# mit-acl/roman

Measured on AMD Instinct MI355X. Metric: submap-pair alignments/sec + p50 latency at n=m=200 objects, d=512, higher is better.
Workload: dtype f64 (fixed-point SpMV sums); 1 GPU; config 3: batch of 256 submap pairs per GPU, n=200 m=200 d=512, method=semanticgrav (xyz + 512-d descriptors + gravity prior); p50 latency measured on config 2 (single pair); pairs_per_call=256, n=200, m=200, d=512, method=semanticgrav, batches_in_flight=3

## Files before the change

include/roman_hip.h:

```cpp
#ifndef ROMAN_HIP_H
#define ROMAN_HIP_H

#include <stdint.h>

#ifdef __cplusplus
extern "C" {
#endif

#if defined(__GNUC__)
#define ROMAN_API __attribute__((visibility("default")))
#else
#define ROMAN_API
#endif

#define ROMAN_MAX_RATIO_FEATURES 8

#define ROMAN_OK                0
#define ROMAN_E_INVALID        -1
#define ROMAN_E_NO_DEVICE      -2
#define ROMAN_E_HIP            -3
#define ROMAN_E_NOMEM          -4
#define ROMAN_E_UNSUPPORTED    -5
#define ROMAN_E_TOO_LARGE      -6
#define ROMAN_E_INTERNAL       -7
// ... 283 lines not shown
                                int32_t S, const roman_submap_desc_t* descs,
                                double* pool, int32_t* count, int32_t* src, int64_t* ids_out, int32_t* status,
                                int32_t desc_dim, double* desc_out);

ROMAN_API int roman_submaps(roman_ctx_t* ctx, const roman_submap_params_t* sparams, int32_t N, int32_t F,
                            const double* seg_feats, const double* seg_times, const int64_t* seg_ids,
                            int32_t S, const roman_submap_desc_t* descs,
                            double* pool, int32_t* count, int32_t* src, int64_t* ids_out, int32_t* status,
                            int32_t desc_dim, double* desc_out);


typedef struct roman_frame_select_params {
    int32_t thin;
    int32_t want_mean;
    double  thin_dist;
    int32_t reserved[2];
} roman_frame_select_params_t;

ROMAN_API int roman_frame_select_dev(roman_ctx_t* ctx, const roman_frame_select_params_t* fparams, int32_t S, int32_t cap,
                                     const int32_t* count, const int32_t* src, int32_t N, const double* seg_times,
                                     int32_t Nf, const double* frame_times, const double* frame_pos, int32_t d, const double* frame_desc,
                                     uint64_t* mask, int32_t* n_sel, double* span, double* mean);

ROMAN_API int roman_frame_select(roman_ctx_t* ctx, const roman_frame_select_params_t* fparams, int32_t S, int32_t cap,
                                 const int32_t* count, const int32_t* src, int32_t N, const double* seg_times,
                                 int32_t Nf, const double* frame_times, const double* frame_pos, int32_t d, const double* frame_desc,
                                 uint64_t* mask, int32_t* n_sel, double* span, double* mean);

ROMAN_API int roman_stacked_sim_dev(roman_ctx_t* ctx, int32_t d, int32_t Nf0, const double* desc0, int32_t S0, const uint64_t* mask0,
                                    int32_t Nf1, const double* desc1, int32_t S1, const uint64_t* mask1, double* sim);

ROMAN_API int roman_stacked_sim(roman_ctx_t* ctx, int32_t d, int32_t Nf0, const double* desc0, int32_t S0, const uint64_t* mask0,
                                int32_t Nf1, const double* desc1, int32_t S1, const uint64_t* mask1, double* sim);

ROMAN_API int roman_ctx_set_stacked_band(roman_ctx_t* ctx, int32_t rows);


#define ROMAN_GRID_NEARBY  1
#define ROMAN_GRID_SKIP    2
#define ROMAN_GRID_GATED   4
#define ROMAN_GRID_TODO    8

typedef struct roman_grid_gate_params {
    double  radius;
    double  skip_distance;
    int32_t desc_dim;
    int32_t reserved0;
    double  desc_thresh;
    int32_t single_robot_lc;
    int32_t reserved1;
    double  lc_time_thresh;
    int32_t reserved[2];
} roman_grid_gate_params_t;

ROMAN_API int roman_grid_gate_dev(roman_ctx_t* ctx, const roman_grid_gate_params_t* gparams, int32_t S0, int32_t S1,
                                  const double* pos0, const double* pos_gt0, const double* T_w0, const double* time0, const double* desc0,
                                  const double* pos1, const double* pos_gt1, const double* T_w1, const double* time1, const double* desc1,
                                  double* dist, int32_t* flags, double* yaw_deg, double* sim, double* T_ij,
                                  int32_t* pairs, double* T_ref, int32_t* enable, int32_t* n_todo);

ROMAN_API int roman_grid_gate(roman_ctx_t* ctx, const roman_grid_gate_params_t* gparams, int32_t S0, int32_t S1,
                              const double* pos0, const double* pos_gt0, const double* T_w0, const double* time0, const double* desc0,
                              const double* pos1, const double* pos_gt1, const double* T_w1, const double* time1, const double* desc1,
                              double* dist, int32_t* flags, double* yaw_deg, double* sim, double* T_ij,
                              int32_t* pairs, double* T_ref, int32_t* enable, int32_t* n_todo);

ROMAN_API int roman_grid_gate_sim_dev(roman_ctx_t* ctx, const roman_grid_gate_params_t* gparams, int32_t S0, int32_t S1,
                                      const double* pos0, const double* pos_gt0, const double* T_w0, const double* time0,
                                      const double* pos1, const double* pos_gt1, const double* T_w1, const double* time1,
                                      double* dist, int32_t* flags, double* yaw_deg, const double* sim, double* T_ij,
                                      int32_t* pairs, double* T_ref, int32_t* enable, int32_t* n_todo);

ROMAN_API int roman_grid_gate_sim(roman_ctx_t* ctx, const roman_grid_gate_params_t* gparams, int32_t S0, int32_t S1,
                                  const double* pos0, const double* pos_gt0, const double* T_w0, const double* time0,
                                  const double* pos1, const double* pos_gt1, const double* T_w1, const double* time1,
                                  double* dist, int32_t* flags, double* yaw_deg, const double* sim, double* T_ij,
                                  int32_t* pairs, double* T_ref, int32_t* enable, int32_t* n_todo);



ROMAN_API int roman_submaps_fill_dev(roman_ctx_t* ctx, int32_t point_dim, int32_t cap, int32_t N, int32_t F,
                                     const double* seg_feats, const int64_t* seg_ids, int32_t S, const roman_submap_desc_t* descs,
                                     const int32_t* count, const int32_t* src, double* pool, int64_t* ids_out,
                                     int32_t desc_dim, double* desc_out);

ROMAN_API int roman_submaps_fill(roman_ctx_t* ctx, int32_t point_dim, int32_t cap, int32_t N, int32_t F,
                                 const double* seg_feats, const int64_t* seg_ids, int32_t S, const roman_submap_desc_t* descs,
                                 const int32_t* count, const int32_t* src, double* pool, int64_t* ids_out,
                                 int32_t desc_dim, double* desc_out);

ROMAN_API int roman_submap_boxes_dev(roman_ctx_t* ctx, int32_t S, int32_t F, int32_t cap, const double* pool, const int32_t* count,
                                     const double* T_odom_center, double* box);

ROMAN_API int roman_submap_boxes(roman_ctx_t* ctx, int32_t S, int32_t F, int32_t cap, const double* pool, const int32_t* count,
                                 const double* T_odom_center, double* box);

ROMAN_API int roman_grid_gate_aabb_dev(roman_ctx_t* ctx, const roman_grid_gate_params_t* gparams, int32_t S0, int32_t S1,
                                       const double* pos0, const double* pos_gt0, const double* T_w0, const double* time0, const double* desc0,
                                       const double* pos1, const double* pos_gt1, const double* T_w1, const double* time1, const double* desc1,
                                       double* dist, int32_t* flags, double* yaw_deg, double* sim, double* T_ij,
                                       int32_t* pairs, double* T_ref, int32_t* enable, int32_t* n_todo,
                                       const double* box0, const double* box1, const double* sim_in);

ROMAN_API int roman_grid_gate_aabb(roman_ctx_t* ctx, const roman_grid_gate_params_t* gparams, int32_t S0, int32_t S1,
                                   const double* pos0, const double* pos_gt0, const double* T_w0, const double* time0, const double* desc0,
                                   const double* pos1, const double* pos_gt1, const double* T_w1, const double* time1, const double* desc1,
                                   double* dist, int32_t* flags, double* yaw_deg, double* sim, double* T_ij,
                                   int32_t* pairs, double* T_ref, int32_t* enable, int32_t* n_todo,
                                   const double* box0, const double* box1, const double* sim_in);


ROMAN_API int roman_create_all_to_all(int32_t n1, int32_t n2, int32_t* out);

ROMAN_API int roman_score(roman_ctx_t* ctx, const roman_params_t* params,
                const double* D1, int32_t n1, const double* D2, int32_t n2, int32_t F,
                const int32_t* assoc, int32_t n_assoc);

ROMAN_API int roman_set_matrix_data(roman_ctx_t* ctx, const roman_params_t* params,
                          const double* M, const double* C, int32_t n);

ROMAN_API int roman_solve(roman_ctx_t* ctx, const double* u0);

ROMAN_API int roman_num_associations(const roman_ctx_t* ctx, int32_t* n_assoc);
ROMAN_API int roman_num_selected(const roman_ctx_t* ctx, int32_t* n_sel);
ROMAN_API int roman_get_selected_associations(const roman_ctx_t* ctx, int32_t* out);
ROMAN_API int roman_get_solution(const roman_ctx_t* ctx, int32_t* nodes, double* u, double* score,
                       roman_stats_t* stats);
ROMAN_API int roman_get_dense_matrices(const roman_ctx_t* ctx, double* M, double* C);
ROMAN_API int roman_get_upper_csr(const roman_ctx_t* ctx, int64_t* nnz, int64_t* rowptr ,
                        int32_t* cols, double* vals, double* diag );


ROMAN_API int roman_pose_batch(roman_ctx_t* ctx, int32_t dim, int32_t B,
                     const double* pts1, const double* pts2, const int64_t* corr_off,
                     double* T_out, int32_t* status_out);


#define ROMAN_STAGE_SINGLE   0
#define ROMAN_STAGE_COUNT_PASS 1
#define ROMAN_STAGE_FILL     2
#define ROMAN_STAGE_SOLVE    3
#define ROMAN_STAGE_COUNT    4
ROMAN_API int roman_profile_enable(roman_ctx_t* ctx, int on);
ROMAN_API int roman_profile_reset(roman_ctx_t* ctx);
ROMAN_API int roman_profile_get(roman_ctx_t* ctx, double ms[ROMAN_STAGE_COUNT],
                      int64_t launches[ROMAN_STAGE_COUNT]);

ROMAN_API int roman_debug_math(roman_ctx_t* ctx, int kind, const double* in1, const double* in2,
                     int64_t n, double* out);
ROMAN_API int roman_debug_cosine(roman_ctx_t* ctx, const roman_params_t* params,
                       const double* D1, int32_t n1, const double* D2, int32_t n2, int32_t F,
                       double* out);
ROMAN_API int roman_debug_live(const roman_ctx_t* ctx, int32_t* n_live, int32_t* idx, double* score);

ROMAN_API const char* roman_version(void);

#ifdef __cplusplus
}
#endif
#endif
```

roman_amd/_abi.py:

```python
import ctypes as C
import os

ROMAN_MAX_RATIO_FEATURES = 8

ROMAN_OK = 0
ROMAN_E_INVALID = -1
ROMAN_E_NOMEM = -4
ROMAN_E_UNSUPPORTED = -5
ROMAN_E_TOO_LARGE = -6
ROMAN_E_INTERNAL = -7
ROMAN_ST_OK = 0
ROMAN_ST_EMPTY_MAP = 1
ROMAN_ST_INSUFFICIENT = 2
ROMAN_ST_MAXITER = 4
ROMAN_ST_ASSOC_TRUNCATED = 8
ROMAN_ST_TIE_FALLBACK = 16
ROMAN_ST_WORKSPACE = 32
ROMAN_ST_INTERNAL = 64

ROMAN_INV_EUCLIDEAN = 0
ROMAN_INV_ROMAN = 1
ROMAN_INV_EUCLIDEAN_PRUNED = 2

ROMAN_FUSE_GEOMETRIC_MEAN = 0
# ... 175 lines not shown
    ]


class RomanSubmapDesc(C.Structure):
    _fields_ = [
        ("pos", C.c_double * 3),
        ("T_center_odom", C.c_double * 16),
        ("time", C.c_double),
        ("t_hi", C.c_double),
        ("t_lo", C.c_double),
    ]


class RomanGridGateParams(C.Structure):
    _fields_ = [
        ("radius", C.c_double),
        ("skip_distance", C.c_double),
        ("desc_dim", C.c_int32),
        ("reserved0", C.c_int32),
        ("desc_thresh", C.c_double),
        ("single_robot_lc", C.c_int32),
        ("reserved1", C.c_int32),
        ("lc_time_thresh", C.c_double),
        ("reserved", C.c_int32 * 2),
    ]


class RomanFrameSelectParams(C.Structure):
    _fields_ = [
        ("thin", C.c_int32),
        ("want_mean", C.c_int32),
        ("thin_dist", C.c_double),
        ("reserved", C.c_int32 * 2),
    ]


ROMAN_GRID_NEARBY = 1
ROMAN_GRID_SKIP = 2
ROMAN_GRID_GATED = 4
ROMAN_GRID_TODO = 8

SUBMAP_LDS_CAND = 4096

STATS_NBYTES = C.sizeof(RomanStats)
MNO_SOLUTION_NBYTES = C.sizeof(RomanMnoSolution)
RANSAC_RECORD_NBYTES = C.sizeof(RomanRansacRecord)
SUBMAP_PARAMS_NBYTES = C.sizeof(RomanSubmapParams)
SUBMAP_DESC_NBYTES = C.sizeof(RomanSubmapDesc)
GRID_GATE_PARAMS_NBYTES = C.sizeof(RomanGridGateParams)
FRAME_SELECT_PARAMS_NBYTES = C.sizeof(RomanFrameSelectParams)
STACKED_BAND_MIN = 32
LC_PARAMS_NBYTES = C.sizeof(RomanLcParams)
LC_RECORD_NBYTES = C.sizeof(RomanLcRecord)
PARAMS_NBYTES = C.sizeof(RomanParams)

_LIB = None
_LIB_PATH = os.environ.get("ROMAN_HIP_LIBRARY") or os.path.join(os.path.dirname(os.path.abspath(__file__)), "csrc", "libroman_hip.so")


class RomanHipError(RuntimeError):
    pass


def lib_path():
    return _LIB_PATH


def load_library():
    global _LIB
    if _LIB is not None:
        return _LIB
    if not os.path.exists(_LIB_PATH):
        raise RomanHipError(
            f"{_LIB_PATH} is missing: build it with `python -c 'import __graft_entry__ as g; g.build()'` "
            "(hipcc --offload-arch=gfx950).  There is no CPU fallback for roman_amd.")
    lib = C.CDLL(_LIB_PATH)
    vp, i32, i64, dbl = C.c_void_p, C.c_int32, C.c_int64, C.c_double
    P = C.POINTER
    ctxp = vp
    protos = {
        "roman_params_default": (C.c_int, [P(RomanParams)]),
        "roman_ctx_create": (C.c_int, [P(ctxp), C.c_int, vp]),
        "roman_ctx_destroy": (C.c_int, [ctxp]),
        "roman_ctx_set_pipeline": (C.c_int, [ctxp, C.c_int]),
        "roman_ctx_sync": (C.c_int, [ctxp]),
        "roman_ctx_set_host_batching": (C.c_int, [ctxp, C.c_int, C.c_int]),
        "roman_ctx_set_wide_teams": (C.c_int, [ctxp, C.c_int]),
        "roman_ctx_join": (C.c_int, [ctxp, C.c_int]),
        "roman_ctx_join_on": (C.c_int, [ctxp, C.c_int, C.c_void_p]),
        "roman_ctx_skipped": (C.c_int, [ctxp, C.c_int, P(i64)]),
        "roman_last_error": (C.c_char_p, [ctxp]),
        "roman_align_batch_dev": (C.c_int, [ctxp, P(RomanParams), i32, vp, vp, vp, vp, vp, i32,
                                            vp, vp, vp, i32, vp, vp, vp, vp, vp]),
        "roman_align_batch": (C.c_int, [ctxp, P(RomanParams), i32, vp, i64, vp, vp, vp, vp, i32,
                                        vp, vp, vp, i32, vp, vp, vp, vp, vp]),
        "roman_align_batch_resident": (C.c_int, [ctxp, P(RomanParams), i32, vp, vp, vp, vp, vp, i32,
                                                 vp, vp, vp, i32, vp, vp, vp, vp, vp]),
        "roman_lc_tail_dev": (C.c_int, [ctxp, P(RomanLcParams), i32, vp, vp, vp, vp, vp, vp, vp, vp, vp, vp, vp, vp]),
        "roman_align_lc_batch_dev": (C.c_int, [ctxp, P(RomanParams), i32, vp, vp, vp, vp, vp, i32,
                                               vp, vp, vp, i32, vp, vp, vp, vp, vp,
                                               P(RomanLcParams), vp, vp, vp, vp, vp, vp, vp, vp, vp]),
        "roman_align_lc_batch": (C.c_int, [ctxp, P(RomanParams), i32, vp, i64, vp, vp, vp, vp, i32,
                                           vp, vp, vp, i32, vp, vp, vp, vp, vp,
                                           P(RomanLcParams), vp, vp, vp, i32, vp, vp, i32, vp, vp, vp, vp]),
        "roman_shared_ids_dev": (C.c_int, [ctxp, i32, vp, vp, vp, vp, vp, vp, vp]),
        "roman_shared_reduce_dev": (C.c_int, [ctxp, i32, i32, vp, i64, vp, vp, vp, vp, vp, vp, vp]),
        "roman_align_lc_batch_ids": (C.c_int, [ctxp, P(RomanParams), i32, vp, i64, vp, vp, vp, vp, i32,
                                               vp, vp, vp, i32, vp, vp, vp, vp, vp,
                                               P(RomanLcParams), vp, vp, vp, i32, vp, vp, i32, vp, vp, vp, vp,
                                               vp, vp, vp, vp]),
        "roman_mno_batch_dev": (C.c_int, [ctxp, P(RomanParams), i32, vp, vp, vp, vp, vp, i32,
                                          vp, vp, i32, i32, vp, vp, vp]),
        "roman_mno_batch": (C.c_int, [ctxp, P(RomanParams), i32, vp, i64, vp, vp, vp, vp, i32,
                                      vp, vp, i32, i32, vp, vp, vp]),
        "roman_ransac_batch_dev": (C.c_int, [ctxp, P(RomanRansacParams), i32, vp, vp, vp, vp, vp, i32, vp, vp, vp]),
        "roman_ransac_batch": (C.c_int, [ctxp, P(RomanRansacParams), i32, vp, i64, vp, vp, vp, vp, i32, vp, vp, vp]),
        "roman_submaps_dev": (C.c_int, [ctxp, P(RomanSubmapParams), i32, i32, vp, vp, vp, i32, vp, vp, vp, vp, vp, vp, i32, vp]),
        "roman_submaps": (C.c_int, [ctxp, P(RomanSubmapParams), i32, i32, vp, vp, vp, i32, vp, vp, vp, vp, vp, vp, i32, vp]),
        "roman_grid_gate_dev": (C.c_int, [ctxp, P(RomanGridGateParams), i32, i32] + [vp] * 19),
        "roman_grid_gate": (C.c_int, [ctxp, P(RomanGridGateParams), i32, i32] + [vp] * 19),
        "roman_grid_gate_sim_dev": (C.c_int, [ctxp, P(RomanGridGateParams), i32, i32] + [vp] * 17),
        "roman_grid_gate_sim": (C.c_int, [ctxp, P(RomanGridGateParams), i32, i32] + [vp] * 17),
        "roman_submaps_fill_dev": (C.c_int, [ctxp, i32, i32, i32, i32, vp, vp, i32, vp, vp, vp, vp, vp, i32, vp]),
        "roman_submaps_fill": (C.c_int, [ctxp, i32, i32, i32, i32, vp, vp, i32, vp, vp, vp, vp, vp, i32, vp]),
        "roman_submap_boxes_dev": (C.c_int, [ctxp, i32, i32, i32, vp, vp, vp, vp]),
        "roman_submap_boxes": (C.c_int, [ctxp, i32, i32, i32, vp, vp, vp, vp]),
        "roman_grid_gate_aabb_dev": (C.c_int, [ctxp, P(RomanGridGateParams), i32, i32] + [vp] * 22),
        "roman_grid_gate_aabb": (C.c_int, [ctxp, P(RomanGridGateParams), i32, i32] + [vp] * 22),
        "roman_frame_select_dev": (C.c_int, [ctxp, P(RomanFrameSelectParams), i32, i32, vp, vp, i32, vp, i32, vp, vp, i32, vp, vp, vp, vp, vp]),
        "roman_frame_select": (C.c_int, [ctxp, P(RomanFrameSelectParams), i32, i32, vp, vp, i32, vp, i32, vp, vp, i32, vp, vp, vp, vp, vp]),
        "roman_stacked_sim_dev": (C.c_int, [ctxp, i32, i32, vp, i32, vp, i32, vp, i32, vp, vp]),
        "roman_stacked_sim": (C.c_int, [ctxp, i32, i32, vp, i32, vp, i32, vp, i32, vp, vp]),
        "roman_ctx_set_stacked_band": (C.c_int, [ctxp, i32]),
        "roman_ctx_has_history": (C.c_int, [ctxp, P(RomanParams), i32, P(i32)]),
        "roman_ctx_cosine_screen_stats": (C.c_int, [ctxp, P(C.c_int64), P(C.c_int64), P(C.c_double)]),
        "roman_create_all_to_all": (C.c_int, [i32, i32, vp]),
        "roman_deal_problems": (C.c_int, [i32, vp, vp, vp, i32, i32, vp, P(i32)]),
        "roman_score": (C.c_int, [ctxp, P(RomanParams), vp, i32, vp, i32, i32, vp, i32]),
        "roman_set_matrix_data": (C.c_int, [ctxp, P(RomanParams), vp, vp, i32]),
        "roman_solve": (C.c_int, [ctxp, vp]),
        "roman_num_associations": (C.c_int, [ctxp, P(i32)]),
        "roman_num_selected": (C.c_int, [ctxp, P(i32)]),
        "roman_get_selected_associations": (C.c_int, [ctxp, vp]),
        "roman_get_solution": (C.c_int, [ctxp, vp, vp, P(dbl), P(RomanStats)]),
        "roman_get_dense_matrices": (C.c_int, [ctxp, vp, vp]),
        "roman_get_upper_csr": (C.c_int, [ctxp, P(i64), vp, vp, vp, vp]),
        "roman_pose_batch": (C.c_int, [ctxp, i32, i32, vp, vp, vp, vp, vp]),
        "roman_profile_enable": (C.c_int, [ctxp, C.c_int]),
        "roman_profile_reset": (C.c_int, [ctxp]),
        "roman_profile_get": (C.c_int, [ctxp, P(dbl), P(i64)]),
        "roman_debug_math": (C.c_int, [ctxp, C.c_int, vp, vp, i64, vp]),
        "roman_debug_cosine": (C.c_int, [ctxp, P(RomanParams), vp, i32, vp, i32, i32, vp]),
        "roman_debug_live": (C.c_int, [ctxp, P(i32), vp, vp]),
        "roman_version": (C.c_char_p, []),
    }
    for name, (res, args) in protos.items():
        fn = getattr(lib, name)
        fn.restype = res
        fn.argtypes = args
    lib._roman_symbols = tuple(protos)
    _LIB = lib
    return lib


EXPORTED_SYMBOLS = (
    "roman_params_default", "roman_ctx_create", "roman_ctx_destroy", "roman_ctx_set_pipeline", "roman_ctx_sync", "roman_ctx_set_host_batching", "roman_ctx_set_wide_teams", "roman_ctx_join", "roman_ctx_join_on",
    "roman_ctx_skipped", "roman_last_error",
    "roman_align_batch_dev", "roman_align_batch", "roman_align_batch_resident", "roman_lc_tail_dev", "roman_align_lc_batch_dev", "roman_align_lc_batch", "roman_shared_ids_dev", "roman_shared_reduce_dev", "roman_align_lc_batch_ids", "roman_mno_batch_dev", "roman_mno_batch", "roman_ransac_batch_dev", "roman_ransac_batch", "roman_submaps_dev", "roman_submaps", "roman_grid_gate_dev", "roman_grid_gate", "roman_grid_gate_sim_dev", "roman_grid_gate_sim", "roman_submaps_fill_dev", "roman_submaps_fill", "roman_submap_boxes_dev", "roman_submap_boxes", "roman_grid_gate_aabb_dev", "roman_grid_gate_aabb", "roman_frame_select_dev", "roman_frame_select", "roman_stacked_sim_dev", "roman_stacked_sim", "roman_ctx_set_stacked_band", "roman_ctx_has_history", "roman_ctx_cosine_screen_stats", "roman_deal_problems", "roman_create_all_to_all", "roman_score",
    "roman_set_matrix_data", "roman_solve", "roman_num_associations", "roman_num_selected",
    "roman_get_selected_associations", "roman_get_solution", "roman_get_dense_matrices",
    "roman_get_upper_csr", "roman_pose_batch", "roman_profile_enable", "roman_profile_reset",
    "roman_profile_get", "roman_debug_math", "roman_debug_cosine", "roman_debug_live",
    "roman_version",
)
```

roman_amd/csrc/kernels.hip.h:

```cpp
#pragma once
#include <hip/hip_cooperative_groups.h>
#include <hip/hip_runtime.h>
#include <stdint.h>
#include <type_traits>
#include "../../include/roman_hip.h"

namespace roman {

constexpr int WAVE = 64;
constexpr int STREAM_MAXL = 3072;

struct DevParams {
    roman_params_t p;
    double sig2;
    double sin_unc;
    double x_eps;
    double x_mindist;
    int32_t single;
    int32_t gravity;
    int32_t F;
    int32_t max_compact;
    int32_t gmode;
    int32_t diag_one;
    int32_t keep_all;
// ... 2287 lines not shown
#define LMARK(i_) do { } while (0)
#endif
        for (int q = tid; q < L; q += LISTS_NT) degS[q] = degGiven ? rowCnt[lo + q] : 0u;
        __syncthreads();
        if (!degGiven) {
        sweep([&](int k, unsigned long long m, int c) {
            if (m) {
                atomicAdd(&degS[k], (uint32_t)__popcll(m));
                while (m) { atomicAdd(&degS[(c << 6) + __builtin_ctzll(m)], 1u); m &= m - 1ull; }
            }
        });
        __syncthreads();
        }
        LMARK(1);
        int N = 64; while (N < L) N <<= 1;
        if (eqMax <= 0 || !place_keys(L, N, eqMax, [&](int k) { return degS[k]; }, keyS, reinterpret_cast<uint32_t*>(tabS), reinterpret_cast<uint32_t*>(tabS) + (STREAM_MAXL + 64), tmpS, wsum)) {
        for (int t = tid; t < N; t += LISTS_NT) keyS[t] = (t < L) ? (((degS[t] + 1u) << 12) | (uint32_t)(4095 - t)) : 0u;
        __syncthreads();
        for (int k2 = 2; k2 <= N; k2 <<= 1)
            for (int j2 = k2 >> 1; j2 > 0; j2 >>= 1) {
                for (int t = tid; t < (N >> 1); t += LISTS_NT) {
                    const int i1 = ((t & ~(j2 - 1)) << 1) | (t & (j2 - 1)), i2 = i1 | j2;
                    const uint32_t a = keyS[i1], c2 = keyS[i2];
                    const bool desc = (i1 & k2) == 0;
                    if ((a < c2) == desc) { keyS[i1] = c2; keyS[i2] = a; }
                }
                __syncthreads();
            }
        }
        LMARK(2);
        uint32_t total = 0;
        {
            const int PER = (L + LISTS_NT - 1) / LISTS_NT;
            uint32_t sum = 0;
            for (int t = 0; t < PER; ++t) {
                const int q = tid * PER + t;
                if (q < L) sum += (min((keyS[q] >> 12) - 1u, (uint32_t)(L - 1 - q)) + 3u) & ~3u;
            }
            const uint32_t inc = wave_incl_scan(sum);
            if (lane == WAVE - 1) wsum[w] = inc;
            __syncthreads();
            uint32_t wbase = 0;
            for (int t = 0; t < NW; ++t) { if (t < w) wbase += wsum[t]; total += wsum[t]; }
            if (tid == 0) {
                const unsigned long long base = atomicAdd(&tot->listTop, (unsigned long long)total);
                st[b].listOff = (int64_t)base;
                const bool fits = (long long)(base + total) <= capList;
                if (!fits) { st[b].kind = 2; atomicAdd(&tot->overflow, 1); }
                okS = fits ? 1 : 0;
            }
            uint32_t run = wbase + inc - sum;
            for (int t = 0; t < PER; ++t) {
                const int q = tid * PER + t;
                if (q < L) {
                    const uint32_t k = 4095u - (keyS[q] & 4095u);
                    perm[lo + q] = k; rowPos[lo + k] = (uint32_t)q; tmpS[q] = (uint16_t)k;
                    tabS[k] = ((unsigned long long)run << 16) | (unsigned long long)q; listOff[lo + q] = run; degS[k] = 0u;
                    run += (min((keyS[q] >> 12) - 1u, (uint32_t)(L - 1 - q)) + 3u) & ~3u;
                }
            }
        }
        __syncthreads();
        if (!okS) continue;
        uint16_t* const lists = listPool + st[b].listOff;
        LMARK(3);
        {
        uint32_t* const qw = qS + w * LISTS_QCAP;
        uint32_t qn = 0;
        auto lds_order = [&]() {
            __builtin_amdgcn_fence(__ATOMIC_RELEASE, "wavefront"); __builtin_amdgcn_wave_barrier(); __builtin_amdgcn_fence(__ATOMIC_ACQUIRE, "wavefront");
        };
        auto place = [&](uint32_t base, uint32_t n, auto full) {
            constexpr int CH = LISTS_QRUN / WAVE;
            uint32_t kk[CH], qq[CH], slot[CH]; unsigned long long tk[CH], tq[CH]; bool act[CH];
#pragma unroll
            for (int x = 0; x < CH; ++x) {
                const uint32_t idx = (uint32_t)(x * WAVE + lane);
                act[x] = decltype(full)::value || idx < n;
                const uint32_t e = qw[base + (act[x] ? idx : 0u)];
                kk[x] = e >> 16; qq[x] = e & 0xffffu;
                tk[x] = tabS[kk[x]]; tq[x] = tabS[qq[x]];
            }
#pragma unroll
            for (int x = 0; x < CH; ++x) {
                const bool mine = ((uint32_t)tk[x] & 0xffffu) < ((uint32_t)tq[x] & 0xffffu);
                if (act[x]) slot[x] = atomicAdd(&degS[mine ? kk[x] : qq[x]], 1u);
            }
#pragma unroll
            for (int x = 0; x < CH; ++x) {
                const bool mine = ((uint32_t)tk[x] & 0xffffu) < ((uint32_t)tq[x] & 0xffffu);
                const uint32_t at = (uint32_t)((mine ? tk[x] : tq[x]) >> 16) + slot[x];
                const uint16_t v = (uint16_t)(mine ? qq[x] : kk[x]);
                if (act[x]) { if (at < (uint32_t)winCap) winS[at] = v; else lists[at] = v; }
            }
        };
        auto drain = [&]() {
            if (qn >= (uint32_t)LISTS_QRUN) {
                lds_order();
                while (qn >= (uint32_t)LISTS_QRUN) { qn -= LISTS_QRUN; place(qn, LISTS_QRUN, std::true_type{}); }
                lds_order();
            }
        };
        sweep([&](int k, unsigned long long m, int c) {
            const uint32_t cnt = (uint32_t)__popcll(m);
            const uint32_t incl = wave_incl_scan(cnt);
            const uint32_t npairs = (uint32_t)__builtin_amdgcn_readlane((int)incl, WAVE - 1);
            const uint32_t kq = ((uint32_t)k << 16) | (uint32_t)(c << 6);
            if (qn + npairs <= (uint32_t)LISTS_QCAP) {
                uint32_t at = qn + incl - cnt;
                while (m) { qw[at++] = kq + (uint32_t)__builtin_ctzll(m); m &= m - 1ull; }
                qn += npairs;
            } else {
                while (true) {
                    const unsigned long long bm = __ballot(m != 0ull);
                    if (bm == 0ull) break;
                    if (m) {
                        qw[qn + __builtin_amdgcn_mbcnt_hi((uint32_t)(bm >> 32), __builtin_amdgcn_mbcnt_lo((uint32_t)bm, 0u))] = kq + (uint32_t)__builtin_ctzll(m);
                        m &= m - 1ull;
                    }
                    qn += (uint32_t)__popcll(bm);
                    drain();
                }
            }
            drain();
        });
        lds_order();
        if (qn) place(0u, qn, std::false_type{});
        }
        __syncthreads();
        LMARK(4);
        for (int p = tid; p < L; p += LISTS_NT) {
            const uint32_t k = tmpS[p];
            const uint32_t cnt = degS[k];
            rowCnt[lo + p] = cnt;
            const uint32_t o = (uint32_t)(tabS[k] >> 16);
            for (uint32_t e = o + cnt; e < o + ((cnt + 3u) & ~3u); ++e) { if (e < (uint32_t)winCap) winS[e] = (uint16_t)0xffffu; else lists[e] = (uint16_t)0xffffu; }
            dst.lp[lo + p] = src.lp[lo + k]; dst.ld[lo + p] = src.ld[lo + k];
        }
        {
            const uint32_t nq = min(total, (uint32_t)winCap) >> 2;
            __syncthreads();
            for (uint32_t i = (uint32_t)tid; i < nq; i += LISTS_NT)
                reinterpret_cast<uint2*>(lists)[i] = reinterpret_cast<const uint2*>(winS)[i];
        }
#ifdef ROMAN_LISTS_TIMING
        LMARK(5);
        if (tid == 0 && (b & 63) == 0) printf("[k_lists] b=%d L=%d cycles: degrees %llu sort %llu offsets %llu scatter %llu tail %llu\n", b, L,
                                              tl_[1] - tl_[0], tl_[2] - tl_[1], tl_[3] - tl_[2], tl_[4] - tl_[3], tl_[5] - tl_[4]);
#endif
#undef LMARK
    }
}

__global__ void __launch_bounds__(64) k_slicegeom(const ProbDesc* __restrict__ probs, ProbState* __restrict__ st,
                                                  const uint32_t* __restrict__ rowCnt,
                                                  uint32_t* __restrict__ sliceWidth, uint32_t* __restrict__ sliceBase)
{
    const int b = blockIdx.x, lane = threadIdx.x;
    if (st[b].kind != 0) return;
    const int L = st[b].L;
    const int64_t lo = probs[b].liveOff;
    const int nsl = (L + 63) >> 6;
    uint32_t width = 0;
    if (lane < nsl) {
        const int hi = min(L, (lane << 6) + 64);
        for (int p = lane << 6; p < hi; ++p) width = max(width, rowCnt[lo + p]);
        width = (width + 3u) & ~3u;
        sliceWidth[lo + lane] = width;
    }
    const uint32_t v = width * 64u;
    const uint32_t ex = wave_excl_scan(v, lane);
    if (lane < nsl) sliceBase[lo + lane] = ex;
    if (lane == WAVE - 1) st[b].nnzCap = ex + v;
}

__global__ void __launch_bounds__(1024) k_probscan(int B, int NG , long long capNnz, ProbState* __restrict__ st, BatchTotals* __restrict__ tot)
{
    __shared__ long long shl[17];
    __shared__ int shi[17];
    __shared__ int red[1];
    const int tid = threadIdx.x, nt = blockDim.x;
    const int PER = (B + nt - 1) / nt;
    const int b0 = tid * PER, b1 = min(B, b0 + PER);
    constexpr int PC = 8;
    int cK[PC], cL[PC]; uint32_t cC[PC];
#pragma unroll
    for (int j = 0; j < PC; ++j) { const int b = b0 + j; const bool in = j < PER && b < b1; cK[j] = in ? st[b].kind : 2; cL[j] = in ? st[b].L : 0; cC[j] = in ? st[b].nnzCap : 0u; }
    auto get = [&](int b, int& kind, int& L, long long& cap) {
        const int j = b - b0;
        if (j < PC) {
#pragma unroll
            for (int t = 0; t < PC; ++t) if (t == j) { kind = cK[t]; L = cL[t]; cap = (long long)cC[t]; }
        } else { kind = st[b].kind; L = st[b].L; cap = (long long)st[b].nnzCap; }
        if (kind >= 2) cap = 0;
    };
    long long sC = 0;
    for (int b = b0; b < b1; ++b) { int kind, L; long long cap; get(b, kind, L, cap); sC += cap; }
    long long totC; int totG;
    const long long baseC = block_excl_scan(sC, shl, totC);
    int sG = 0;
    {
        long long acc = baseC;
        for (int b = b0; b < b1; ++b) {
            int kind, L; long long cap; get(b, kind, L, cap);
            acc += cap;
            if (kind == 0 && acc <= capNnz) sG += min(NG, (L + 63) >> 6);
        }
    }
    const int baseG = block_excl_scan(sG, shi, totG);
    if (tid == 0) red[0] = 0;
    __syncthreads();
    int nover = 0;
    {
        long long acc = baseC; int gacc = baseG;
        for (int b = b0; b < b1; ++b) {
            int kind, L; long long cap; get(b, kind, L, cap);
            const bool fits = acc + cap <= capNnz;
            const int ng = (kind == 0 && fits) ? min(NG, (L + 63) >> 6) : 0;
            st[b].nnzOff = fits ? acc : 0; st[b].sgBase = gacc;
            if (!fits && kind < 2) { st[b].kind = 2; ++nover; }
            acc += cap; gacc += ng;
        }
    }
    for (int off = 32; off > 0; off >>= 1) nover += __shfl_xor(nover, off);
    if ((tid & 63) == 0 && nover) atomicAdd(&red[0], nover);
    __syncthreads();
    if (tid == 0) { tot->nnzTotal = totC < capNnz ? totC : capNnz; tot->sliceGroups = totG; tot->needNnz = totC; tot->overflow += red[0]; }
}

constexpr int FILL_E = 1;
constexpr int FILL_Q = 256;

constexpr int FILL_RPB = 128;
struct FillRows { int32_t* k; int32_t* i; int32_t* j; uint32_t* base; double* s; double* za; double* zb; };
constexpr int FILL_ROWBYTES = 4 * 4 + 3 * 8;

template <bool GRAV, typename IdxT, int CM, bool QUAD>
__device__ __forceinline__ uint32_t fill_item(const DevParams& D, const ProbDesc& pd, int L, int row0, int nrows, int wq0, int Ww,
                                              int w, int wpb, int lane,
                                              const int32_t* cI, const int32_t* cJ, const double* cS,
                                              const double* cZa, const double* cZb, const uint32_t* cBase, const uint32_t* cPos,
                                              const double* __restrict__ TA, const double* __restrict__ TB,
                                              const unsigned long long* __restrict__ mbase, const uint32_t* __restrict__ pbase,
                                              const FillRows& R ,
                                              uint32_t* qK, uint32_t* qQ, uint32_t* qE,
                                              IdxT* __restrict__ cols, double* __restrict__ vals)
{
    constexpr bool LDSCOL = CM == 1;
    const int W = (L + 63) >> 6;
    const int64_t nwords = (int64_t)nrows * Ww;
    const int w0 = wq0 >> 6;
    const unsigned long long lt = (1ull << lane) - 1ull;
    uint32_t head = 0, queued = 0, upper = 0;

    auto evaluate = [&](uint32_t take) {
        __builtin_amdgcn_fence(__ATOMIC_RELEASE, "wavefront");
        __builtin_amdgcn_wave_barrier();
        __builtin_amdgcn_fence(__ATOMIC_ACQUIRE, "wavefront");
        bool on[FILL_E]; int rl[FILL_E], k[FILL_E], q[FILL_E]; uint32_t e[FILL_E];
        int i[FILL_E], j[FILL_E], iq[FILL_E], jq[FILL_E]; double sk[FILL_E], sq[FILL_E], dz[FILL_E];
        uint32_t base[FILL_E], pk[FILL_E], pq[FILL_E];
#pragma unroll
        for (int h = 0; h < FILL_E; ++h) {
            const uint32_t idx = (uint32_t)lane + 64u * (uint32_t)h;
            on[h] = idx < take;
            const uint32_t s = (head + (on[h] ? idx : 0u)) & (FILL_Q - 1);
            rl[h] = (int)qK[s]; k[h] = R.k[rl[h]]; q[h] = (int)qQ[s]; e[h] = qE[s];
        }
#pragma unroll
        for (int h = 0; h < FILL_E; ++h) {
            if (LDSCOL) {
                i[h] = cI[k[h]]; j[h] = cJ[k[h]]; iq[h] = cI[q[h]]; jq[h] = cJ[q[h]]; sk[h] = cS[k[h]]; sq[h] = cS[q[h]];
                dz[h] = GRAV ? (cZa[k[h]] - cZa[q[h]]) - (cZb[k[h]] - cZb[q[h]]) : 0.0;
                base[h] = cBase[k[h]]; pk[h] = cPos[k[h]]; pq[h] = cPos[q[h]];
            } else {
                const int r_ = rl[h], ql = q[h] - wq0;
                i[h] = R.i[r_]; j[h] = R.j[r_]; iq[h] = cI[ql]; jq[h] = cJ[ql]; sk[h] = R.s[r_]; sq[h] = cS[ql];
                dz[h] = GRAV ? (R.za[r_] - cZa[ql]) - (R.zb[r_] - cZb[ql]) : 0.0;
                base[h] = R.base[r_]; pk[h] = (uint32_t)(row0 + r_); pq[h] = cPos[ql];
            }
        }
        double a[FILL_E], bb[FILL_E];
#pragma unroll
        for (int h = 0; h < FILL_E; ++h) { a[h] = TA[(int64_t)i[h] * pd.n1 + iq[h]]; bb[h] = TB[(int64_t)j[h] * pd.n2 + jq[h]]; }
#pragma unroll
        for (int h = 0; h < FILL_E; ++h) {
            double c;
            if (GRAV && D.gmode != 3) {
                const double ch = fabs(a[h] - bb[h]);
                const double hm = a[h] > bb[h] ? a[h] : bb[h];
                double cv = fabs(dz[h]) - D.sin_unc * hm;
                if (cv < 0.0) cv = 0.0;
                c = sqrt(ch * ch + cv * cv);
            } else {
                c = fabs(a[h] - bb[h]);
            }
            const double sa = fx_exp(((-0.5 * c) * c) / D.sig2);
            const double v = fuse_pair(D, sa, sk[h], sq[h]);
            const bool keep = v > D.p.affinityeps;
            if (on[h]) {
                cols[col_pos<QUAD>(base[h] & ~63u, base[h] & 63u, e[h])] = keep ? (IdxT)pq[h] : fb_inert<IdxT>(pk[h]);
                vals[val_pos<QUAD>(base[h] & ~63u, base[h] & 63u, e[h])] = keep ? v : 0.0;
                upper += (keep && q[h] > k[h]) ? 1u : 0u;
            }
        }
        head = (head + take) & (FILL_Q - 1); queued -= take;
    };

    const int64_t nblk = (nwords + 63) >> 6;
    unsigned long long m_next = 0ull; uint32_t p_next = 0u, k_next = 0u;
    auto fetch = [&](int64_t x_) {
        const int r_ = (int)x_ / Ww;
        const int64_t a_ = (int64_t)R.k[r_] * W + (w0 + ((int)x_ - r_ * Ww));
        k_next = (uint32_t)r_; m_next = mbase[a_]; p_next = pbase[a_];
    };
    {
        const int64_t x = (int64_t)w * 64 + lane;
        if (w < nblk && x < nwords) fetch(x);
    }
    for (int64_t blk = w; blk < nblk; blk += wpb) {
        unsigned long long m = m_next; uint32_t e = p_next; const uint32_t kl = k_next;
        const int64_t x = blk * 64 + lane;
        {
            const int64_t xn = x + (int64_t)wpb * 64;
            m_next = 0ull; p_next = 0u;
            if (blk + wpb < nblk && xn < nwords) fetch(xn);
// ... 1014 lines not shown
constexpr int ST_MAXSL = STREAM_MAXL / 64;
constexpr int SMALL_MAXL = 128;
constexpr int COO_E = 6;
constexpr int COO_CAP = 64 * COO_E;
constexpr uint32_t ST_CZ = 0x8000u, ST_MASK = 0x7fffu;
constexpr unsigned long long FX_MAGIC_BITS = 0x4338000000000000ull;
#define FX_MAGIC 6755399441055744.0

#define ROMAN_GLOBAL __attribute__((address_space(1)))
#define ROMAN_LDS __attribute__((address_space(3)))
typedef const ROMAN_GLOBAL unsigned long long* g_quad_cp;
typedef const ROMAN_GLOBAL dbl2_t* g_pair_cp;
typedef const ROMAN_LDS double* l_vec_cp;
typedef ROMAN_LDS unsigned long long* l_acc_p;

__device__ __forceinline__ uint32_t uni(uint32_t v) { return (uint32_t)__builtin_amdgcn_readfirstlane((int)v); }
__device__ __forceinline__ int uni(int v) { return __builtin_amdgcn_readfirstlane(v); }
__device__ __forceinline__ double uni(double v)
{
    const long long b = __double_as_longlong(v);
    const int lo = __builtin_amdgcn_readfirstlane((int)b), hi = __builtin_amdgcn_readfirstlane((int)(b >> 32));
    return __longlong_as_double(((long long)hi << 32) | (unsigned int)lo);
}

template <int CTRL, int ROWMASK>
__device__ __forceinline__ double dpp_mov(double v)
{
    const long long b = __double_as_longlong(v);
    const int lo = __builtin_amdgcn_update_dpp(0, (int)b, CTRL, ROWMASK, 0xf, false);
    const int hi = __builtin_amdgcn_update_dpp(0, (int)(b >> 32), CTRL, ROWMASK, 0xf, false);
    return __longlong_as_double(((long long)hi << 32) | (unsigned int)lo);
}
__device__ __forceinline__ double wave_sum63(double v)
{
    v += dpp_mov<0xB1, 0xf>(v);
    v += dpp_mov<0x4E, 0xf>(v);
    v += dpp_mov<0x124, 0xf>(v);
    v += dpp_mov<0x128, 0xf>(v);
    v += dpp_mov<0x142, 0xa>(v);
    v += dpp_mov<0x143, 0xc>(v);
    return v;
}
__device__ __forceinline__ double wave_max63(double v)
{
    v = fmax(v, dpp_mov<0xB1, 0xf>(v));
    v = fmax(v, dpp_mov<0x4E, 0xf>(v));
    v = fmax(v, dpp_mov<0x124, 0xf>(v));
    v = fmax(v, dpp_mov<0x128, 0xf>(v));
    v = fmax(v, dpp_mov<0x142, 0xa>(v));
    v = fmax(v, dpp_mov<0x143, 0xc>(v));
    return v;
}
__device__ __forceinline__ double readlane63(double v)
{
    const long long b = __double_as_longlong(v);
    const int lo = __builtin_amdgcn_readlane((int)b, 63), hi = __builtin_amdgcn_readlane((int)(b >> 32), 63);
    return __longlong_as_double(((long long)hi << 32) | (unsigned int)lo);
}

constexpr int RED_STRIDE = 8;
constexpr int red_doubles(int NW) { return 2 * NW * RED_STRIDE + 8 > 72 ? 2 * NW * RED_STRIDE + 8 : 72; }
template <int NW, int NS, int NM>
__device__ __forceinline__ void block_red(double (&sv)[NS > 0 ? NS : 1], double (&mv)[NM > 0 ? NM : 1], double* red, int& par, int tid)
{
    static_assert(NS + NM <= RED_STRIDE, "reduction scratch");
    static_assert(NW == 1 || NW == 4 || NW == 8 || NW == 16, "cross-wave butterfly");
    if (NW == 1) {
#pragma unroll
        for (int i = 0; i < NS; ++i) sv[i] = uni(readlane63(wave_sum63(sv[i])));
#pragma unroll
        for (int i = 0; i < NM; ++i) mv[i] = uni(readlane63(wave_max63(mv[i])));
        __syncthreads();
        return;
    }
    double* rr = red + NW * RED_STRIDE * par;
    par ^= 1;
    const int w = uni(tid >> 6);
#pragma unroll
    for (int i = 0; i < NS; ++i) {
        const double s = readlane63(wave_sum63(sv[i]));
        if ((tid & 63) == 0) rr[RED_STRIDE * w + i] = s;
    }
#pragma unroll
    for (int i = 0; i < NM; ++i) {
        const double m = readlane63(wave_max63(mv[i]));
        if ((tid & 63) == 0) rr[RED_STRIDE * w + NS + i] = m;
    }
    __syncthreads();
    const int src = (tid & 63) & (NW - 1);
#pragma unroll
    for (int i = 0; i < NS; ++i) {
        double v = rr[RED_STRIDE * src + i];
        v += dpp_mov<0xB1, 0xf>(v);
        v += dpp_mov<0x4E, 0xf>(v);
        if (NW > 4) v += dpp_mov<0x124, 0xf>(v);
        if (NW > 8) v += dpp_mov<0x128, 0xf>(v);
        sv[i] = uni(v);
    }
#pragma unroll
    for (int i = 0; i < NM; ++i) {
        double v = rr[RED_STRIDE * src + NS + i];
        v = fmax(v, dpp_mov<0xB1, 0xf>(v));
        v = fmax(v, dpp_mov<0x4E, 0xf>(v));
        if (NW > 4) v = fmax(v, dpp_mov<0x124, 0xf>(v));
        if (NW > 8) v = fmax(v, dpp_mov<0x128, 0xf>(v));
        mv[i] = uni(v);
    }
}

template <int NW, int NS>
__device__ __forceinline__ const double* block_post(const double (&sv)[NS], double* red, int& par, int tid)
{
    static_assert(NW == 4 || NW == 8 || NW == 16, "cross-wave butterfly");
    double* rr = red + NW * RED_STRIDE * par;
    par ^= 1;
    const int w = uni(tid >> 6);
#pragma unroll
    for (int i = 0; i < NS; ++i) {
        const double s = readlane63(wave_sum63(sv[i]));
        if ((tid & 63) == 0) rr[RED_STRIDE * w + i] = s;
    }
    return rr;
}
template <int NW, int NS>
__device__ __forceinline__ void block_collect(double (&sv)[NS], const double* rr, int tid)
{
    const int src = (tid & 63) & (NW - 1);
#pragma unroll
    for (int i = 0; i < NS; ++i) {
        double v = rr[RED_STRIDE * src + i];
        v += dpp_mov<0xB1, 0xf>(v);
        v += dpp_mov<0x4E, 0xf>(v);
        if (NW > 4) v += dpp_mov<0x124, 0xf>(v);
        if (NW > 8) v += dpp_mov<0x128, 0xf>(v);
        sv[i] = uni(v);
    }
}

__device__ __forceinline__ double fx_decode(unsigned long long a, double inv)
{
    return fma((double)(uint32_t)(a >> 32), 4294967296.0, (double)(uint32_t)a) * inv;
}

template <int NW, bool HASCZ, int MAXL, bool COOONLY = false >
__device__ void solve_up(const DevParams& D, int b, const ProbDesc& pd, ProbState* st,
                         const double* __restrict__ feats, const int32_t* __restrict__ assoc,
                         const int32_t* __restrict__ plp , const int32_t* __restrict__ lpAsc,
                         const uint32_t* __restrict__ rowPosPool, const double* __restrict__ pld ,
                         const uint32_t* __restrict__ sliceBasePool,
                         const uint16_t* __restrict__ colsPool, const double* __restrict__ valsPool,
                         const double* __restrict__ u0, const SolveOut& O,
                         double* xg , unsigned long long* accM , unsigned long long* accC , int Lc,
                         uint32_t* cumQ , double* red, int* sint, unsigned char* cooLds ,
                         int cooPre = -1 ,
                         int rbPre = -1 )
{
    constexpr int NT = NW * 64;
#ifdef ROMAN_SOLVE_TIMING
    const unsigned long long tentry_ = __builtin_readcyclecounter();
#endif
#ifdef ROMAN_SMALL_TIMING
    const unsigned long long tw0_ = wall_clock64();
#endif
    constexpr int KMAX = (MAXL + NT - 1) / NT;
    constexpr int LCAP = MAXL + 64;
    const roman_params_t& P = D.p;
    const double p_eps = uni(P.eps), p_beta = uni(P.beta), p_tol_u = uni(P.tol_u), p_tol_F = uni(P.tol_F);
    const int p_maxin = uni(P.maxiniters), p_maxout = uni(P.maxoliters), p_maxls = uni(P.maxlsiters), p_rescale = uni(P.rescale_u0);
    const int tid = threadIdx.x, lane = tid & 63, w = uni(tid >> 6);
#define FOR_K_ALL(k_, p_) _Pragma("unroll") for (int k_ = 0; k_ < KMAX; ++k_) if ([[maybe_unused]] const int p_ = tid + k_ * NT; true)
#define FOR_K(k_, p_) _Pragma("unroll") for (int k_ = 0; k_ < KMAX; ++k_) if ([[maybe_unused]] const int p_ = tid + k_ * NT; NW != 1 || k_ < kUsed)
    const int L = uni(st[b].L), rb = rbPre >= 0 ? rbPre : uni(st[b].rowBase);
    const int kUsed = uni((L + NT - 1) / NT);
    const int64_t lo = pd.liveOff;
    const int nsl = (L + 63) >> 6;
    int par = 0;

    int status = ROMAN_ST_OK;
    roman_stats_t S;
    S.n_assoc_in = pd.nA; S.n_live = L; S.nnz_upper = (int64_t)st[b].nnzUpper;
    S.n_pass = 0; S.outer_iters = 0; S.inner_iters = 0; S.ls_trials = 0; S.score = 0.0; S.d_final = 0.0;
    int n_pass = 0, ls_trials = 0, inner_iters = 0;
    double F = 0.0, d = 0.0;
    if (pd.n1 == 0 || pd.n2 == 0) status |= ROMAN_ST_EMPTY_MAP;
    if (L <= 0) {
        finish_one(D, b, pd, feats, assoc, plp, lpAsc, rowPosPool, nullptr, O, nullptr, nullptr, nullptr, nullptr, L, rb, lo, F, status, S, red, sint);
        return;
    }
#ifdef ROMAN_SOLVE_TIMING
    unsigned long long tacc[8] = {0, 0, 0, 0, 0, 0, 0, 0}, tcnt[8] = {0, 0, 0, 0, 0, 0, 0, 0};
    unsigned long long tlast = __builtin_readcyclecounter();
#endif
    g_quad_cp cbase = (g_quad_cp)(colsPool + st[b].nnzOff) + lane;
    g_pair_cp vbase = (g_pair_cp)(valsPool + st[b].nnzOff) + lane;
    l_vec_cp xl = (l_vec_cp)xg;
    l_acc_p aM = (l_acc_p)accM; l_acc_p aC = (l_acc_p)accC;

    __syncthreads();
    const uint32_t cqv = cooPre >= 0 ? 0u : ((lane < nsl) ? (sliceBasePool[lo + lane] >> 8) : (st[b].nnzCap >> 8));
#define CUMQ(s_) ((uint32_t)__builtin_amdgcn_readlane((int)cqv, (s_)))
    for (int p = tid; p < Lc; p += NT) { xg[p] = 0.0; accM[p] = 0ull; accC[p] = 0ull; }
    double u[KMAX], Wu[KMAX], sd[KMAX], tk[KMAX], Mn[KMAX], Cn[KMAX];
    FOR_K_ALL(k, p) {
        const bool in = p < L;
        sd[k] = in ? pld[lo + p] : 0.0;
        u[k] = in ? (u0 ? u0[lo + plp[lo + p]] : 1.0) : 0.0;
        Wu[k] = tk[k] = Mn[k] = Cn[k] = 0.0;
    }
    __syncthreads();

    [[maybe_unused]] uint32_t cpq[COO_E]; [[maybe_unused]] double cv[COO_E];
    [[maybe_unused]] int cooRounds = -1;
    if constexpr (NW == 1) {
        uint32_t* lpq = reinterpret_cast<uint32_t*>(cooLds); double* lv = reinterpret_cast<double*>(cooLds + 4 * COO_CAP);
        const uint32_t Tq = CUMQ(nsl);
        const uint32_t q1 = nsl > 1 ? CUMQ(1) : Tq;
        uint32_t cnt = 0;
        if (cooPre >= 0) {
            cnt = (uint32_t)cooPre;
            cooRounds = (int)((cnt + 63u) >> 6);
#pragma unroll
            for (int e = 0; e < COO_E; ++e) {
                const uint32_t at = (uint32_t)lane * (uint32_t)cooRounds + (uint32_t)e;
                const bool have = e < cooRounds && at < cnt;
                const uint32_t dummy = (uint32_t)L + (uint32_t)lane;
                cpq[e] = have ? lpq[at] : (dummy | (dummy << 8) | 0x10000u);
                cv[e] = have ? lv[at] : 0.0;
            }
            __syncthreads();
        } else
        if (!COOONLY && (unsigned long long)st[b].nnzUpper <= (unsigned long long)COO_CAP && nsl <= 2) {
            for (uint32_t qq = 0; qq < Tq; ++qq) {
                const unsigned long long cw = cbase[(size_t)qq * 64];
                const dbl2_t v0 = vbase[(size_t)(2 * qq) * 64], v1 = vbase[(size_t)(2 * qq + 1) * 64];
                const uint32_t row = (qq >= q1 ? 64u : 0u) + (uint32_t)lane;
                const double v4[4] = {v0.x, v0.y, v1.x, v1.y};
#pragma unroll
                for (int e = 0; e < 4; ++e) {
                    const uint32_t lab = (uint32_t)(cw >> (16 * e)) & 0xffffu, col = lab & ST_MASK;
                    const bool real = col < (uint32_t)L;
                    const unsigned long long m_ = __ballot(real);
                    if (real) {
                        const uint32_t at = cnt + (uint32_t)__builtin_amdgcn_mbcnt_hi((uint32_t)(m_ >> 32), __builtin_amdgcn_mbcnt_lo((uint32_t)m_, 0u));
                        if (at < (uint32_t)COO_CAP) { lpq[at] = row | (col << 8) | ((lab & ST_CZ) ? 0x10000u : 0u); lv[at] = v4[e]; }
                    }
                    cnt += (uint32_t)__popcll(m_);
                }
            }
            __syncthreads();
            if (cnt <= (uint32_t)COO_CAP) {
                cooRounds = (int)((cnt + 63u) >> 6);
#pragma unroll
                for (int e = 0; e < COO_E; ++e) {
                    const uint32_t at = (uint32_t)lane * (uint32_t)cooRounds + (uint32_t)e;
                    const bool have = e < cooRounds && at < cnt;
                    const uint32_t dummy = (uint32_t)L + (uint32_t)lane;
                    cpq[e] = have ? lpq[at] : (dummy | (dummy << 8) | 0x10000u);
                    cv[e] = have ? lv[at] : 0.0;
                }
            }
            __syncthreads();
        }
    }

    [[maybe_unused]] const double* pendRR = nullptr; [[maybe_unused]] bool pend = false;
    double usum = 0.0, alpha = 1.0, unsum = 0.0, du2 = 0.0, xmaxT = 0.0;
    auto collect_pending = [&]() {
        if constexpr (NW != 1) {
            if (pend) { double q2[2]; block_collect<NW, 2>(q2, pendRR, tid); unsum = q2[0]; du2 = q2[1]; pend = false; }
        }
    };
    auto spmv = [&](double xmax, int mp1, const bool split, const double de_) {
        TMARK(3);
        if (!(xmax > 0.0) || mp1 <= 0) {
            if constexpr (NW != 1) { if (pend) { __syncthreads(); collect_pending(); } }
            FOR_K(k, p) { Mn[k] = 0.0; Cn[k] = 0.0; }
            ++n_pass;
            return;
        }
        const double de = (!split && de_ > 0.0) ? de_ : 0.0;
        int e_ = (int)((__double_as_longlong(xmax) >> 52) & 0x7ff) - 1023;
        int s_ = 48 - e_;
        if (de > 0.0) s_ -= (int)((__double_as_longlong(1.0 + de) >> 52) & 0x7ff) - 1023 + 1;
        s_ = s_ > 960 ? 960 : (s_ < -960 ? -960 : s_);
        const double sc = bits_f64((unsigned long long)(1023 + s_) << 52), inv = bits_f64((unsigned long long)(1023 - s_) << 52);
        bool streamed = false;
        if constexpr (NW == 1) streamed = cooRounds >= 0;
        const int Sx = (COOONLY || streamed) ? 0 : min(nsl, (mp1 + 63) >> 6);
        const uint32_t T = COOONLY ? 0u : CUMQ(Sx);
        const uint32_t qs = (uint32_t)(((unsigned long long)T * (unsigned)w) / NW), qe = (uint32_t)(((unsigned long long)T * (unsigned)(w + 1)) / NW);
        [[maybe_unused]] unsigned long long rc[ST_D]; [[maybe_unused]] dbl2_t rv0[ST_D], rv1[ST_D];
        if constexpr (!COOONLY) {
            const uint32_t qlast = (qe > qs ? qe : qs + 1u) - 1u;
            g_quad_cp cb0 = T ? cbase : (g_quad_cp)colsPool + lane;
            g_pair_cp vb0 = T ? vbase : (g_pair_cp)valsPool + lane;
#pragma unroll
            for (int t = 0; t < ST_D; ++t) {
                const uint32_t qq = min(qs + (uint32_t)t, qlast);
                rc[t] = cb0[(size_t)qq * 64];
                rv0[t] = vb0[(size_t)(2 * qq) * 64]; rv1[t] = vb0[(size_t)(2 * qq + 1) * 64];
            }
        }
        FOR_K(k, p) if (p < L) xg[p] = tk[k] * sc;
        __syncthreads();
        collect_pending();
        TMARK(6);
        if constexpr (NW == 1) {
            if (cooRounds >= 0) {
#pragma unroll
                for (int e = 0; e < COO_E; ++e) {
                    if (e < cooRounds) {
                        const uint32_t p_ = cpq[e] & 0xffu, q_ = (cpq[e] >> 8) & 0xffu;
                        const bool cz = HASCZ && (cpq[e] & 0x10000u);
                        const double xp_ = xl[p_], xq_ = xl[q_];
                        const double w_ = cz ? cv[e] : cv[e] + de;
                        if (xq_ != 0.0) {
                            __hip_atomic_fetch_add(aM + p_, (unsigned long long)__double_as_longlong(fma(w_, xq_, FX_MAGIC)) - FX_MAGIC_BITS, __ATOMIC_RELAXED, __HIP_MEMORY_SCOPE_WORKGROUP);
                            if (split && !cz) __hip_atomic_fetch_add(aC + p_, (unsigned long long)__double_as_longlong(xq_ + FX_MAGIC) - FX_MAGIC_BITS, __ATOMIC_RELAXED, __HIP_MEMORY_SCOPE_WORKGROUP);
                        }
                        if (xp_ != 0.0) {
                            __hip_atomic_fetch_add(aM + q_, (unsigned long long)__double_as_longlong(fma(w_, xp_, FX_MAGIC)) - FX_MAGIC_BITS, __ATOMIC_RELAXED, __HIP_MEMORY_SCOPE_WORKGROUP);
                            if (split && !cz) __hip_atomic_fetch_add(aC + q_, (unsigned long long)__double_as_longlong(xp_ + FX_MAGIC) - FX_MAGIC_BITS, __ATOMIC_RELAXED, __HIP_MEMORY_SCOPE_WORKGROUP);
                        }
                        __builtin_amdgcn_sched_barrier(0);
                    }
                }
            }
        }
        auto stream = [&](auto split_tag) {
            constexpr bool SPLIT = decltype(split_tag)::value;
            int s = 0;
            {
                int lo_ = 0, hi_ = Sx;
                while (hi_ - lo_ > 1) { const int mid_ = (lo_ + hi_) >> 1; if (CUMQ(mid_) <= qs) lo_ = mid_; else hi_ = mid_; }
                s = lo_;
            }
            uint32_t nextB = CUMQ(s + 1);
            unsigned long long smI = 0ull; [[maybe_unused]] unsigned long long scI = 0ull;
            uint32_t pieceQ = qs;
            double xp = xl[s * 64 + lane];
            double xpn = xl[(s + 1) * 64 + lane];
            [[maybe_unused]] unsigned long long iCp = (unsigned long long)__double_as_longlong(xp + FX_MAGIC) - FX_MAGIC_BITS;
            l_vec_cp ga[4], gn[4]; double xa[4], xn[4];
#define UP_GATHER(C_, G_, X_)                                                                               \
            {                                                                                               \
                const uint32_t lo__ = (uint32_t)(C_), hi__ = (uint32_t)((C_) >> 32);                        \
                (G_)[0] = xl + (lo__ & ST_MASK); (G_)[1] = xl + ((lo__ >> 16) & ST_MASK);                   \
                (G_)[2] = xl + (hi__ & ST_MASK); (G_)[3] = xl + ((hi__ >> 16) & ST_MASK);                   \
                (X_)[0] = *(G_)[0]; (X_)[1] = *(G_)[1]; (X_)[2] = *(G_)[2]; (X_)[3] = *(G_)[3];             \
            }
#define UP_PUSH(G_, OFF_, V_) __hip_atomic_fetch_add((l_acc_p)(G_) + (OFF_), (V_), __ATOMIC_RELAXED, __HIP_MEMORY_SCOPE_WORKGROUP)
#define UP_CONSUME(Q_, C_, V0_, V1_)                                                                        \
            {                                                                                               \
                [[maybe_unused]] const uint32_t clo = (uint32_t)(C_), chi = (uint32_t)((C_) >> 32);         \
                                                         \
                const double w0 = SPLIT ? (V0_).x : ((HASCZ && (clo & ST_CZ)) ? (V0_).x : (V0_).x + de);    \
                const double w1 = SPLIT ? (V0_).y : ((HASCZ && (clo & (ST_CZ << 16))) ? (V0_).y : (V0_).y + de); \
                const double w2 = SPLIT ? (V1_).x : ((HASCZ && (chi & ST_CZ)) ? (V1_).x : (V1_).x + de);    \
                const double w3 = SPLIT ? (V1_).y : ((HASCZ && (chi & (ST_CZ << 16))) ? (V1_).y : (V1_).y + de); \
                smI += (unsigned long long)__double_as_longlong(fma(w0, xa[0], FX_MAGIC));                  \
                smI += (unsigned long long)__double_as_longlong(fma(w1, xa[1], FX_MAGIC));                  \
                smI += (unsigned long long)__double_as_longlong(fma(w2, xa[2], FX_MAGIC));                  \
                smI += (unsigned long long)__double_as_longlong(fma(w3, xa[3], FX_MAGIC));                  \
                if constexpr (SPLIT) {                                                                      \
                    if (HASCZ) {                                                                            \
                        scI += (unsigned long long)__double_as_longlong(((clo & ST_CZ) ? 0.0 : xa[0]) + FX_MAGIC); \
                        scI += (unsigned long long)__double_as_longlong(((clo & (ST_CZ << 16)) ? 0.0 : xa[1]) + FX_MAGIC); \
                        scI += (unsigned long long)__double_as_longlong(((chi & ST_CZ) ? 0.0 : xa[2]) + FX_MAGIC); \
                        scI += (unsigned long long)__double_as_longlong(((chi & (ST_CZ << 16)) ? 0.0 : xa[3]) + FX_MAGIC); \
                    } else {                  \
                        scI += (unsigned long long)__double_as_longlong(xa[0] + FX_MAGIC);                  \
                        scI += (unsigned long long)__double_as_longlong(xa[1] + FX_MAGIC);                  \
                        scI += (unsigned long long)__double_as_longlong(xa[2] + FX_MAGIC);                  \
                        scI += (unsigned long long)__double_as_longlong(xa[3] + FX_MAGIC);                  \
                    }                                                                                       \
                }                                                                                           \
                if (xp != 0.0) {                                \
                    UP_PUSH(ga[0], LCAP, (unsigned long long)__double_as_longlong(fma(w0, xp, FX_MAGIC)) - FX_MAGIC_BITS); \
                    UP_PUSH(ga[1], LCAP, (unsigned long long)__double_as_longlong(fma(w1, xp, FX_MAGIC)) - FX_MAGIC_BITS); \
                    UP_PUSH(ga[2], LCAP, (unsigned long long)__double_as_longlong(fma(w2, xp, FX_MAGIC)) - FX_MAGIC_BITS); \
                    UP_PUSH(ga[3], LCAP, (unsigned long long)__double_as_longlong(fma(w3, xp, FX_MAGIC)) - FX_MAGIC_BITS); \
                    if constexpr (SPLIT) {                                                                  \
                        if (!HASCZ || !(clo & ST_CZ)) UP_PUSH(ga[0], 2 * LCAP, iCp);                        \
                        if (!HASCZ || !(clo & (ST_CZ << 16))) UP_PUSH(ga[1], 2 * LCAP, iCp);                \
                        if (!HASCZ || !(chi & ST_CZ)) UP_PUSH(ga[2], 2 * LCAP, iCp);                        \
                        if (!HASCZ || !(chi & (ST_CZ << 16))) UP_PUSH(ga[3], 2 * LCAP, iCp);                \
                    }                                                                                       \
                }                                                                                           \
                if ((Q_) + 1 == nextB || (Q_) + 1 == qe) {             \
                    const unsigned long long nterm = (unsigned long long)(((Q_) + 1 - pieceQ) * 4u) * FX_MAGIC_BITS; \
                    UP_PUSH(xl + (s * 64 + lane), LCAP, smI - nterm);                                       \
                    if constexpr (SPLIT) UP_PUSH(xl + (s * 64 + lane), 2 * LCAP, scI - nterm);              \
                    smI = 0ull; scI = 0ull; pieceQ = (Q_) + 1;                                              \
                    if ((Q_) + 1 < qe) {                                                                    \
                        const int s_old_ = s;                                                               \
                        do { ++s; nextB = CUMQ(s + 1); } while (nextB <= (Q_) + 1);                         \
                        xp = (s == s_old_ + 1) ? xpn : xl[s * 64 + lane];                                   \
                        xpn = xl[(s + 1) * 64 + lane];                                                      \
                        iCp = (unsigned long long)__double_as_longlong(xp + FX_MAGIC) - FX_MAGIC_BITS;      \
                    }                                                                                       \
                }                                                                                           \
            }
            UP_GATHER(rc[0], ga, xa)
            uint32_t q0 = qs;
            for (; q0 + ST_D <= qe; q0 += ST_D) {
#pragma unroll
                for (int t = 0; t < ST_D; ++t) {
                    const uint32_t q = q0 + t;
                    const unsigned long long c = rc[t];
                    const dbl2_t v0 = rv0[t], v1 = rv1[t];
                    const uint32_t qn = min(q + (uint32_t)ST_D, qe - 1u);
                    rc[t] = cbase[(size_t)qn * 64];
                    rv0[t] = vbase[(size_t)(2 * qn) * 64]; rv1[t] = vbase[(size_t)(2 * qn + 1) * 64];
                    UP_GATHER(rc[(t + 1) % ST_D], gn, xn)
                    UP_CONSUME(q, c, v0, v1)
#pragma unroll
                    for (int e = 0; e < 4; ++e) { ga[e] = gn[e]; xa[e] = xn[e]; }
                }
            }
#pragma unroll
            for (int t = 0; t < ST_D; ++t) {
                const uint32_t q = q0 + t;
                if (q < qe) {
                    UP_GATHER(rc[(t + 1) % ST_D], gn, xn)
                    UP_CONSUME(q, rc[t], rv0[t], rv1[t])
#pragma unroll
                    for (int e = 0; e < 4; ++e) { ga[e] = gn[e]; xa[e] = xn[e]; }
                }
            }
#undef UP_CONSUME
#undef UP_PUSH
#undef UP_GATHER
        };
        if (!COOONLY && qs < qe) {
            if (split) stream(std::true_type{}); else stream(std::false_type{});
        }
        TMARK(Sx <= 2 ? 4 : 0);
        __syncthreads();
        TMARK(1);
        FOR_K(k, p) {
            if (p < L) {
                Mn[k] = fx_decode(accM[p], inv); accM[p] = 0ull;
                if (split) { Cn[k] = fx_decode(accC[p], inv); accC[p] = 0ull; } else Cn[k] = 0.0;
            } else { Mn[k] = 0.0; Cn[k] = 0.0; }
        }
        ++n_pass;
        TMARK(2);
    };

    enum { PH_RESCALE, PH_INIT, PH_TRIAL, PH_SPLIT };
    int phase = p_rescale ? PH_RESCALE : PH_INIT;
    int mp1T = 0;
    int i = 0, j = 0, kk = 0;

    auto normalize_u = [&]() {
        double r[1] = {0.0}, m0[1] = {0.0};
        FOR_K(k, p) r[0] += u[k] * u[k];
        block_red<NW, 1, 0>(r, m0, red, par, tid);
        const double nr = sqrt(r[0]);
        if (nr > 0.0) FOR_K(k, p) u[k] /= nr;
    };
    auto load_u_as_x = [&]() {
        double r0[1] = {0.0}, m2[2] = {0.0, 0.0};
        FOR_K(k, p) { tk[k] = u[k]; m2[0] = fmax(m2[0], u[k]); if (u[k] > 0.0) m2[1] = (double)(p + 1); }
        block_red<NW, 0, 2>(r0, m2, red, par, tid);
        xmaxT = m2[0]; mp1T = (int)m2[1];
    };
    auto finish_trial = [&](double r2, const double (&m2)[2]) {
        const double nr = sqrt(r2);
        double q[2] = {0.0, 0.0}, m0[1] = {0.0};
        FOR_K(k, p) {
            double t = tk[k];
            if (nr > 0.0 && t != 0.0) { t /= nr; tk[k] = t; }
            q[0] += t;
            const double df = t - u[k]; q[1] += df * df;
        }
        TMARK(3);
        if constexpr (NW == 1) { block_red<NW, 2, 0>(q, m0, red, par, tid); unsum = q[0]; du2 = q[1]; }
        else { pendRR = block_post<NW, 2>(q, red, par, tid); pend = true; }
        TMARK(7);
        xmaxT = (nr > 0.0) ? m2[0] / nr : m2[0]; mp1T = (int)m2[1];
    };
    auto build_trial = [&]() {
        double r[1] = {0.0}, m2[2] = {0.0, 0.0};
        FOR_K(k, p) {
            const double up = u[k];
            const double g = ((sd[k] + d) * up - d * usum) + Wu[k];
            double t = up + alpha * g;
            t = (p < L && t > 0.0) ? t : 0.0;
            tk[k] = t; r[0] += t * t;
            m2[0] = fmax(m2[0], t);
            if (t > 0.0) m2[1] = (double)(p + 1);
        }
        TMARK(3);
        block_red<NW, 1, 2>(r, m2, red, par, tid);
        TMARK(6);
        finish_trial(r[0], m2);
    };
    auto objective = [&](const double (&uu)[KMAX], const double (&ww)[KMAX], double us) -> double {
        double r[1] = {0.0}, m0[1] = {0.0};
        FOR_K(k, p) {
            const double up = uu[k];
            const double g = ((sd[k] + d) * up - d * us) + ww[k];
            r[0] += up * g;
        }
        block_red<NW, 1, 0>(r, m0, red, par, tid);
        return r[0];
    };
    auto d_ratio = [&](bool absval, double& acc, double& cnt) {
        double r2[2] = {0.0, 0.0}, m0[1] = {0.0};
        FOR_K(k, p) {
            const double up = u[k], Cbu = (usum - Cn[k]) - up;
            if (p < L && Cbu > p_eps && up > p_eps) { const double r_ = (Mn[k] + sd[k] * up) / Cbu; r2[0] += absval ? fabs(r_) : r_; r2[1] += 1.0; }
        }
        block_red<NW, 2, 0>(r2, m0, red, par, tid);
        acc = r2[0]; cnt = r2[1];
    };

    if (phase == PH_INIT) normalize_u();
    load_u_as_x();
    for (;;) {
        spmv(xmaxT, mp1T, phase == PH_INIT || phase == PH_SPLIT, phase == PH_TRIAL ? d : 0.0);
        if (phase == PH_RESCALE) {
            FOR_K(k, p) u[k] = (p < L) ? Mn[k] + sd[k] * u[k] : 0.0;
            normalize_u();
            load_u_as_x();
            phase = PH_INIT;
            continue;
        }
        if (phase == PH_INIT) {
            double r1[1] = {0.0}, m0[1] = {0.0};
            FOR_K(k, p) r1[0] += u[k];
            block_red<NW, 1, 0>(r1, m0, red, par, tid);
            usum = r1[0];
            double acc, cnt;
            d_ratio(false, acc, cnt);
            d = (cnt > 0.0) ? acc / cnt : 0.0;
            i = 0;
            if (i >= p_maxout) break;
        } else if (phase == PH_SPLIT) {
            double acc, cnt;
            d_ratio(true, acc, cnt);
            if (cnt > 0.0) d += acc / cnt; else break;
            ++i;
            if (i >= p_maxout) break;
        } else {
            ++ls_trials;
            const double Fnew = objective(tk, Mn, unsum);
            const double deltaF = Fnew - F;
            if (deltaF < -p_eps && kk + 1 < p_maxls) {
                alpha *= p_beta; ++kk;
                build_trial();
                continue;
            }
            const double du = sqrt(du2);
            F = Fnew; usum = unsum;
            FOR_K(k, p) { u[k] = tk[k]; Wu[k] = Mn[k]; }
            ++inner_iters; ++j;
            const bool stop = du < p_tol_u || fabs(deltaF) < p_tol_F;
            if (stop || j >= p_maxin) {
                phase = PH_SPLIT;
                continue;
            }
        }
        if (phase != PH_TRIAL) {
            FOR_K(k, p) Wu[k] = Mn[k] + Cn[k] * d;
            F = objective(u, Wu, usum); j = 0;
        }
        alpha = 1.0; kk = 0;
        build_trial();
        phase = PH_TRIAL;
    }
    if (i >= p_maxout) status |= ROMAN_ST_MAXITER;
    S.n_pass = n_pass; S.ls_trials = ls_trials; S.inner_iters = inner_iters;
    S.outer_iters = i; S.score = F; S.d_final = d;
#ifdef ROMAN_SOLVE_TIMING
    TMARK(3);
#endif
    __syncthreads();
    FOR_K(k, p) if (p < L) xg[p] = u[k];
#ifdef ROMAN_SMALL_TIMING
    const unsigned long long tt0_ = __builtin_readcyclecounter();
    const unsigned long long tw1_ = wall_clock64();
#endif
    finish_one(D, b, pd, feats, assoc, plp, lpAsc, rowPosPool, nullptr, O, xg, reinterpret_cast<double*>(accM),
               reinterpret_cast<int32_t*>(accC), reinterpret_cast<int32_t*>(accC) + Lc, L, rb, lo, F, status, S, red, sint);
#ifdef ROMAN_SOLVE_TIMING
    if (tid == 0 && O.dbg) {
        unsigned long long sum_ = 0; for (int t = 0; t < 8; ++t) sum_ += tacc[t];
        tacc[5] = __builtin_readcyclecounter() - tentry_ - sum_; tcnt[5] = 1;
        unsigned long long* dg = O.dbg + (size_t)b * 16;
        for (int t = 0; t < 8; ++t) { dg[t] = tacc[t]; dg[8 + t] = tcnt[t]; }
    }
#endif
#ifdef ROMAN_SMALL_TIMING
    if (tid == 0 && ((b & 255) == 0 || b < 2 || (NW == 1 && n_pass >= 100)))
        printf("[solve_up<%d>] b=%d L=%d nnz=%llu passes %d tail (selection, pose, outputs) %llu cycles; wall clock (10 ns): entered %llu iteration done %llu left %llu\n", NW, b, L,
               (unsigned long long)st[b].nnzUpper, n_pass, __builtin_readcyclecounter() - tt0_, tw0_, tw1_, wall_clock64());
#endif
#undef FOR_K
#undef FOR_K_ALL
#undef CUMQ
}

template <int NW, bool HASCZ, int MAXL>
__global__ void __launch_bounds__(NW * 64, NW == 1 ? 3 : 1) k_solve_up(DevParams D, int B, const ProbDesc* __restrict__ probs,
                                                      ProbState* __restrict__ st,
                                                      const double* __restrict__ feats, const int32_t* __restrict__ assoc,
                                                      const int32_t* __restrict__ plp, const int32_t* __restrict__ lpAsc,
                                                      const uint32_t* __restrict__ rowPos, const double* __restrict__ pld,
                                                      const uint32_t* __restrict__ sliceBase,
                                                      const uint16_t* __restrict__ cols, const double* __restrict__ vals,
                                                      const double* __restrict__ u0, SolveOut O,
                                                      int* __restrict__ queue, int Lc, int Llo, int Lhi, int R )
{
    extern __shared__ __attribute__((aligned(16))) unsigned char smem[];
    double* xg = reinterpret_cast<double*>(smem);
    unsigned long long* accM = reinterpret_cast<unsigned long long*>(xg + Lc);
    unsigned long long* accC = accM + Lc;
    double* red = reinterpret_cast<double*>(accC + Lc);
    uint32_t* cumQ = reinterpret_cast<uint32_t*>(red + red_doubles(NW));
    int* sint = reinterpret_cast<int*>(cumQ + ST_MAXSL + 2);
    unsigned char* cooLds = reinterpret_cast<unsigned char*>(sint + 8);
    for (;;) {
        if (threadIdx.x < WAVE) {
            const int ln = threadIdx.x;
            int base_ = B; unsigned long long m_ = 0ull;
            for (;;) {
                int t_ = 0;
                if (ln == 0) t_ = atomicAdd(queue, R);
                base_ = __builtin_amdgcn_readfirstlane(t_);
                if (base_ >= B) break;
                const int b_ = base_ + ln;
                bool take = false;
                if (ln < R && b_ < B) { const int Lq = st[b_].L; take = st[b_].kind == 0 && Lq >= Llo && Lq <= Lhi; }
                m_ = __ballot(take);
                if (m_) break;
            }
            if (ln == 0) { sint[2] = base_; sint[3] = (int)(uint32_t)m_; sint[4] = (int)(uint32_t)(m_ >> 32); }
        }
        __syncthreads();
        const int base = uni(sint[2]);
        unsigned long long mask = ((unsigned long long)(uint32_t)uni(sint[4]) << 32) | (unsigned long long)(uint32_t)uni(sint[3]);
        __syncthreads();
        if (base >= B) break;
        while (mask) {
        const int b = base + __builtin_ctzll(mask);
        mask &= mask - 1ull;
        const ProbDesc pd = probs[b];
        solve_up<NW, HASCZ, MAXL>(D, b, pd, st, feats, assoc, plp, lpAsc, rowPos, pld, sliceBase, cols, vals, u0, O,
                                  xg, accM, accC, Lc, cumQ, red, sint, cooLds);
        __syncthreads();
        }
    }
}

constexpr int SMALL_PAIR_CAP = 2304;
constexpr size_t small_lds_bytes()
{
    size_t o = (size_t)3 * 8 * (SMALL_MAXL + 64) + sizeof(double) * red_doubles(1) + sizeof(uint32_t) * (ST_MAXSL + 2) + sizeof(int) * 8;
    o = (o + 15) & ~(size_t)15;
    return o + (size_t)12 * COO_CAP + (size_t)SMALL_MAXL * (16 + 8 + 4 + 2 + 2);
}

__device__ __forceinline__ bool pair_gate_rt(const DevParams& D, int gm, double a, double bb, double dz)
{
    switch (gm) {
    case 1: return pair_gate<1>(D, a, bb, dz);
    case 2: return pair_gate<2>(D, a, bb, dz);
    case 3: return pair_gate<3>(D, a, bb, dz);
    default: return pair_gate<0>(D, a, bb, dz);
    }
}

template <bool FAST>
__global__ void __launch_bounds__(64, 3) k_small(DevParams D, int B, const ProbDesc* __restrict__ probs, ProbState* __restrict__ st,
                                              const double* __restrict__ feats, const int32_t* __restrict__ assoc,
                                              const double* __restrict__ tabPool,
                                              const int32_t* __restrict__ lp, const int32_t* __restrict__ li, const int32_t* __restrict__ lj,
                                              const double* __restrict__ ls, const double* __restrict__ ld,
                                              const double* __restrict__ lza, const double* __restrict__ lzb,
                                              int32_t* __restrict__ plp, double* __restrict__ pld, uint32_t* __restrict__ rowPos,
                                              const double* __restrict__ u0, SolveOut O, int* __restrict__ queue)
{
    constexpr int Lc1 = SMALL_MAXL + 64;
    extern __shared__ __attribute__((aligned(16))) unsigned char smem[];
    double* xg = reinterpret_cast<double*>(smem);
    unsigned long long* accM = reinterpret_cast<unsigned long long*>(xg + Lc1);
    unsigned long long* accC = accM + Lc1;
    double* red = reinterpret_cast<double*>(accC + Lc1);
    uint32_t* cumQ = reinterpret_cast<uint32_t*>(red + red_doubles(1));
    int* sint = reinterpret_cast<int*>(cumQ + ST_MAXSL + 2);
    unsigned char* cooLds = smem + (((size_t)(reinterpret_cast<unsigned char*>(sint + 8) - smem) + 15) & ~(size_t)15);
    uint32_t* lpq = reinterpret_cast<uint32_t*>(cooLds); double* lv = reinterpret_cast<double*>(cooLds + 4 * COO_CAP);
    double2* cZ = reinterpret_cast<double2*>(cooLds + 12 * COO_CAP);
    static_assert((12 * COO_CAP) % 16 == 0, "cZ alignment");
    double* cS = reinterpret_cast<double*>(cZ + SMALL_MAXL);
    uint32_t* cIJ = reinterpret_cast<uint32_t*>(cS + SMALL_MAXL);
    uint16_t* posS = reinterpret_cast<uint16_t*>(cIJ + SMALL_MAXL);
    uint16_t* degS = posS + SMALL_MAXL;
    uint16_t* pairs = reinterpret_cast<uint16_t*>(smem);
    static_assert(SMALL_PAIR_CAP * 2 <= 3 * 8 * Lc1, "pair list fits the solver's vectors");
    const int lane = threadIdx.x;
    const int gm = D.gmode;
    for (;;) {
        {
            int t_ = 0;
            if (lane == 0) t_ = atomicAdd(queue, 1);
            const int b = __builtin_amdgcn_readfirstlane(t_);
            if (b >= B) break;
            {
                const int Lq = uni_i(st[b].L);
                if (!(uni_i(st[b].kind) == 0 && Lq >= 1 && Lq <= SMALL_MAXL)) continue;
            }
            const ProbDesc pd = probs[b];
            const int L = uni_i(st[b].L);
            const int64_t lo = pd.liveOff;
            const double* TA = tabPool + pd.tabOff;
            const double* TB = TA + (int64_t)pd.n1 * pd.n1;
            __syncthreads();
#ifdef ROMAN_SMALL_TIMING
            unsigned long long ts_[8]; ts_[0] = __builtin_readcyclecounter();
#define SMARK(i_) ts_[i_] = __builtin_readcyclecounter()
#else
#define SMARK(i_) do { } while (0)
#endif
            int ri[2], rj[2], rlp[2]; double rd[2], rza[2], rzb[2]; bool rv[2];
#pragma unroll
            for (int r = 0; r < 2; ++r) {
                const int k = r * 64 + lane;
                rv[r] = k < L;
                const int kk = rv[r] ? k : 0;
                ri[r] = li[lo + kk]; rj[r] = lj[lo + kk]; rlp[r] = lp[lo + kk]; rd[r] = ld[lo + kk];
                rza[r] = lza[lo + kk]; rzb[r] = lzb[lo + kk];
                if (rv[r]) { cIJ[k] = (uint32_t)ri[r] | ((uint32_t)rj[r] << 16); cZ[k] = make_double2(rza[r], rzb[r]); cS[k] = ls[lo + kk]; }
            }
            __syncthreads();
            SMARK(1);
            unsigned long long m[2][2] = {{0ull, 0ull}, {0ull, 0ull}};
            const double* rowA[2] = {TA + (int64_t)ri[0] * pd.n1, TA + (int64_t)ri[1] * pd.n1};
            const double* rowB[2] = {TB + (int64_t)rj[0] * pd.n2, TB + (int64_t)rj[1] * pd.n2};
            const int nr = L > 64 ? 2 : 1;
#pragma unroll
            for (int wd = 0; wd < 2; ++wd) {
                const int q1 = min(L, (wd + 1) * 64);
                for (int q0 = wd * 64; q0 < q1; q0 += 4) {
                    uint32_t pk[4]; double2 zz[4]; double a[2][4], bb[2][4];
#pragma unroll
                    for (int x = 0; x < 4; ++x) { const int q = min(q0 + x, q1 - 1); pk[x] = cIJ[q]; zz[x] = cZ[q]; }
#pragma unroll
                    for (int x = 0; x < 4; ++x)
#pragma unroll
                        for (int r = 0; r < 2; ++r)
                            if (r < nr) { a[r][x] = rowA[r][pk[x] & 0xffffu]; bb[r][x] = rowB[r][pk[x] >> 16]; }
#pragma unroll
                    for (int x = 0; x < 4; ++x) {
                        if (q0 + x < q1) {
#pragma unroll
                            for (int r = 0; r < 2; ++r) {
                                if (r < nr) {
                                    const double dz = gm ? fabs((rza[r] - zz[x].x) - (rzb[r] - zz[x].y)) : 0.0;
                                    const bool is = pair_gate_rt(D, gm, a[r][x], bb[r][x], dz);
                                    m[r][wd] |= (unsigned long long)(is ? 1u : 0u) << ((q0 + x) & 63);
                                }
                            }
                        }
                    }
                }
            }
#pragma unroll
            for (int r = 0; r < 2; ++r) if (!rv[r]) { m[r][0] = 0ull; m[r][1] = 0ull; }
            SMARK(2);
            int dg[2], pos[2];
#pragma unroll
            for (int r = 0; r < 2; ++r) { dg[r] = __popcll(m[r][0]) + __popcll(m[r][1]); if (rv[r]) degS[r * 64 + lane] = (uint16_t)dg[r]; }
            __syncthreads();
#pragma unroll
            for (int r = 0; r < 2; ++r) {
                int rank = 0;
                const int k = r * 64 + lane;
                if (r < nr) for (int k2 = 0; k2 < L; ++k2) { const int d2 = (int)degS[k2]; rank += (d2 > dg[r] || (d2 == dg[r] && k2 < k)) ? 1 : 0; }
                pos[r] = rank;
                if (rv[r]) { posS[k] = (uint16_t)rank; rowPos[lo + k] = (uint32_t)rank; plp[lo + rank] = rlp[r]; pld[lo + rank] = rd[r]; }
            }
            __syncthreads();
            SMARK(3);
            uint32_t cnt[2] = {0u, 0u};
#pragma unroll
            for (int r = 0; r < 2; ++r)
#pragma unroll
                for (int wd = 0; wd < 2; ++wd) {
                    unsigned long long x = m[r][wd], keep = 0ull;
                    while (x) {
                        const int bit = __builtin_ctzll(x);
                        x &= x - 1ull;
                        if ((int)posS[wd * 64 + bit] > pos[r]) { keep |= 1ull << bit; ++cnt[r]; }
                    }
                    m[r][wd] = keep;
                }
            const uint32_t inc0 = wave_incl_scan(cnt[0]), tot0 = (uint32_t)__builtin_amdgcn_readlane((int)inc0, 63);
            const uint32_t inc1 = wave_incl_scan(cnt[1]), tot1 = (uint32_t)__builtin_amdgcn_readlane((int)inc1, 63);
            const uint32_t cand = tot0 + tot1;
            if (cand > (uint32_t)SMALL_PAIR_CAP) continue;
            uint32_t off[2] = {inc0 - cnt[0], tot0 + inc1 - cnt[1]};
#pragma unroll
            for (int r = 0; r < 2; ++r)
#pragma unroll
                for (int wd = 0; wd < 2; ++wd) {
                    unsigned long long x = m[r][wd];
                    while (x) {
                        const int bit = __builtin_ctzll(x);
                        x &= x - 1ull;
                        pairs[off[r]++] = (uint16_t)((r * 64 + lane) | ((wd * 64 + bit) << 8));
                    }
                }
            __syncthreads();
            SMARK(4);
            uint32_t nk = 0;
            for (uint32_t c0 = 0; c0 < cand; c0 += 64u) {
                const uint32_t idx = c0 + (uint32_t)lane;
                const bool have = idx < cand;
                const uint32_t pr = pairs[have ? idx : 0u];
                const int k = (int)(pr & 0xffu), q = (int)(pr >> 8);
                const uint32_t pkk = cIJ[k], pkq = cIJ[q];
                const double a = TA[(int64_t)(pkk & 0xffffu) * pd.n1 + (pkq & 0xffffu)], bb = TB[(int64_t)(pkk >> 16) * pd.n2 + (pkq >> 16)];
                const double2 zk = cZ[k], zq = cZ[q];
                const double sk = cS[k], sq = cS[q];
                double v;
                if (D.gravity) v = fill_value<true, FAST>(D, a, bb, zk.x - zq.x, zk.y - zq.y, sk * sq, sk, sq);
                else v = fill_value<false, FAST>(D, a, bb, 0.0, 0.0, sk * sq, sk, sq);
                const bool keep = have && v > D.p.affinityeps;
                const unsigned long long km = __ballot(keep);
                if (keep) {
                    const uint32_t at = nk + (uint32_t)__builtin_amdgcn_mbcnt_hi((uint32_t)(km >> 32), __builtin_amdgcn_mbcnt_lo((uint32_t)km, 0u));
                    if (at < (uint32_t)COO_CAP) { lpq[at] = (uint32_t)posS[k] | ((uint32_t)posS[q] << 8); lv[at] = v; }
                }
                nk += (uint32_t)__popcll(km);
            }
            if (nk > (uint32_t)COO_CAP) continue;
            if (lane == 0) st[b].nnzUpper = (unsigned long long)nk;
            __syncthreads();
            SMARK(5);
            solve_up<1, false, SMALL_MAXL, true>(D, b, pd, st, feats, assoc, plp, lp, rowPos, pld, nullptr, nullptr, nullptr, u0, O,
                                           xg, accM, accC, Lc1, cumQ, red, sint, cooLds, (int)nk, (int)lo);
            if (lane == 0) st[b].kind = 3;
#ifdef ROMAN_SMALL_TIMING
            SMARK(6);
            if (lane == 0 && ((b & 255) == 0 || B <= 4)) printf("[k_small] b=%d L=%d cand=%u nnz=%u cycles: rows %llu tests %llu ranks %llu keep %llu values %llu solve+tail %llu\n", b, L, cand, nk,
                                                                ts_[1] - ts_[0], ts_[2] - ts_[1], ts_[3] - ts_[2], ts_[4] - ts_[3], ts_[5] - ts_[4], ts_[6] - ts_[5]);
#endif
#undef SMARK
        }
    }
}

constexpr int WIDE_NT = 512;
constexpr int WIDE_NW = WIDE_NT / 64;
constexpr int WIDE_KW = 2;
constexpr int WIDE_NRED = 10;
constexpr int WIDE_MAXBLK = 8;
constexpr int WIDE_U = 3;
constexpr int WIDE_MAXCH = 8;

__host__ __device__ constexpr size_t wide_fixed_lds(int bmWords) { return ((size_t)3 * 8 * (size_t)bmWords + 4 * ((size_t)bmWords + 2) + 15) & ~(size_t)15; }

struct WideShared {
    double wred[2][WIDE_NW][WIDE_NRED];
    double bc[2][WIDE_NRED];
    double red[72];
    int sint[4];
    int abort_;
    int sS[WIDE_NT / 64][8];
    uint32_t upT[WIDE_MAXBLK], upCS[WIDE_MAXBLK], upPB[WIDE_MAXBLK], upSB[WIDE_MAXBLK];
    int upG[WIDE_MAXBLK], upCU[WIDE_MAXBLK];
    int upI[4];
    double upFx;
};

__device__ __forceinline__ void st_pub(double* p, double v)
{
    __hip_atomic_store(reinterpret_cast<unsigned long long*>(p), (unsigned long long)__double_as_longlong(v), __ATOMIC_RELAXED, __HIP_MEMORY_SCOPE_AGENT);
}

constexpr int WIDE_MAX_TEAMS = 32;
constexpr int WIDE_BAR_WORDS = (56 + WIDE_MAX_TEAMS) * 32;
struct WideBar { unsigned* bar; unsigned epoch; int G; int xcc; unsigned nX; unsigned nActive; unsigned long long budget ;
                 int teamMode; int tG ; int tRank ; int team; };

__device__ __forceinline__ bool wide_spin(const unsigned* word, unsigned target, unsigned* bar, unsigned long long budget)
{
    const unsigned long long t0 = wall_clock64();
    unsigned n = 0;
    while (__hip_atomic_load(word, __ATOMIC_RELAXED, __HIP_MEMORY_SCOPE_AGENT) < target) {
        __builtin_amdgcn_s_sleep(1);
        if (((++n & 255u) == 0u || budget == 0ull) && (wall_clock64() - t0 > budget || __hip_atomic_load(bar, __ATOMIC_RELAXED, __HIP_MEMORY_SCOPE_AGENT) != 0u)) {
            __hip_atomic_store(bar, 1u, __ATOMIC_RELAXED, __HIP_MEMORY_SCOPE_AGENT);
            return false;
        }
    }
    return true;
}

template <bool RELEASE>
__device__ __forceinline__ bool wide_sync(WideShared& sh, WideBar& wb, int ltid)
{
    asm volatile("s_waitcnt vmcnt(0)" ::: "memory");
    __syncthreads();
    ++wb.epoch;
    if (ltid == 0) {
        if (RELEASE) { __builtin_amdgcn_fence(__ATOMIC_RELEASE, "agent"); asm volatile("s_waitcnt vmcnt(0)" ::: "memory"); }
        unsigned* bar = wb.bar;
        bool ok = true;
        if (wb.teamMode) {
            const unsigned old = __hip_atomic_fetch_add(bar + 32 * (24 + wb.team), 1u, __ATOMIC_RELAXED, __HIP_MEMORY_SCOPE_AGENT);
            if (old + 1u == wb.epoch * (unsigned)wb.tG) __hip_atomic_store(bar + 32 * (56 + wb.team), wb.epoch, __ATOMIC_RELAXED, __HIP_MEMORY_SCOPE_AGENT);
            else ok = wide_spin(bar + 32 * (56 + wb.team), wb.epoch, bar, wb.budget);
            if (!ok) sh.abort_ = 1;
            __builtin_amdgcn_fence(__ATOMIC_ACQUIRE, "agent");
        } else {
        const unsigned old = __hip_atomic_fetch_add(bar + 32 * (1 + wb.xcc), 1u, __ATOMIC_RELAXED, __HIP_MEMORY_SCOPE_AGENT);
        if (old + 1u == wb.epoch * wb.nX) {
            __hip_atomic_fetch_add(bar + 32 * 9, 1u, __ATOMIC_RELAXED, __HIP_MEMORY_SCOPE_AGENT);
            ok = wide_spin(bar + 32 * 9, wb.epoch * wb.nActive, bar, wb.budget);
            if (ok) __hip_atomic_store(bar + 32 * (10 + wb.xcc), wb.epoch, __ATOMIC_RELAXED, __HIP_MEMORY_SCOPE_AGENT);
        } else {
            ok = wide_spin(bar + 32 * (10 + wb.xcc), wb.epoch, bar, wb.budget);
        }
        if (!ok) sh.abort_ = 1;
        __builtin_amdgcn_fence(__ATOMIC_ACQUIRE, "agent");
        }
    }
    __syncthreads();
    return sh.abort_ == 0;
}

__device__ __forceinline__ bool wide_census(WideShared& sh, WideBar& wb, int ltid)
{
    unsigned x;
    asm volatile("s_getreg_b32 %0, hwreg(HW_REG_XCC_ID)" : "=s"(x));
    wb.xcc = (int)(x & 7u);
    if (ltid == 0) {
        unsigned* bar = wb.bar;
        sh.sint[2] = (int)__hip_atomic_fetch_add(bar + 32 * 18 + wb.xcc, 1u, __ATOMIC_RELAXED, __HIP_MEMORY_SCOPE_AGENT);
        asm volatile("s_waitcnt vmcnt(0)" ::: "memory");
        __hip_atomic_fetch_add(bar + 32 * 19, 1u, __ATOMIC_RELAXED, __HIP_MEMORY_SCOPE_AGENT);
        const bool ok = wide_spin(bar + 32 * 19, (unsigned)wb.G, bar, wb.budget);
        unsigned act = 0;
        for (int t = 0; t < 8; ++t) {
            const unsigned c_ = __hip_atomic_load(bar + 32 * 18 + t, __ATOMIC_RELAXED, __HIP_MEMORY_SCOPE_AGENT);
            act += c_ ? 1u : 0u;
            if (t == wb.xcc) sh.sint[0] = (int)c_;
        }
        sh.sint[1] = (int)act;
        if (!ok) sh.abort_ = 1;
    }
    __syncthreads();
    wb.nX = (unsigned)sh.sint[0]; wb.nActive = (unsigned)sh.sint[1];
    const int rankX = sh.sint[2];
    __syncthreads();
    if (wb.teamMode) {
        const int sub = wb.teamMode, nX = (int)wb.nX;
        const int sidx = min(sub - 1, (rankX * sub) / max(nX, 1));
        const int f0 = (sidx * nX + sub - 1) / sub, f1 = ((sidx + 1) * nX + sub - 1) / sub;
        wb.tG = f1 - f0; wb.tRank = rankX - f0; wb.team = wb.xcc * sub + sidx;
    } else { wb.tG = wb.G; wb.tRank = (int)blockIdx.x; wb.team = 0; }
    return sh.abort_ == 0;
}

template <int N, int NM = 0>
__device__ __forceinline__ bool wide_reduce(double (&v)[N > 0 ? N : 1], WideShared& sh, double* slots, WideBar& wb, int ltid)
{
    static_assert(N <= WIDE_NRED && NM <= N, "slot width");
    const int lane = ltid & 63, w = ltid >> 6, par = (int)(wb.epoch & 1u);
    const int G = wb.tG;
    slots += (size_t)wb.team * 2 * (size_t)wb.G * WIDE_NRED;
    if (N > 0) {
#pragma unroll
        for (int i = 0; i < N; ++i) {
            double x = v[i];
            if (i < N - NM) { for (int off = 32; off > 0; off >>= 1) x += __shfl_xor(x, off); }
            else { for (int off = 32; off > 0; off >>= 1) x = fmax(x, __shfl_xor(x, off)); }
            if (lane == 0) sh.wred[par][w][i] = x;
        }
        __syncthreads();
        if (ltid < N) {
            double t = 0.0;
            if (ltid < N - NM) { for (int ww = 0; ww < WIDE_NW; ++ww) t += sh.wred[par][ww][ltid]; }
            else { for (int ww = 0; ww < WIDE_NW; ++ww) t = fmax(t, sh.wred[par][ww][ltid]); }
            st_pub(slots + ((size_t)par * G + wb.tRank) * WIDE_NRED + ltid, t);
        }
    }
    if (!wide_sync<false>(sh, wb, ltid)) return false;
    if (N > 0) {
        if (w == 0) {
#pragma unroll
            for (int i = 0; i < N; ++i) {
                double a = 0.0;
// ... 2066 lines not shown
```

roman_amd/csrc/roman_hip.hip:

```cpp
#include <hip/hip_runtime.h>
#include <algorithm>
#include <cmath>
#include <cstdarg>
#include <cstdint>
#include <cstdio>
#include <cstdlib>
#include <cstring>
#include <new>
#include <string>
#include <vector>

#include "kernels.hip.h"

using namespace roman;

namespace {

thread_local std::string g_last_error;

struct DevBuf {
    void* p = nullptr; size_t cap = 0;
    hipError_t ensure(size_t bytes) {
        if (bytes <= cap) return hipSuccess;
        if (p) { hipError_t e = hipFree(p); p = nullptr; cap = 0; if (e != hipSuccess) return e; }
// ... 563 lines not shown
        if (D.pre_invw > 0.0 && std::isfinite(D.pre_invw)) {
            HIPCHK(c, WS.qtabPool.ensure(sizeof(uint16_t) * 4 * (size_t)std::max<int64_t>(sumQ4, 1) + 64));
            qtab = WS.qtabPool.as<uint16_t>();
        }
        hipLaunchKernelGGL(k_tables, dim3((unsigned)((maxN + RBt - 1) / RBt), 2, B), dim3(thr), tabLds, WS.stream, D, dP, in.feats, WS.tabPool.as<double>(), RBt, qtab);
    DBG(c, "k_tables");
    }
    {
        const int maxChunks = std::max(1, (maxA + LIVE_CHUNK - 1) / LIVE_CHUNK);
        const int32_t* only = cosLive ? WS.cosDense.as<int32_t>() : nullptr;
        HIPCHK(c, WS.chunkCnt.ensure(sizeof(int32_t) * (size_t)B * (size_t)maxChunks * 4));
        hipLaunchKernelGGL(k_live<0>, dim3((unsigned)maxChunks, (unsigned)B), dim3(256), 0, WS.stream, D, dP, dS, in.feats, in.assoc, WS.cosPool.as<double>(), WS.sTmp.as<double>(), PP.lp ,
                           WS.chunkCnt.as<int32_t>(), maxChunks, LP.lp, LP.li, LP.lj, LP.ls, LP.ld, LP.lza, LP.lzb, only);
        hipLaunchKernelGGL(k_live<1>, dim3((unsigned)maxChunks, (unsigned)B), dim3(256), 0, WS.stream, D, dP, dS, in.feats, in.assoc, WS.cosPool.as<double>(), WS.sTmp.as<double>(), PP.lp ,
                           WS.chunkCnt.as<int32_t>(), maxChunks, LP.lp, LP.li, LP.lj, LP.ls, LP.ld, LP.lza, LP.lzb, only);
    DBG(c, "k_live");
    }
    t0.stop();

    const int expL = std::max(SZ.expectMaxL, 1);
    const int ldsPerRow = ((2 * std::max(maxN, 1) + 1 + 1) & ~1) + 2;
    const int colBytesC = D.gravity ? 20 : 4;
    const int Lneed = (expL + 255) & ~255;
    const int NRc = ((size_t)16 * 2 * ldsPerRow * sizeof(double) + (size_t)std::min(Lneed, 2048) * colBytesC <= c->lds_max) ? 2 : 1;
    int wpb = 16;
    while (wpb > 1 && (size_t)wpb * NRc * ldsPerRow * sizeof(double) + 256 * colBytesC > c->lds_max) wpb >>= 1;
    if ((size_t)wpb * NRc * ldsPerRow * sizeof(double) + 256 * colBytesC > c->lds_max)
        return fail(c, ROMAN_E_TOO_LARGE, "maps of %d objects exceed the LDS table staging of this build", maxN);
    const int ldsPerWave = NRc * ldsPerRow;
    const size_t tabLds = (size_t)wpb * ldsPerWave * sizeof(double);
    int TCc = (int)std::min<size_t>((c->lds_max - tabLds) / colBytesC, 32768) & ~255;
    TCc = std::min(TCc, Lneed);
    const size_t pairLds = tabLds + (size_t)TCc * colBytesC;
    const int pairGrid = c->num_cu * std::max(1, std::min(2048 / (wpb * 64), (int)(c->lds_max / pairLds)));
    int preNR = 0, preWpb = 0, preTC = 0; size_t preLds = 0;
    const int preRow = (2 * std::max(maxN, 1) + 1 + 3) & ~3;
    {
        const char* preEnv = getenv("ROMAN_COUNT_PRE");
        const bool want = (preEnv ? preEnv[0] != '0' : true) && D.pre_invw > 0.0 && std::isfinite(D.pre_invw) && Lneed <= (preEnv ? 16000 : 4096) && maxN <= 32767;
        if (want) {
            const int tc = Lneed;
            for (int wp = PRE_WAVES; wp >= 8; wp -= 4) {
                const size_t need = (size_t)(tc + PRE_COLPAD + 4) * 4 + (size_t)wp * (size_t)count_pre_wave_bytes(preRow, tc);
                if (need <= c->lds_max) { preNR = PRE_NR; preWpb = wp; preTC = tc; preLds = need; break; }
            }
        }
    }

    StageTimer t1(c, ROMAN_STAGE_COUNT_PASS);
    {
        static const char* fusedEnv = getenv("ROMAN_SMALL_FUSED");
        const bool want = smallOut != nullptr && !(fusedEnv && fusedEnv[0] == '0') && D.p.maxiniters >= 1 && D.p.maxlsiters >= 1 && maxTab > 0 &&
                          (c->hist.valid ? c->hist.smallSeen : maxA <= 16 * SMALL_MAXL);
        if (want) {
            SolveOut O;
            int rc = make_solve_out(c, B, sumA, *smallOut, &O);
            if (rc) return rc;
            HIPCHK(c, hipMemsetAsync(WS.queue.as<int>() + 8, 0, sizeof(int), WS.stream));
            const bool fast = D.single && (D.p.single_mode == ROMAN_SINGLE_BOTH || D.p.single_mode == ROMAN_SINGLE_OFFDIAG) && D.p.distance_weight == 1.0 &&
                              D.p.fusion_method != ROMAN_FUSE_ARITHMETIC_MEAN && D.p.fusion_method != ROMAN_FUSE_PRODUCT;
            constexpr size_t ldsSmall = small_lds_bytes();
            const int grid = std::max(1, std::min(B, c->num_cu * 12));
            auto ks = fast ? k_small<true> : k_small<false>;
            hipLaunchKernelGGL(ks, dim3(grid), dim3(64), ldsSmall, WS.stream, D, B, dP, dS, in.feats, in.assoc, WS.tabPool.as<double>(),
                               LP.lp, LP.li, LP.lj, LP.ls, LP.ld, LP.lza, LP.lzb, WS.plp.as<int32_t>(), WS.pld.as<double>(), WS.rowPos.as<uint32_t>(),
                               smallU0, O, WS.queue.as<int>() + 8);
    DBG(c, "k_small");
            static const char* onlyEnv = getenv("ROMAN_SMALL_ONLY");
            D.small_only = (c->hist.valid && !c->hist.generalSeen && !(onlyEnv && onlyEnv[0] == '0')) ? 1 : 0;
            Dout->small_only = D.small_only;
        }
    }
    hipLaunchKernelGGL(k_rowbase, dim3(1), dim3(B > 256 ? 1024 : 256), 0, WS.stream, B, RPB, SZ.capMaskWords, dS, dT, D.small_only, cosScreen ? (const int32_t*)WS.cosDense.as<int32_t>() : (const int32_t*)nullptr);
    DBG(c, "k_rowbase");
    if (!D.small_only) {
    hipLaunchKernelGGL(k_items, dim3(B), dim3(256), 0, WS.stream, RPB, dS, WS.items.as<ItemDesc>());
    DBG(c, "k_items");
    }
    if (sumA > 0 && !D.small_only) {
        const bool needTiled = D.allow_fallback || TCc < Lneed;
        int degGiven = 0;
        for (int tiled = 0; tiled < (needTiled ? 2 : 1); ++tiled) {
            const void* kc = nullptr;
#define ROMAN_KC(GM_) kc = tiled ? (NRc == 2 ? reinterpret_cast<const void*>(k_count<GM_, 2, true>) : reinterpret_cast<const void*>(k_count<GM_, 1, true>)) \
                                 : (NRc == 2 ? reinterpret_cast<const void*>(k_count<GM_, 2, false>) : reinterpret_cast<const void*>(k_count<GM_, 1, false>))
            switch (D.gmode) { case 1: ROMAN_KC(1); break; case 2: ROMAN_KC(2); break; case 3: ROMAN_KC(3); break; default: ROMAN_KC(0); break; }
#undef ROMAN_KC
            const bool usePre = !tiled && preNR > 0;
            if (usePre) {
#define ROMAN_KP(GM_) kc = reinterpret_cast<const void*>(k_count<GM_, 1, false, true>)
                switch (D.gmode) { case 1: ROMAN_KP(1); break; case 2: ROMAN_KP(2); break; case 3: ROMAN_KP(3); break; default: ROMAN_KP(0); break; }
#undef ROMAN_KP
            }
            const size_t ldsK = usePre ? preLds : pairLds;
            const int wpbK = usePre ? preWpb : wpb;
            const int gridK = usePre ? c->num_cu * std::max(1, std::min(2048 / (wpbK * 64), (int)(c->lds_max / ldsK))) : pairGrid;
            const char* wholeEnv = getenv("ROMAN_COUNT_WHOLE");
            const bool wholeP = usePre && (wholeEnv ? wholeEnv[0] != '0' : B >= c->num_cu) && preLds + (size_t)preTC * 4 <= c->lds_max;
            if (wholeP) degGiven = 1;
            HIPCHK(c, dyn_lds(c, kc, ldsK + (wholeP ? (size_t)preTC * 4 : 0)));
            DevParams a_D = D; const ProbDesc* a_dP = dP; const ProbState* a_dS = dS; const BatchTotals* a_dT = dT; const ItemDesc* a_items = WS.items.as<ItemDesc>();
            const double* a_tab = WS.tabPool.as<double>(); const int32_t* a_li = LP.li; const int32_t* a_lj = LP.lj; const double* a_za = LP.lza; const double* a_zb = LP.lzb;
            uint32_t* a_rc = WS.rowCnt.as<uint32_t>(); unsigned long long* a_mask = WS.maskPool.as<unsigned long long>(); uint32_t* a_pref = WS.prefPool.as<uint32_t>();
            int a_TC = usePre ? preTC : TCc, a_lpw = usePre ? preRow : ldsPerWave;
            int a_RPB = wholeP ? -B : RPB;
            const uint16_t* a_qtab = WS.qtabPool.as<uint16_t>();
            void* args[] = {&a_D, &a_dP, &a_dS, &a_dT, &a_items, &a_tab, &a_li, &a_lj, &a_za, &a_zb, &a_rc, &a_mask, &a_pref, &a_TC, &a_lpw, &a_RPB, &a_qtab};
            HIPCHK(c, hipLaunchKernel(kc, dim3(gridK), dim3(wpbK * 64), args, ldsK + (wholeP ? (size_t)preTC * 4 : 0), WS.stream));
        }
    DBG(c, "k_count");
        const char* listsEnv = getenv("ROMAN_LISTS");
        const int fusedLists = listsEnv ? (listsEnv[0] == '0' ? 0 : 1) : (B >= std::max(8, c->num_cu / 8) ? 1 : 0);
        if (fusedLists) {
            static size_t listsStatic = 0;
            if (listsStatic == 0) {
                hipFuncAttributes fa;
                HIPCHK(c, hipFuncGetAttributes(&fa, reinterpret_cast<const void*>(k_lists)));
                listsStatic = std::max<size_t>(fa.sharedSizeBytes, 1);
            }
            const char* llEnv = getenv("ROMAN_LISTS_LDS");
            const size_t room = c->lds_max > listsStatic ? c->lds_max - listsStatic : 0;
            const size_t winBytes = std::min(room, llEnv ? (size_t)std::max(0, atoi(llEnv)) : room) & ~(size_t)15;
            if (winBytes) HIPCHK(c, dyn_lds(c, reinterpret_cast<const void*>(k_lists), winBytes));
            hipLaunchKernelGGL(k_lists, dim3((unsigned)std::max(1, std::min(B, 2 * c->num_cu))), dim3(LISTS_NT), winBytes, WS.stream, B, dP, dS, dT,
                               WS.maskPool.as<unsigned long long>(), WS.listPool.as<uint16_t>(), WS.listOff.as<uint32_t>(),
                               WS.rowCnt.as<uint32_t>(), WS.perm.as<uint32_t>(), WS.rowPos.as<uint32_t>(), LP, PP, (long long)SZ.capList, sort_eq_max(), degGiven,
                               (int)(winBytes / sizeof(uint16_t)));
    DBG(c, "k_lists");
        }
        if (!fusedLists || D.allow_fallback) {
        {
            const int Wexp = (expL + 63) / 64;
            const int tasks = ((Wexp + 7) / 8) * ((std::max(Wexp - 1, 1) + 7) / 8);
            const int T = std::max(tasks, 1);
            hipLaunchKernelGGL(k_mirror, dim3((unsigned)(T * ((B + 7) / 8) * 8)), dim3(512), 0, WS.stream, B, T, dS, WS.maskPool.as<unsigned long long>(), fusedLists);
    DBG(c, "k_mirror");
        }
        hipLaunchKernelGGL(k_rowprefix, dim3(c->num_cu * 2), dim3(1024), 0, WS.stream, dP, dS, dT, WS.items.as<ItemDesc>(),
                           WS.maskPool.as<unsigned long long>(), WS.prefPool.as<uint32_t>(), WS.rowCnt.as<uint32_t>(), RPB, fusedLists);
    DBG(c, "k_rowprefix");
        int sortThr = 1024;
        if (!D.allow_fallback) { int N2 = 64; while (N2 < expL) N2 <<= 1; sortThr = std::max(64, std::min(1024, N2 / 2)); }
        hipLaunchKernelGGL(k_rowsort, dim3(B), dim3(sortThr), 0, WS.stream, dP, dS, dT, WS.rowCnt.as<uint32_t>(), WS.rowPos.as<uint32_t>(), WS.perm.as<uint32_t>(),
                           WS.sliceWidth.as<uint32_t>(), WS.sliceBase.as<uint32_t>(), WS.listOff.as<uint32_t>(), SZ.capList, fusedLists, sort_eq_max());
    DBG(c, "k_rowsort");
        if (!fusedLists) {
        const int upThr = expL <= 256 ? 256 : 1024;
        hipLaunchKernelGGL(k_upper, dim3(c->num_cu * 2 * (1024 / upThr)), dim3(upThr), 0, WS.stream, dP, dS, dT, WS.items.as<ItemDesc>(),
                           WS.maskPool.as<unsigned long long>(), WS.listPool.as<uint16_t>(), WS.listOff.as<uint32_t>(),
                           WS.rowCnt.as<uint32_t>(), WS.perm.as<uint32_t>(), WS.rowPos.as<uint32_t>(), LP, PP, RPB);
    DBG(c, "k_upper");
        }
        }
        hipLaunchKernelGGL(k_slicegeom, dim3(B), dim3(64), 0, WS.stream, dP, dS, WS.rowCnt.as<uint32_t>(), WS.sliceWidth.as<uint32_t>(), WS.sliceBase.as<uint32_t>());
    DBG(c, "k_slicegeom");
    }
    int NG = (int)std::max<int64_t>(1, std::min<int64_t>(FILLS_MAXSPI, (3 * (int64_t)c->num_cu + B / 2) / std::max(B, 1)));
    {
        const int stride = std::max(1, (c->num_cu & ~7) / 8);
        auto gcd = [](int a, int b) { while (b) { const int t = a % b; a = b; b = t; } return a; };
        while (NG > 1 && gcd(stride % NG, NG) != 1) --NG;
    }
    const int Wmax = std::max(1, D.stream_maxL / 64);
    const int SPI = (Wmax + std::min(NG, Wmax) - 1) / std::min(NG, Wmax);
    if (!D.small_only) {
    hipLaunchKernelGGL(k_probscan, dim3(1), dim3(B > 256 ? 1024 : 256), 0, WS.stream, B, NG, SZ.capNnz, dS, dT);
    DBG(c, "k_probscan");
    }
    t1.stop();

    StageTimer t2(c, ROMAN_STAGE_FILL);
    if (sumA > 0 && !D.small_only) {
        const int colBytesF = D.gravity ? 32 : 16;
        const int TCs = D.stream_maxL;
        const int NO = (std::max(maxN, 1) + 1) & ~1;
        const size_t groupLds = sizeof(uint32_t) * (size_t)(3 * SPI * 64 + 2 * (SPI + 1) + 2);
        const bool obj = (size_t)TCs * (16 + 2) + (size_t)64 * NO + groupLds <= c->lds_max;
        const size_t sliceLds = obj ? (size_t)TCs * (16 + 2) + (size_t)64 * NO + groupLds : (size_t)TCs * (colBytesF + 2) + groupLds;
        if (sliceLds > c->lds_max) return fail(c, ROMAN_E_TOO_LARGE, "internal: stream column tile does not fit the LDS");
        const bool fast = D.single && (D.p.single_mode == ROMAN_SINGLE_BOTH || D.p.single_mode == ROMAN_SINGLE_OFFDIAG) && D.p.distance_weight == 1.0 &&
                          D.p.fusion_method != ROMAN_FUSE_ARITHMETIC_MEAN && D.p.fusion_method != ROMAN_FUSE_PRODUCT;
        auto kf = D.gravity ? (fast ? k_fill_list<true, true, false> : k_fill_list<true, false, false>) : (fast ? k_fill_list<false, true, false> : k_fill_list<false, false, false>);
        if (obj) kf = D.gravity ? (fast ? k_fill_list<true, true, true> : k_fill_list<true, false, true>) : (fast ? k_fill_list<false, true, true> : k_fill_list<false, false, true>);
        HIPCHK(c, dyn_lds(c, reinterpret_cast<const void*>(kf), sliceLds));
        const int fillThr = expL <= 256 ? 256 : 1024;
        const int fillWgs = std::max(1, std::min(1024 / fillThr, (int)(c->lds_max / sliceLds)));
        hipLaunchKernelGGL(kf, dim3((unsigned)((c->num_cu & ~7) * fillWgs)), dim3(fillThr), sliceLds, WS.stream,
                           D, B, dP, dS, dT, WS.tabPool.as<double>(), in.feats, NO, LP.li, LP.lj, LP.ls, LP.lza, LP.lzb,
                           WS.listPool.as<uint16_t>(), WS.listOff.as<uint32_t>(), WS.rowCnt.as<uint32_t>(), WS.perm.as<uint32_t>(), WS.rowPos.as<uint32_t>(),
                           WS.sliceWidth.as<uint32_t>(), WS.sliceBase.as<uint32_t>(), WS.cols16.as<uint16_t>(), WS.vals.as<double>(), TCs, NG, SPI);
    DBG(c, "k_fill_list");
        if (D.allow_fallback && (SZ.maxA > D.stream_maxL || D.p.maxiniters < 1 || D.p.maxlsiters < 1)) {
            const int colBytesG = D.gravity ? 40 : 24;
            const size_t ringLds = (size_t)16 * 3 * FILL_Q * sizeof(uint32_t) + (size_t)FILL_RPB * FILL_ROWBYTES;
            static_assert(FILL_RPB >= 128, "the work items of a batch are blocks of at most 128 rows");
            int TCf = (int)std::min<size_t>((c->lds_max - ringLds) / colBytesG, 32768) & ~63;
            TCf = std::min(TCf, std::max(64, (Lneed + 63) & ~63));
            const size_t fillLds = ringLds + (size_t)TCf * colBytesG;
            const int fillGrid = c->num_cu * std::max(1, std::min(2, (int)(c->lds_max / fillLds)));
            if (D.idx16) {
                auto kg = D.gravity ? k_fill<true, uint16_t, true> : k_fill<false, uint16_t, true>;
                HIPCHK(c, dyn_lds(c, reinterpret_cast<const void*>(kg), fillLds));
                hipLaunchKernelGGL(kg, dim3(fillGrid), dim3(1024), fillLds, WS.stream, D, dP, dS, dT, WS.items.as<ItemDesc>(), WS.tabPool.as<double>(),
                                   LP.li, LP.lj, LP.ls, LP.lza, LP.lzb,
                                   WS.rowCnt.as<uint32_t>(), WS.maskPool.as<unsigned long long>(), WS.prefPool.as<uint32_t>(), WS.rowPos.as<uint32_t>(),
                                   WS.sliceWidth.as<uint32_t>(), WS.sliceBase.as<uint32_t>(), WS.cols16.as<uint16_t>(), WS.vals.as<double>(), TCf, RPB, (const uint32_t*)WS.perm.as<uint32_t>());
            } else {
                auto kg = D.gravity ? k_fill<true, uint32_t, true> : k_fill<false, uint32_t, true>;
                HIPCHK(c, dyn_lds(c, reinterpret_cast<const void*>(kg), fillLds));
                hipLaunchKernelGGL(kg, dim3(fillGrid), dim3(1024), fillLds, WS.stream, D, dP, dS, dT, WS.items.as<ItemDesc>(), WS.tabPool.as<double>(),
                                   LP.li, LP.lj, LP.ls, LP.lza, LP.lzb,
                                   WS.rowCnt.as<uint32_t>(), WS.maskPool.as<unsigned long long>(), WS.prefPool.as<uint32_t>(), WS.rowPos.as<uint32_t>(),
                                   WS.sliceWidth.as<uint32_t>(), WS.sliceBase.as<uint32_t>(), WS.cols32.as<uint32_t>(), WS.vals.as<double>(), TCf, RPB, (const uint32_t*)WS.perm.as<uint32_t>());
            }
    DBG(c, "k_fill");
        }
    }
    t2.stop();
    HIPCHK(c, hipMemcpyAsync(WS.pinnedTotals, dT, sizeof(BatchTotals), hipMemcpyDeviceToHost, WS.stream));
    HIPCHK(c, hipEventRecord(WS.totEvent, WS.stream));
    WS.totPending = true; WS.totMaskBound = SZ.maskBound; WS.totSumA = SZ.sumA; WS.totMaxA = SZ.maxA; WS.totEpoch = c->histEpoch;
    HIPCHK(c, hipGetLastError());
    return ROMAN_OK;
}

int enqueue_solve(roman_ctx* c, const DevParams& D, int B, int64_t sumA, int64_t maxA , const double* feats, const int32_t* assoc,
                  const double* u0, bool hascz, int mayFallback , const BatchOut& out)
{
    const size_t R1 = (size_t)std::max<int64_t>(sumA, 1);
    SolveOut O;
    { int rc_ = make_solve_out(c, B, sumA, out, &O); if (rc_) return rc_; }
#ifdef ROMAN_SOLVE_TIMING
    HIPCHK(c, WS.hAux3.ensure(sizeof(unsigned long long) * 16 * (size_t)B));
    HIPCHK(c, hipMemsetAsync(WS.hAux3.p, 0, sizeof(unsigned long long) * 16 * (size_t)B, WS.stream));
    O.dbg = WS.hAux3.as<unsigned long long>();
#endif
    constexpr int NW = SOLVE_WAVES;
    const int Lc = STREAM_MAXL + 64;
    const size_t ldsUp = (size_t)3 * 8 * Lc + sizeof(double) * red_doubles(NW) + sizeof(uint32_t) * (ST_MAXSL + 2) + sizeof(int) * 8 + 16;
    const int wgPerCu = std::max(1, std::min((int)(c->lds_max / ldsUp), 2048 / (NW * 64)));
    const int gridUp = std::max(1, std::min(B, c->num_cu * wgPerCu));

    StageTimer t3(c, ROMAN_STAGE_SOLVE);
    const bool coopPlanned = mayFallback && D.wide != 0 && c->coop_ok;
    if (coopPlanned) {
        HIPCHK(c, WS.wideBar.ensure(sizeof(unsigned) * WIDE_BAR_WORDS));
        HIPCHK(c, WS.fbList.ensure(sizeof(int32_t) * (size_t)B));
        HIPCHK(c, hipMemsetAsync(WS.wideBar.p, 0, sizeof(unsigned) * WIDE_BAR_WORDS, WS.stream));
    }
    hipLaunchKernelGGL(k_skipped, dim3((unsigned)((B + 255) / 256)), dim3(256), 0, WS.stream, B, WS.probs.as<ProbDesc>(), WS.state.as<ProbState>(), O, WS.queue.as<int>(),
                       coopPlanned ? WS.fbList.as<int32_t>() : (int32_t*)nullptr, coopPlanned ? WS.wideBar.as<unsigned>() : (unsigned*)nullptr);
    DBG(c, "k_skipped");
    if (D.small_only) { t3.stop(); HIPCHK(c, hipGetLastError()); return ROMAN_OK; }
    static const char* smallEnv = getenv("ROMAN_SMALL");
    const bool small = !(smallEnv && smallEnv[0] == '0') && D.p.maxiniters >= 1 && D.p.maxlsiters >= 1 &&
                       (c->hist.valid ? c->hist.smallSeen : maxA <= 16 * SMALL_MAXL);
    const int Lc1 = SMALL_MAXL + 64;
    const size_t ldsUp1 = (size_t)3 * 8 * Lc1 + sizeof(double) * red_doubles(1) + sizeof(uint32_t) * (ST_MAXSL + 2) + sizeof(int) * 8 + 16 + (size_t)COO_CAP * 12;
    const int gridUp1 = std::max(1, std::min(B, c->num_cu * 24));
#define ROMAN_LAUNCH_UP(CZ_)                                                                                                  \
    do {                                                                                                                      \
        auto kup = k_solve_up<NW, CZ_, STREAM_MAXL>;                                                                          \
        HIPCHK(c, dyn_lds(c, reinterpret_cast<const void*>(kup), ldsUp)); \
        hipLaunchKernelGGL(kup, dim3(gridUp), dim3(NW * 64), ldsUp, WS.stream, D, B, WS.probs.as<ProbDesc>(), WS.state.as<ProbState>(), feats, assoc, \
                           WS.plp.as<int32_t>(), WS.lp.as<int32_t>(), WS.rowPos.as<uint32_t>(), WS.pld.as<double>(), WS.sliceBase.as<uint32_t>(), \
                           WS.cols16.as<uint16_t>(), WS.vals.as<double>(), u0, O, WS.queue.as<int>(), Lc, small ? SMALL_MAXL + 1 : 0, STREAM_MAXL, (small && c->hist.valid && !c->hist.largeSeen) ? 64 : 1); \
        if (small) {                                                                                                          \
            HIPCHK(c, dyn_lds(c, reinterpret_cast<const void*>(k_solve_up<1, CZ_, SMALL_MAXL>), ldsUp1));                       \
            hipLaunchKernelGGL((k_solve_up<1, CZ_, SMALL_MAXL>), dim3(gridUp1), dim3(64), ldsUp1, WS.stream, D, B, WS.probs.as<ProbDesc>(), WS.state.as<ProbState>(), feats, assoc, \
                               WS.plp.as<int32_t>(), WS.lp.as<int32_t>(), WS.rowPos.as<uint32_t>(), WS.pld.as<double>(), WS.sliceBase.as<uint32_t>(), \
                               WS.cols16.as<uint16_t>(), WS.vals.as<double>(), u0, O, WS.queue.as<int>() + 1, Lc1, 0, SMALL_MAXL, 1); \
        }                                                                                                                     \
    } while (0)
    if (hascz) ROMAN_LAUNCH_UP(true); else ROMAN_LAUNCH_UP(false);
#undef ROMAN_LAUNCH_UP
    DBG(c, "k_solve_up");
    if (mayFallback) {
        HIPCHK(c, WS.vMu.ensure(sizeof(double) * R1)); HIPCHK(c, WS.vCu.ensure(sizeof(double) * R1));
        HIPCHK(c, WS.vMun.ensure(sizeof(double) * R1)); HIPCHK(c, WS.vCun.ensure(sizeof(double) * R1));
        HIPCHK(c, WS.gU.ensure(sizeof(double) * R1)); HIPCHK(c, WS.gUn.ensure(sizeof(double) * R1));
        bool coop = D.wide != 0 && c->coop_ok;
        if (coop) {
            const int G = c->num_cu;
            int a_teams = 0;
            const int perXcd = std::max(1, (G + c->num_xcc - 1) / c->num_xcc);
            {
                constexpr int margin = 2;
                auto cap = [&](int sub) { return (int64_t)WIDE_KW * std::max(1, perXcd / sub - margin) * WIDE_NW * 64; };
                if (mayFallback >= 2 && maxA <= cap(1)) {
                    a_teams = 1;
                    for (int s_ = 2; s_ <= 4; ++s_) if (mayFallback > 6 * s_ && maxA <= cap(s_)) a_teams = s_;
                    if (a_teams == 2 && mayFallback > 18 && G == c->num_cu && maxA <= (int64_t)WIDE_KW * (perXcd / 3) * WIDE_NW * 64) a_teams = 3;
                }
                const char* teamEnv = getenv("ROMAN_WIDE_TEAMS");
                const int forced = teamEnv ? atoi(teamEnv) : c->wide_teams;
                if (teamEnv || c->wide_teams >= 0) a_teams = (forced >= 1 && forced <= 4 && mayFallback >= 1 && maxA <= cap(forced)) ? forced : 0;
            }
            if (a_teams) c->teams_launched = true;
            const int nTeams = a_teams ? 8 * a_teams : 1;
            const int NWGt = a_teams ? std::min(G, 2 * ((perXcd + a_teams - 1) / a_teams) + 8) * WIDE_NW : G * WIDE_NW;
            int a_ucfg = (D.idx16 && a_teams > 0 && maxA >= 8000) ? 1 : 0;
            { const char* e_ = getenv("ROMAN_WIDE_UPPER"); if (e_ && e_[0]) a_ucfg = (D.idx16 && e_[0] != '0') ? 1 : 0; }
            long long a_partStride = (long long)(((size_t)NWGt * WIDE_MAXCH + (size_t)(a_ucfg ? WIDE_MAXBLK : 1) * ((size_t)(maxA + 63) / 64) + 4) * 64 * 2);
            HIPCHK(c, WS.widePart.ensure(sizeof(double) * (size_t)a_partStride * (size_t)nTeams));
            HIPCHK(c, WS.wideSlots.ensure(sizeof(double) * 2 * (size_t)G * WIDE_NRED * (size_t)nTeams));
            DevParams Dv = D; int Bv = B;
            const ProbDesc* a_probs = WS.probs.as<ProbDesc>(); ProbState* a_state = WS.state.as<ProbState>();
            const double* a_feats = feats; const int32_t* a_assoc = assoc;
            const int32_t* a_lp = WS.lp.as<int32_t>(); const double* a_ld = WS.ld.as<double>();
            const uint32_t* a_perm = WS.perm.as<uint32_t>(); const uint32_t* a_rpos = WS.rowPos.as<uint32_t>(); const uint32_t* a_sb = WS.sliceBase.as<uint32_t>();
            const void* a_cols = D.idx16 ? (const void*)WS.cols16.as<uint16_t>() : (const void*)WS.cols32.as<uint32_t>(); const double* a_vals = WS.vals.as<double>();
            double* a_vU = WS.gU.as<double>(); double* a_vX = WS.gUn.as<double>(); double* a_vX2 = WS.vCun.as<double>();
            double* a_s0 = WS.vMu.as<double>(); double* a_s1 = WS.vCu.as<double>(); double* a_s2 = WS.vMun.as<double>();
            int32_t* a_plp = WS.plp.as<int32_t>();
            const double* a_u0 = u0; SolveOut a_O = O;
            double* a_part = WS.widePart.as<double>(); double* a_slots = WS.wideSlots.as<double>(); unsigned* a_bar = WS.wideBar.as<unsigned>();
            int a_bmw = (int)((maxA + 63) / 64) + 1;
            HIPCHK(c, WS.wideBm.ensure(sizeof(unsigned long long) * 3 * (size_t)a_bmw * (size_t)nTeams));
            unsigned long long* a_bm = WS.wideBm.as<unsigned long long>();
            const int64_t wideFixed = (int64_t)wide_fixed_lds(a_bmw);
            int a_xcap = (int)(((int64_t)c->lds_max - 4096 - wideFixed) / (int64_t)sizeof(double)) & ~63;
            if (a_xcap < 0) a_xcap = 0;
            const size_t wideLds = sizeof(double) * (size_t)a_xcap + (size_t)wideFixed;
            int a_ccfg = 6 | (128 << 8) | (4 << 16);
            { const char* e_ = getenv("ROMAN_WIDE_COMPACT"); if (e_ && e_[0]) a_ccfg = (int)strtol(e_, nullptr, 0); }
            int a_ySlots = NWGt / WIDE_NW;
            int a_ycap = a_ucfg ? ((a_xcap / 3) & ~63) : 0;
            if (a_ucfg && a_ycap < 64) a_ucfg = 0;
            if (a_ucfg) {
                HIPCHK(c, WS.wideY.ensure(sizeof(unsigned long long) * 2 * (size_t)a_ycap * (size_t)a_ySlots * (size_t)nTeams));
                HIPCHK(c, WS.wideUp.ensure(sizeof(uint32_t) * 1800 * (size_t)a_bmw * (size_t)nTeams));
            }
            unsigned long long* a_yPart = WS.wideY.as<unsigned long long>(); uint32_t* a_upMeta = WS.wideUp.as<uint32_t>();
            if ((a_ccfg & 0xff) || a_ucfg) {
                HIPCHK(c, WS.valsC.ensure(sizeof(double) * (size_t)WS.capNnz));
                HIPCHK(c, WS.colsC.ensure((D.idx16 ? sizeof(uint16_t) : sizeof(uint32_t)) * (size_t)WS.capNnz));
            }
            void* a_colsC = WS.colsC.p; double* a_valsC = WS.valsC.as<double>();
            const void* wideFn = D.idx16 ? (a_ucfg ? reinterpret_cast<const void*>(k_solve_wide<uint16_t, true>) : reinterpret_cast<const void*>(k_solve_wide<uint16_t, false>))
                                         : reinterpret_cast<const void*>(k_solve_wide<uint32_t, false>);
            HIPCHK(c, dyn_lds(c, wideFn, wideLds));
            unsigned long long a_ticks = c->spin_ticks;
            const int32_t* a_fb = WS.fbList.as<int32_t>();
            void* args[] = {&Dv, &Bv, &a_probs, &a_state, &a_feats, &a_assoc, &a_lp, &a_ld, &a_perm, &a_rpos, &a_sb, &a_cols, &a_vals,
                            &a_vU, &a_vX, &a_vX2, &a_s0, &a_s1, &a_s2, &a_plp, &a_u0, &a_O, &a_part, &a_slots, &a_bar, &a_bm, &a_bmw, &a_xcap, &a_ticks,
                            &a_teams, &a_fb, &a_partStride, &a_colsC, &a_valsC, &a_ccfg, &a_ucfg, &a_yPart, &a_ySlots, &a_ycap, &a_upMeta};
            if (!c->coopDone) HIPCHK(c, hipEventCreateWithFlags(&c->coopDone, hipEventDisableTiming));
            if (c->coopIssued) HIPCHK(c, hipStreamWaitEvent(WS.stream, c->coopDone, 0));
            const hipError_t e = hipLaunchCooperativeKernel(wideFn, dim3((unsigned)G), dim3(WIDE_NT), args, wideLds, WS.stream);
            if (e == hipSuccess) { HIPCHK(c, hipEventRecord(c->coopDone, WS.stream)); c->coopIssued = true; }
            if (e != hipSuccess) {
                (void)hipGetLastError();
                fprintf(stderr, "[roman_hip] cooperative launch failed (%s); large problems use the single-workgroup solver\n", hipGetErrorString(e));
                c->coop_ok = false; coop = false;
                if (D.idx16) return fail(c, ROMAN_E_HIP, "cooperative launch of the large-problem solver failed (%s); run the call again (it now takes the single-workgroup solver)", hipGetErrorString(e));
            }
    DBG(c, "k_solve_wide");
        }
        if (!coop) {
        const size_t fixed = 72 * sizeof(double) + 4 * sizeof(int);
        const int Lcap = (int)(((c->lds_max - fixed) / (2 * sizeof(double))) & ~(size_t)1);
        const size_t lds = (size_t)2 * sizeof(double) * (size_t)Lcap + fixed;
        const int grid = std::max(1, std::min(B, c->num_cu));
        HIPCHK(c, dyn_lds(c, reinterpret_cast<const void*>(k_solve<uint32_t, 1>), lds));
        hipLaunchKernelGGL((k_solve<uint32_t, 1>), dim3(grid), dim3(1024), lds, WS.stream, D, B, WS.probs.as<ProbDesc>(), WS.state.as<ProbState>(), feats, assoc,
                           WS.lp.as<int32_t>(), WS.ld.as<double>(), WS.perm.as<uint32_t>(), WS.rowPos.as<uint32_t>(), WS.sliceWidth.as<uint32_t>(), WS.sliceBase.as<uint32_t>(), WS.cols32.as<uint32_t>(), WS.vals.as<double>(),
                           WS.vMu.as<double>(), WS.vCu.as<double>(), WS.vMun.as<double>(), WS.vCun.as<double>(), WS.gU.as<double>(), WS.gUn.as<double>(),
                           WS.plp.as<int32_t>(), WS.pld.as<double>(), u0, O, WS.queue.as<int>() + 4, Lcap);
        }
    DBG(c, "k_solve");
    }
    t3.stop();
    HIPCHK(c, hipGetLastError());
#ifdef ROMAN_SOLVE_TIMING
    {
        std::vector<unsigned long long> h((size_t)B * 16);
        HIPCHK(c, hipMemcpyAsync(h.data(), WS.hAux3.p, sizeof(unsigned long long) * 16 * (size_t)B, hipMemcpyDeviceToHost, WS.stream));
        HIPCHK(c, hipStreamSynchronize(WS.stream));
        double acc[16] = {0};
        for (int b = 0; b < B; ++b) for (int t = 0; t < 16; ++t) acc[t] += (double)h[(size_t)b * 16 + t];
        const char* nm[8] = {"stream", "spmv-barrier", "decode", "elementwise", "stream-narrow", "setup+tail", "publish", "red-sums"};
        fprintf(stderr, "[solve timing] B=%d cycles/problem:", B);
        double tot_ = 0; for (int t = 0; t < 8; ++t) tot_ += acc[t] / B;
        for (int t = 0; t < 8; ++t) fprintf(stderr, " %s %.0f (n=%.1f)", nm[t], acc[t] / B, acc[8 + t] / B);
        fprintf(stderr, " total %.0f\n", tot_);
        if (B > 1) {
            std::vector<std::pair<double, int>> tt;
            for (int b = 0; b < B; ++b) { double t_ = 0; for (int t = 0; t < 8; ++t) t_ += (double)h[(size_t)b * 16 + t]; tt.push_back({t_, b}); }
            std::sort(tt.begin(), tt.end());
            for (int r = 0; r < 3; ++r) {
                const int b = tt[(size_t)(B - 1 - r)].second;
                fprintf(stderr, "   slow #%d (b=%d, %.0f cyc):", r, b, tt[(size_t)(B - 1 - r)].first);
                for (int t = 0; t < 8; ++t) fprintf(stderr, " %s %.0f (n=%.0f)", nm[t], (double)h[(size_t)b * 16 + t], (double)h[(size_t)b * 16 + 8 + t]);
                fprintf(stderr, "\n");
            }
            fprintf(stderr, "   median problem: %.0f cyc\n", tt[(size_t)B / 2].first);
        }
    }
#endif
    return ROMAN_OK;
}

int may_fallback(const DevParams& D, const std::vector<ProbDesc>& hd)
{
    if (!D.allow_fallback) return 0;
    if (D.p.maxiniters < 1 || D.p.maxlsiters < 1) return (int)hd.size();
    int n = 0;
    for (const ProbDesc& d : hd) if (d.nA > D.stream_maxL) ++n;
    return n;
}

int ensure_events(roman_ctx* c)
{
    for (int k = 0; k < ROMAN_MAX_PIPELINE; ++k)
        for (int s = 0; s < ROMAN_STAGE_COUNT; ++s) {
            if (!c->ws[k].evA[s]) HIPCHK(c, hipEventCreate(&c->ws[k].evA[s]));
            if (!c->ws[k].evB[s]) HIPCHK(c, hipEventCreate(&c->ws[k].evB[s]));
        }
    return ROMAN_OK;
}

int run_batch(roman_ctx* c, const DevParams& D0, const roman_params_t* params, const BatchIn& in, const double* u0, const BatchOut& out)
{
// ... 1788 lines not shown
        return fail(nullptr, ROMAN_E_INVALID, "bad arguments");
    std::vector<int64_t> work((size_t)B);
    for (int b = 0; b < B; ++b) {
        int64_t a = assoc_off ? assoc_off[b + 1] - assoc_off[b] : 0;
        if (a <= 0) a = (int64_t)n1[b] * n2[b];
        work[(size_t)b] = a * a;
    }
    std::vector<int32_t> order((size_t)B);
    for (int b = 0; b < B; ++b) order[(size_t)b] = b;
    std::stable_sort(order.begin(), order.end(), [&](int32_t x, int32_t y) { return work[(size_t)x] > work[(size_t)y]; });
    std::vector<int64_t> load((size_t)world, 0), count((size_t)world, 0);
    std::vector<int32_t> mine;
    for (int32_t b : order) {
        int r = 0;
        for (int t = 1; t < world; ++t)
            if (load[(size_t)t] < load[(size_t)r] || (load[(size_t)t] == load[(size_t)r] && count[(size_t)t] < count[(size_t)r])) r = t;
        load[(size_t)r] += std::max<int64_t>(work[(size_t)b], 1); count[(size_t)r] += 1;
        if (r == rank) mine.push_back(b);
    }
    std::sort(mine.begin(), mine.end());
    for (size_t t = 0; t < mine.size(); ++t) idx_out[t] = mine[t];
    *n_out = (int32_t)mine.size();
    return ROMAN_OK;
}

int roman_create_all_to_all(int32_t n1, int32_t n2, int32_t* out)
{
    if (n1 < 0 || n2 < 0 || (!out && (int64_t)n1 * n2 > 0)) return fail(nullptr, ROMAN_E_INVALID, "bad arguments");
    for (int32_t i = 0; i < n1; ++i) for (int32_t j = 0; j < n2; ++j) { out[2 * ((int64_t)i * n2 + j)] = i; out[2 * ((int64_t)i * n2 + j) + 1] = j; }
    return ROMAN_OK;
}

int roman_score(roman_ctx_t* c, const roman_params_t* params, const double* D1, int32_t n1,
                const double* D2, int32_t n2, int32_t F, const int32_t* assoc, int32_t n_assoc)
{
    if (!c) return fail(nullptr, ROMAN_E_INVALID, "ctx is NULL");
    if (n1 < 0 || n2 < 0 || F < 0 || (assoc && n_assoc < 0)) return fail(c, ROMAN_E_INVALID, "negative size");
    if ((n1 > 0 && !D1) || (n2 > 0 && !D2)) return fail(c, ROMAN_E_INVALID, "NULL feature matrix");
    HIPCHK(c, hipSetDevice(c->device));
    { int rc0 = use_ws0(c); if (rc0) return rc0; }
    roman_ctx::Last& Lst = c->last;
    Lst.scored = false; Lst.solved = false; Lst.dense = false; Lst.hascz = false;
    DevParams D0;
    int rc = make_dev_params(c, params, F, &D0);
    if (rc) return rc;
    const int64_t nobj = (int64_t)n1 + n2;
    HIPCHK(c, WS.hFeats.ensure(sizeof(double) * (size_t)std::max<int64_t>(nobj * F, 1)));
    if ((int64_t)n1 * F > 0) HIPCHK(c, hipMemcpyAsync(WS.hFeats.p, D1, sizeof(double) * (size_t)n1 * F, hipMemcpyHostToDevice, WS.stream));
    if ((int64_t)n2 * F > 0) HIPCHK(c, hipMemcpyAsync(WS.hFeats.as<double>() + (size_t)n1 * F, D2, sizeof(double) * (size_t)n2 * F, hipMemcpyHostToDevice, WS.stream));
    const int32_t* dA = nullptr;
    if (assoc && n_assoc == 0) assoc = nullptr;
    int64_t aoff[2] = {0, n_assoc};
    Lst.assoc.clear();
    if (assoc) {
        for (int32_t k = 0; k < n_assoc; ++k)
            if (assoc[2 * k] < 0 || assoc[2 * k] >= n1 || assoc[2 * k + 1] < 0 || assoc[2 * k + 1] >= n2)
                return fail(c, ROMAN_E_INVALID, "association %d = (%d,%d) out of range", k, assoc[2 * k], assoc[2 * k + 1]);
        Lst.assoc.assign(assoc, assoc + 2 * (size_t)n_assoc);
        HIPCHK(c, WS.hAssoc.ensure(sizeof(int32_t) * 2 * (size_t)std::max(n_assoc, 1)));
        if (n_assoc > 0) HIPCHK(c, hipMemcpyAsync(WS.hAssoc.p, assoc, sizeof(int32_t) * 2 * (size_t)n_assoc, hipMemcpyHostToDevice, WS.stream));
        dA = WS.hAssoc.as<int32_t>();
    }
    const int64_t o1 = 0, o2 = n1;
    const BatchIn in{1, WS.hFeats.as<double>(), &o1, &n1, &o2, &n2, F, dA, aoff};
    std::vector<ProbDesc> hd;
    ProbState ps{};
    for (int attempt = 0; ; ++attempt) {
        rc = enqueue_score(c, D0, params, in, hd, &Lst.D);
        if (rc) return rc;
        HIPCHK(c, hipMemcpyAsync(&ps, WS.state.p, sizeof(ProbState), hipMemcpyDeviceToHost, WS.stream));
        HIPCHK(c, hipStreamSynchronize(WS.stream));
        if (!batch_overflowed(c)) break;
        if (attempt + 1 >= MAX_ATTEMPTS) return fail(c, ROMAN_E_NOMEM, "the sparse workspace still does not fit after %d attempts", attempt + 1);
    }
    Lst.pd = hd[0]; Lst.nA = hd[0].nA; Lst.L = ps.L; Lst.kind = ps.kind; Lst.nnzCap = ps.nnzCap; Lst.scored = true;
    return ROMAN_OK;
}

int roman_set_matrix_data(roman_ctx_t* c, const roman_params_t* params, const double* M, const double* Cm, int32_t n)
{
    if (!c) return fail(nullptr, ROMAN_E_INVALID, "ctx is NULL");
    if (n < 0 || (n > 0 && (!M || !Cm))) return fail(c, ROMAN_E_INVALID, "bad matrix arguments");
    HIPCHK(c, hipSetDevice(c->device));
    { int rc0 = use_ws0(c); if (rc0) return rc0; }
    roman_ctx::Last& Lst = c->last;
    Lst.scored = false; Lst.solved = false; Lst.dense = true; Lst.assoc.clear();
    roman_params_t p = *params; p.invariant = ROMAN_INV_EUCLIDEAN;
    int rc = make_dev_params(c, &p, p.point_dim, &Lst.D);
    if (rc) return rc;
    const size_t n1_ = (size_t)std::max(n, 1);
    HIPCHK(c, WS.hAux1.ensure(sizeof(double) * n1_ * n1_)); HIPCHK(c, WS.hAux2.ensure(sizeof(double) * n1_ * n1_)); HIPCHK(c, WS.hAux3.ensure(sizeof(int) * 4));
    HIPCHK(c, hipMemsetAsync(WS.hAux3.p, 0, sizeof(int) * 4, WS.stream));
    int rangeFlag = 0;
    if (n > 0) {
        HIPCHK(c, hipMemcpyAsync(WS.hAux1.p, M, sizeof(double) * n1_ * n1_, hipMemcpyHostToDevice, WS.stream));
        HIPCHK(c, hipMemcpyAsync(WS.hAux2.p, Cm, sizeof(double) * n1_ * n1_, hipMemcpyHostToDevice, WS.stream));
        hipLaunchKernelGGL(k_dense_range, dim3((unsigned)std::min(c->num_cu * 8, (n + 3) / 4)), dim3(256), 0, WS.stream, n, WS.hAux1.as<double>(), WS.hAux3.as<int>());
        HIPCHK(c, hipGetLastError());
        HIPCHK(c, hipMemcpyAsync(&rangeFlag, WS.hAux3.as<int>() + 1, sizeof(int), hipMemcpyDeviceToHost, WS.stream));
        HIPCHK(c, hipStreamSynchronize(WS.stream));
    }
    const bool iter = Lst.D.p.maxiniters >= 1 && Lst.D.p.maxlsiters >= 1;
    const bool up = n <= STREAM_MAXL && iter && rangeFlag == 0;
    Lst.D.wide = (!up && n > STREAM_MAXL && c->coop_ok && iter && n <= (int64_t)WIDE_KW * c->num_cu * WIDE_NW * 64) ? 1 : 0;
    Lst.D.idx16 = 0;
    Lst.D.stream_maxL = up ? std::max(64, (n + 63) & ~63) : 64;
    const int W = (n + 63) / 64;
    const int RPB = 128;
    const size_t maskWords = std::max<size_t>((size_t)n * (size_t)W, 1);
    const long long capList = up ? (long long)n * (n - 1) / 2 + 4LL * n + 4 : 4;
    HIPCHK(c, WS.probs.ensure(sizeof(ProbDesc))); HIPCHK(c, WS.state.ensure(sizeof(ProbState))); HIPCHK(c, WS.totals.ensure(sizeof(BatchTotals)));
    HIPCHK(c, WS.queue.ensure(sizeof(int) * 16));
    {
        DevBuf* i32s[] = {&WS.lp, &WS.plp, &WS.rowCnt, &WS.rowPos, &WS.perm, &WS.sliceWidth, &WS.sliceBase, &WS.listOff};
        for (DevBuf* b_ : i32s) HIPCHK(c, b_->ensure(sizeof(int32_t) * n1_));
        DevBuf* f64s[] = {&WS.ls, &WS.ld, &WS.pld};
        for (DevBuf* b_ : f64s) HIPCHK(c, b_->ensure(sizeof(double) * n1_));
    }
    HIPCHK(c, WS.maskPool.ensure(sizeof(unsigned long long) * maskWords)); HIPCHK(c, WS.prefPool.ensure(sizeof(uint32_t) * maskWords));
    HIPCHK(c, WS.listPool.ensure(sizeof(uint16_t) * (size_t)capList));
    HIPCHK(c, WS.items.ensure(sizeof(ItemDesc) * ((size_t)n / RPB + 2)));
    WS.capMaskWords = std::max<long long>(WS.capMaskWords, (long long)maskWords); WS.capList = std::max<long long>(WS.capList, capList);
    ProbDesc pd{}; pd.off1 = 0; pd.off2 = 0; pd.assocOff = -1; pd.liveOff = 0; pd.n1 = n; pd.n2 = 1; pd.nA = n;
    ProbState ps{}; ps.L = n; ps.kind = up ? 0 : 1;
    HIPCHK(c, hipMemcpyAsync(WS.probs.p, &pd, sizeof(pd), hipMemcpyHostToDevice, WS.stream));
    HIPCHK(c, hipMemcpyAsync(WS.state.p, &ps, sizeof(ps), hipMemcpyHostToDevice, WS.stream));
    HIPCHK(c, hipStreamSynchronize(WS.stream));
    const ProbDesc* dP = WS.probs.as<ProbDesc>(); ProbState* dS = WS.state.as<ProbState>(); BatchTotals* dT = WS.totals.as<BatchTotals>();
    const double* dM = WS.hAux1.as<double>(); const double* dC = WS.hAux2.as<double>();
    if (n > 0) {
        std::vector<int32_t> ident(n1_); std::vector<double> ones(n1_, 1.0);
        for (int k = 0; k < n; ++k) ident[(size_t)k] = k;
        HIPCHK(c, hipMemcpy(WS.lp.p, ident.data(), sizeof(int32_t) * n1_, hipMemcpyHostToDevice));
        HIPCHK(c, hipMemcpy(WS.plp.p, ident.data(), sizeof(int32_t) * n1_, hipMemcpyHostToDevice));
        HIPCHK(c, hipMemcpy(WS.ls.p, ones.data(), sizeof(double) * n1_, hipMemcpyHostToDevice));
        HIPCHK(c, hipMemcpy(WS.ld.p, ones.data(), sizeof(double) * n1_, hipMemcpyHostToDevice));
        HIPCHK(c, hipMemcpy(WS.pld.p, ones.data(), sizeof(double) * n1_, hipMemcpyHostToDevice));
    }
    const LivePools LP{WS.lp.as<int32_t>(), nullptr, nullptr, WS.ls.as<double>(), WS.ld.as<double>(), nullptr, nullptr};
    const LivePools PP{WS.plp.as<int32_t>(), nullptr, nullptr, nullptr, WS.pld.as<double>(), nullptr, nullptr};
    hipLaunchKernelGGL(k_rowbase, dim3(1), dim3(256), 0, WS.stream, 1, RPB, (long long)maskWords, dS, dT, 0, (const int32_t*)nullptr);
    hipLaunchKernelGGL(k_items, dim3(1), dim3(256), 0, WS.stream, RPB, dS, WS.items.as<ItemDesc>());
    if (n > 0) {
        hipLaunchKernelGGL(k_dense_mask, dim3((unsigned)std::min(c->num_cu * 8, (n + 3) / 4)), dim3(256), 0, WS.stream, n, dM, dC,
                           WS.maskPool.as<unsigned long long>(), WS.hAux3.as<int>());
        hipLaunchKernelGGL(k_rowprefix, dim3(c->num_cu * 2), dim3(1024), 0, WS.stream, dP, dS, dT, WS.items.as<ItemDesc>(),
                           WS.maskPool.as<unsigned long long>(), WS.prefPool.as<uint32_t>(), WS.rowCnt.as<uint32_t>(), RPB, 0);
        hipLaunchKernelGGL(k_rowsort, dim3(1), dim3(1024), 0, WS.stream, dP, dS, dT, WS.rowCnt.as<uint32_t>(), WS.rowPos.as<uint32_t>(), WS.perm.as<uint32_t>(),
                           WS.sliceWidth.as<uint32_t>(), WS.sliceBase.as<uint32_t>(), WS.listOff.as<uint32_t>(), capList, 0, sort_eq_max());
        if (up) {
            hipLaunchKernelGGL(k_upper, dim3(c->num_cu * 2), dim3(1024), 0, WS.stream, dP, dS, dT, WS.items.as<ItemDesc>(),
                               WS.maskPool.as<unsigned long long>(), WS.listPool.as<uint16_t>(), WS.listOff.as<uint32_t>(),
                               WS.rowCnt.as<uint32_t>(), WS.perm.as<uint32_t>(), WS.rowPos.as<uint32_t>(), LP, PP, RPB);
            hipLaunchKernelGGL(k_slicegeom, dim3(1), dim3(64), 0, WS.stream, dP, dS, WS.rowCnt.as<uint32_t>(), WS.sliceWidth.as<uint32_t>(), WS.sliceBase.as<uint32_t>());
        }
    }
    HIPCHK(c, hipGetLastError());
    HIPCHK(c, hipMemcpyAsync(&ps, WS.state.p, sizeof(ps), hipMemcpyDeviceToHost, WS.stream));
    HIPCHK(c, hipStreamSynchronize(WS.stream));
    if (ps.kind == 2) return fail(c, ROMAN_E_NOMEM, "internal: dense problem does not fit its own workspace");
    const uint64_t total = ps.nnzCap;
    if (total > 4000000000ull) return fail(c, ROMAN_E_TOO_LARGE, "dense matrix has too many non-zeros");
    const size_t nnz1 = (size_t)std::max<uint64_t>(total, 1);
    HIPCHK(c, WS.vals.ensure(sizeof(double) * nnz1)); HIPCHK(c, WS.cols16.ensure(sizeof(uint16_t) * nnz1)); HIPCHK(c, WS.cols32.ensure(sizeof(uint32_t) * nnz1));
    WS.capNnz = std::max<long long>(WS.capNnz, (long long)nnz1);
    hipLaunchKernelGGL(k_probscan, dim3(1), dim3(256), 0, WS.stream, 1, 1, (long long)nnz1, dS, dT);
    if (total > 0) {
        const unsigned grid = (unsigned)std::min<uint64_t>((total + 255) / 256, (uint64_t)c->num_cu * 16);
        auto kf = up ? k_dense_fill<0> : k_dense_fill<1>;
        hipLaunchKernelGGL(kf, dim3(grid), dim3(256), 0, WS.stream, n, dM, dC, dS, WS.rowCnt.as<uint32_t>(), WS.rowPos.as<uint32_t>(), WS.perm.as<uint32_t>(),
                           WS.sliceWidth.as<uint32_t>(), WS.sliceBase.as<uint32_t>(), WS.listPool.as<uint16_t>(), WS.listOff.as<uint32_t>(),
                           WS.maskPool.as<unsigned long long>(), WS.prefPool.as<uint32_t>(), WS.cols16.as<uint16_t>(), WS.cols32.as<uint32_t>(), WS.vals.as<double>());
    }
    HIPCHK(c, hipGetLastError());
    int flags[4] = {0, 0, 0, 0};
    HIPCHK(c, hipMemcpyAsync(&ps, WS.state.p, sizeof(ps), hipMemcpyDeviceToHost, WS.stream));
    HIPCHK(c, hipMemcpyAsync(flags, WS.hAux3.p, sizeof(flags), hipMemcpyDeviceToHost, WS.stream));
    HIPCHK(c, hipStreamSynchronize(WS.stream));
    if (ps.kind == 2) return fail(c, ROMAN_E_NOMEM, "internal: dense problem does not fit its own workspace");
    Lst.hascz = flags[0] != 0;
    Lst.pd = pd; Lst.nA = n; Lst.L = n; Lst.kind = ps.kind; Lst.nnzCap = (int64_t)total;
    Lst.scored = true;
    return ROMAN_OK;
}

int roman_solve(roman_ctx_t* c, const double* u0)
{
    if (!c) return fail(nullptr, ROMAN_E_INVALID, "ctx is NULL");
    if (!c->last.scored) return fail(c, ROMAN_E_INVALID, "roman_solve: no matrices (call roman_score or roman_set_matrix_data first)");
    HIPCHK(c, hipSetDevice(c->device));
    { int rc0 = use_ws0(c); if (rc0) return rc0; }
    return solve_last(c, u0);
}

int roman_num_associations(const roman_ctx_t* c, int32_t* n)
{
    if (!c || !n) return fail(nullptr, ROMAN_E_INVALID, "NULL argument");
    if (!c->last.scored) return fail(const_cast<roman_ctx*>(c), ROMAN_E_INVALID, "nothing scored yet");
    *n = c->last.nA; return ROMAN_OK;
}
int roman_num_selected(const roman_ctx_t* c, int32_t* n)
{
    if (!c || !n) return fail(nullptr, ROMAN_E_INVALID, "NULL argument");
    if (!c->last.solved) return fail(const_cast<roman_ctx*>(c), ROMAN_E_INVALID, "nothing solved yet");
    *n = c->last.nsel; return ROMAN_OK;
}
int roman_get_selected_associations(const roman_ctx_t* c, int32_t* out)
{
    if (!c) return fail(nullptr, ROMAN_E_INVALID, "ctx is NULL");
    const roman_ctx::Last& L = c->last;
    if (!L.solved) return fail(const_cast<roman_ctx*>(c), ROMAN_E_INVALID, "nothing solved yet");
    for (int32_t t = 0; t < L.nsel; ++t) {
        const int32_t p = L.nodes[(size_t)t];
        if (!L.assoc.empty()) { out[2 * t] = L.assoc[2 * (size_t)p]; out[2 * t + 1] = L.assoc[2 * (size_t)p + 1]; }
        else if (L.dense) { out[2 * t] = p; out[2 * t + 1] = p; }
        else { out[2 * t] = p / L.pd.n2; out[2 * t + 1] = p % L.pd.n2; }
    }
    return ROMAN_OK;
}
int roman_get_solution(const roman_ctx_t* c, int32_t* nodes, double* u, double* score, roman_stats_t* stats)
{
    if (!c) return fail(nullptr, ROMAN_E_INVALID, "ctx is NULL");
    const roman_ctx::Last& L = c->last;
    if (!L.solved) return fail(const_cast<roman_ctx*>(c), ROMAN_E_INVALID, "nothing solved yet");
    if (nodes) for (int32_t t = 0; t < L.nsel; ++t) nodes[t] = L.nodes[(size_t)t];
    if (u) for (int32_t p = 0; p < L.nA; ++p) u[p] = L.u[(size_t)p];
    if (score) *score = L.stats.score;
    if (stats) *stats = L.stats;
    return ROMAN_OK;
}

int roman_get_upper_csr(const roman_ctx_t* c, int64_t* nnz, int64_t* rowptr, int32_t* cols_out, double* vals_out, double* diag)
{
    if (!c) return fail(nullptr, ROMAN_E_INVALID, "ctx is NULL");
    const roman_ctx::Last& Lst = c->last;
    if (!Lst.scored) return fail(const_cast<roman_ctx*>(c), ROMAN_E_INVALID, "nothing scored yet");
    std::vector<uint32_t> rs, rl, cols; std::vector<double> vals, ls; std::vector<int32_t> lp;
    int rc = fetch_last_csr(c, rs, rl, cols, vals, lp, ls);
    if (rc) return rc;
    const int L = Lst.L, nA = Lst.nA;
    int64_t cnt = 0;
    std::vector<int64_t> rp((size_t)nA + 1, 0);
    for (int k = 0; k < L; ++k) {
        int64_t rc_ = 0;
        for (uint32_t e = 0; e < rl[(size_t)k]; ++e) { const uint32_t q = cols[(size_t)rs[(size_t)k] + e] & 0x7fffffffu; if ((int)q > k) ++rc_; }
        rp[(size_t)lp[(size_t)k] + 1] = rc_; cnt += rc_;
    }
    for (int p = 0; p < nA; ++p) rp[(size_t)p + 1] += rp[(size_t)p];
    if (nnz) *nnz = cnt;
    if (rowptr) for (int p = 0; p <= nA; ++p) rowptr[p] = rp[(size_t)p];
    if (cols_out || vals_out) {
        for (int k = 0; k < L; ++k) {
            int64_t w = rp[(size_t)lp[(size_t)k]];
            for (uint32_t e = 0; e < rl[(size_t)k]; ++e) {
                const uint32_t q = cols[(size_t)rs[(size_t)k] + e] & 0x7fffffffu;
                if ((int)q > k) { if (cols_out) cols_out[w] = lp[(size_t)q]; if (vals_out) vals_out[w] = vals[(size_t)rs[(size_t)k] + e]; ++w; }
            }
        }
    }
    if (diag) {
        const bool single = Lst.D.single && !Lst.dense;
        for (int p = 0; p < nA; ++p) diag[p] = single ? 0.0 : 1.0;
        if (single) for (int k = 0; k < L; ++k) diag[(size_t)lp[(size_t)k]] = ls[(size_t)k];
    }
    return ROMAN_OK;
}

int roman_get_dense_matrices(const roman_ctx_t* c, double* M, double* Cm)
{
    if (!c) return fail(nullptr, ROMAN_E_INVALID, "ctx is NULL");
    const roman_ctx::Last& Lst = c->last;
    if (!Lst.scored) return fail(const_cast<roman_ctx*>(c), ROMAN_E_INVALID, "nothing scored yet");
    std::vector<uint32_t> rs, rl, cols; std::vector<double> vals, ls; std::vector<int32_t> lp;
    int rc = fetch_last_csr(c, rs, rl, cols, vals, lp, ls);
    if (rc) return rc;
    const int L = Lst.L; const int64_t nA = Lst.nA;
    if (M) memset(M, 0, sizeof(double) * (size_t)(nA * nA));
    if (Cm) memset(Cm, 0, sizeof(double) * (size_t)(nA * nA));
    const bool single = Lst.D.single && !Lst.dense;
    for (int64_t p = 0; p < nA; ++p) { if (M) M[p * nA + p] = single ? 0.0 : 1.0; if (Cm) Cm[p * nA + p] = 1.0; }
    for (int k = 0; k < L; ++k) {
        const int64_t p = lp[(size_t)k];
        if (single && M) M[p * nA + p] = ls[(size_t)k];
        for (uint32_t e = 0; e < rl[(size_t)k]; ++e) {
            const uint32_t cq = cols[(size_t)rs[(size_t)k] + e];
            const int64_t q = lp[(size_t)(cq & 0x7fffffffu)];
            if (M) M[p * nA + q] = vals[(size_t)rs[(size_t)k] + e];
            if (Cm) Cm[p * nA + q] = (cq & 0x80000000u) ? 0.0 : 1.0;
        }
    }
    return ROMAN_OK;
}

int roman_pose_batch(roman_ctx_t* c, int32_t dim, int32_t B, const double* pts1, const double* pts2,
                     const int64_t* corr_off, double* T_out, int32_t* status_out)
{
    if (!c) return fail(nullptr, ROMAN_E_INVALID, "ctx is NULL");
    if (dim != 2 && dim != 3) return fail(c, ROMAN_E_INVALID, "dim must be 2 or 3");
    if (B < 0 || !corr_off || !T_out || !status_out) return fail(c, ROMAN_E_INVALID, "bad arguments");
    if (B == 0) return ROMAN_OK;
    HIPCHK(c, hipSetDevice(c->device));
    { int rc0 = use_ws0(c); if (rc0) return rc0; }
    const int64_t K = corr_off[B];
    if (K < 0 || (K > 0 && (!pts1 || !pts2))) return fail(c, ROMAN_E_INVALID, "bad correspondence arrays");
    HIPCHK(c, WS.hAux1.ensure(sizeof(double) * (size_t)std::max<int64_t>(K * dim, 1)));
    HIPCHK(c, WS.hAux2.ensure(sizeof(double) * (size_t)std::max<int64_t>(K * dim, 1)));
    HIPCHK(c, WS.hAux3.ensure(sizeof(int64_t) * ((size_t)B + 1)));
    HIPCHK(c, WS.oT.ensure(sizeof(double) * 16 * (size_t)B)); HIPCHK(c, WS.oStatus.ensure(sizeof(int32_t) * (size_t)B));
    if (K > 0) {
        HIPCHK(c, hipMemcpyAsync(WS.hAux1.p, pts1, sizeof(double) * (size_t)(K * dim), hipMemcpyHostToDevice, WS.stream));
        HIPCHK(c, hipMemcpyAsync(WS.hAux2.p, pts2, sizeof(double) * (size_t)(K * dim), hipMemcpyHostToDevice, WS.stream));
    }
    HIPCHK(c, hipMemcpyAsync(WS.hAux3.p, corr_off, sizeof(int64_t) * ((size_t)B + 1), hipMemcpyHostToDevice, WS.stream));
    hipLaunchKernelGGL(k_pose, dim3(B), dim3(64), 0, WS.stream, dim, WS.hAux1.as<double>(), WS.hAux2.as<double>(), WS.hAux3.as<int64_t>(),
                       WS.oT.as<double>(), WS.oStatus.as<int32_t>());
    HIPCHK(c, hipGetLastError());
    HIPCHK(c, hipMemcpyAsync(T_out, WS.oT.p, sizeof(double) * 16 * (size_t)B, hipMemcpyDeviceToHost, WS.stream));
    HIPCHK(c, hipMemcpyAsync(status_out, WS.oStatus.p, sizeof(int32_t) * (size_t)B, hipMemcpyDeviceToHost, WS.stream));
    HIPCHK(c, hipStreamSynchronize(WS.stream));
    return ROMAN_OK;
}

int roman_debug_math(roman_ctx_t* c, int kind, const double* in1, const double* in2, int64_t n, double* out)
{
    if (!c) return fail(nullptr, ROMAN_E_INVALID, "ctx is NULL");
    if (n < 0 || (n > 0 && (!in1 || !out))) return fail(c, ROMAN_E_INVALID, "bad arguments");
    if (n == 0) return ROMAN_OK;
    HIPCHK(c, hipSetDevice(c->device));
    { int rc0 = use_ws0(c); if (rc0) return rc0; }
    HIPCHK(c, WS.hAux1.ensure(sizeof(double) * (size_t)n)); HIPCHK(c, WS.hAux2.ensure(sizeof(double) * (size_t)n)); HIPCHK(c, WS.hAux3.ensure(sizeof(double) * (size_t)n));
    HIPCHK(c, hipMemcpyAsync(WS.hAux1.p, in1, sizeof(double) * (size_t)n, hipMemcpyHostToDevice, WS.stream));
    if (in2) HIPCHK(c, hipMemcpyAsync(WS.hAux2.p, in2, sizeof(double) * (size_t)n, hipMemcpyHostToDevice, WS.stream));
    hipLaunchKernelGGL(k_debug_math, dim3((unsigned)((n + 255) / 256)), dim3(256), 0, WS.stream, kind, WS.hAux1.as<double>(),
                       in2 ? WS.hAux2.as<double>() : (const double*)nullptr, n, WS.hAux3.as<double>());
    HIPCHK(c, hipGetLastError());
    HIPCHK(c, hipMemcpyAsync(out, WS.hAux3.p, sizeof(double) * (size_t)n, hipMemcpyDeviceToHost, WS.stream));
    HIPCHK(c, hipStreamSynchronize(WS.stream));
    return ROMAN_OK;
}

int roman_debug_cosine(roman_ctx_t* c, const roman_params_t* params, const double* D1, int32_t n1,
                       const double* D2, int32_t n2, int32_t F, double* out)
{
    if (!c) return fail(nullptr, ROMAN_E_INVALID, "ctx is NULL");
    if (n1 <= 0 || n2 <= 0 || !D1 || !D2 || !out) return fail(c, ROMAN_E_INVALID, "bad arguments");
    HIPCHK(c, hipSetDevice(c->device));
    { int rc0 = use_ws0(c); if (rc0) return rc0; }
    DevParams D;
    int rc = make_dev_params(c, params, F, &D);
    if (rc) return rc;
    if (D.p.cos_feature_dim <= 0) return fail(c, ROMAN_E_INVALID, "cos_feature_dim is 0");
    HIPCHK(c, WS.hFeats.ensure(sizeof(double) * (size_t)(n1 + n2) * F));
    HIPCHK(c, hipMemcpyAsync(WS.hFeats.p, D1, sizeof(double) * (size_t)n1 * F, hipMemcpyHostToDevice, WS.stream));
    HIPCHK(c, hipMemcpyAsync(WS.hFeats.as<double>() + (size_t)n1 * F, D2, sizeof(double) * (size_t)n2 * F, hipMemcpyHostToDevice, WS.stream));
    ProbDesc pd{}; pd.off1 = 0; pd.off2 = n1; pd.assocOff = -1; pd.n1 = n1; pd.n2 = n2; pd.nA = n1 * n2;
    HIPCHK(c, WS.probs.ensure(sizeof(ProbDesc)));
    HIPCHK(c, WS.cosPool.ensure(sizeof(double) * (size_t)n1 * n2));
    HIPCHK(c, hipMemcpyAsync(WS.probs.p, &pd, sizeof(pd), hipMemcpyHostToDevice, WS.stream));
    const char* selEnv = getenv("ROMAN_COS_SEL");
    if (selEnv && (!strcmp(selEnv, "approx") || !strcmp(selEnv, "gated")) && n1 <= CSEL_MAXN && n2 <= CSEL_MAXN) {
        HIPCHK(c, WS.cosDense.ensure(sizeof(int32_t)));
        HIPCHK(c, launch_cos_sel(c, WS.stream, D, 1, n1, n2, WS.probs.as<ProbDesc>(), WS.hFeats.as<double>(), WS.cosPool.as<double>(), WS.cosDense.as<int32_t>(), selEnv[0] == 'a'));
    } else
    HIPCHK(c, launch_cos(c, WS.stream, D, 1, n1, n2, WS.probs.as<ProbDesc>(), WS.hFeats.as<double>(), WS.cosPool.as<double>()));
    HIPCHK(c, hipMemcpyAsync(out, WS.cosPool.p, sizeof(double) * (size_t)n1 * n2, hipMemcpyDeviceToHost, WS.stream));
    HIPCHK(c, hipStreamSynchronize(WS.stream));
    c->last.scored = false; c->last.solved = false;
    return ROMAN_OK;
}

int roman_debug_live(const roman_ctx_t* cc, int32_t* n_live, int32_t* idx, double* score)
{
    if (!cc) return fail(nullptr, ROMAN_E_INVALID, "ctx is NULL");
    roman_ctx* c = const_cast<roman_ctx*>(cc);
    if (!c->last.scored) return fail(c, ROMAN_E_INVALID, "nothing scored yet");
    const int L = c->last.L;
    if (n_live) *n_live = L;
    HIPCHK(c, hipSetDevice(c->device));
    if (idx && L > 0) HIPCHK(c, hipMemcpy(idx, WS.lp.p, sizeof(int32_t) * (size_t)L, hipMemcpyDeviceToHost));
    if (score && L > 0) HIPCHK(c, hipMemcpy(score, WS.ls.p, sizeof(double) * (size_t)L, hipMemcpyDeviceToHost));
    return ROMAN_OK;
}

}
```

roman_amd/runtime.py:

```python
import ctypes as C
from dataclasses import dataclass
from typing import Optional

import numpy as np

from . import _abi
from ._abi import RomanHipError, RomanLcParams, RomanParams, RomanStats


def _ptr(a):
    return None if a is None else C.c_void_p(a.ctypes.data)


def _f64(a):
    return np.ascontiguousarray(a, dtype=np.float64)


def _vp(x):
    return C.c_void_p(int(x)) if x else None


def _given(a, shape, dtype, fill):
    if a is None:
        return np.full(shape, fill, dtype=dtype)
# ... 620 lines not shown
        return res()

    def align_lc_batch_ids(self, params, feats, ids, off1, n1, off2, n2, lc, assoc=None, assoc_off=None, u0=None, kmax=None, want_keep=True):
        feats = _f64(feats)
        if feats.ndim != 2:
            raise ValueError("feats must be (n_objects, F)")
        n_obj, F = feats.shape
        ids = np.ascontiguousarray(ids, dtype=np.int64).reshape(-1)
        if ids.shape[0] != n_obj:
            raise ValueError("ids must hold one entry per row of feats")
        off1 = np.ascontiguousarray(off1, dtype=np.int64); off2 = np.ascontiguousarray(off2, dtype=np.int64)
        n1 = np.ascontiguousarray(n1, dtype=np.int32); n2 = np.ascontiguousarray(n2, dtype=np.int32)
        B = int(n1.shape[0])
        if assoc is not None:
            assoc = np.ascontiguousarray(assoc, dtype=np.int32).reshape(-1, 2)
            assoc_off = np.ascontiguousarray(assoc_off, dtype=np.int64)
        if u0 is not None:
            u0 = _f64(u0)
        if kmax is None:
            kmax = int(max(1, np.max(np.minimum(n1, n2)))) if B else 1
        a_out = np.zeros((B, kmax, 2), dtype=np.int32); n_out = np.zeros(B, dtype=np.int32)
        T = np.zeros((B, 16), dtype=np.float64); status = np.zeros(B, dtype=np.int32); stats = np.zeros(B, dtype=stats_dtype())
        records = np.zeros(B, dtype=lc_record_dtype()); idx = np.zeros(max(B, 1), dtype=np.int32); cnt = np.zeros(1, dtype=np.int32)
        k1 = np.zeros(B, dtype=np.int32); k2 = np.zeros(B, dtype=np.int32)
        keep = np.full(int(n1.sum(dtype=np.int64) + n2.sum(dtype=np.int64)), -1, dtype=np.int32) if want_keep else None
        lp = lc.params()
        T_ref, enable, FL, iL, FR, iR = lc.arrays(B)
        self._generation += 1
        rc = self._lib.roman_align_lc_batch_ids(self._h, C.byref(params), B, _ptr(feats), n_obj, _ptr(off1), _ptr(n1), _ptr(off2), _ptr(n2), F,
                                                _ptr(assoc), _ptr(assoc_off), _ptr(u0), kmax, _ptr(a_out), _ptr(n_out), _ptr(T), _ptr(status), _ptr(stats),
                                                C.byref(lp), _ptr(T_ref), _ptr(enable), _ptr(FL), 0 if FL is None else FL.shape[0], _ptr(iL),
                                                _ptr(FR), 0 if FR is None else FR.shape[0], _ptr(iR), _ptr(records), _ptr(idx), _ptr(cnt),
                                                _ptr(ids), _ptr(k1), _ptr(k2), _ptr(keep))
        s = params.point_dim + 1
        res = lambda: LoopClosureResult([a_out[b, :n_out[b]].copy() for b in range(B)], T[:, :s * s].reshape(B, s, s).copy(), status, stats,
                                        records, idx[:int(cnt[0])].copy(), k1, k2, keep)
        if rc == _abi.ROMAN_E_INTERNAL:
            msg = self._lib.roman_last_error(self._h)
            err = RomanHipError(f"roman_align_lc_batch_ids failed ({rc}): {msg.decode() if msg else ''}")
            err.result = res()
            raise err
        self._check(rc, "roman_align_lc_batch_ids")
        return res()

    def shared_ids_dev(self, B, ids_ptr, off1, n1, off2, n2, keep_ptr, kept_ptr):
        off1 = np.ascontiguousarray(off1, dtype=np.int64); off2 = np.ascontiguousarray(off2, dtype=np.int64)
        n1 = np.ascontiguousarray(n1, dtype=np.int32); n2 = np.ascontiguousarray(n2, dtype=np.int32)
        rc = self._lib.roman_shared_ids_dev(self._h, int(B), _vp(ids_ptr), _ptr(off1), _ptr(n1), _ptr(off2), _ptr(n2), _vp(keep_ptr), _vp(kept_ptr))
        self._check(rc, "roman_shared_ids_dev")

    def shared_reduce_dev(self, B, F, feats_ptr, region_row0, ids_ptr, off1, n1, off2, n2, keep_ptr, kept_ptr):
        off1 = np.ascontiguousarray(off1, dtype=np.int64); off2 = np.ascontiguousarray(off2, dtype=np.int64)
        n1 = np.ascontiguousarray(n1, dtype=np.int32); n2 = np.ascontiguousarray(n2, dtype=np.int32)
        rc = self._lib.roman_shared_reduce_dev(self._h, int(B), int(F), _vp(feats_ptr), int(region_row0), _vp(ids_ptr), _ptr(off1), _ptr(n1),
                                               _ptr(off2), _ptr(n2), _vp(keep_ptr), _vp(kept_ptr))
        self._check(rc, "roman_shared_reduce_dev")

    def lc_tail_dev(self, lc_params, B, T_ptr, n_assoc_ptr, status_ptr, records_ptr, accepted_idx_ptr, n_accepted_ptr,
                    T_ref_ptr=None, enable_ptr=None, FL_ptr=None, iL_ptr=None, FR_ptr=None, iR_ptr=None):
        rc = self._lib.roman_lc_tail_dev(self._h, C.byref(lc_params), int(B), _vp(T_ptr), _vp(n_assoc_ptr), _vp(status_ptr), _vp(T_ref_ptr), _vp(enable_ptr),
                                         _vp(FL_ptr), _vp(iL_ptr), _vp(FR_ptr), _vp(iR_ptr), _vp(records_ptr), _vp(accepted_idx_ptr), _vp(n_accepted_ptr))
        self._check(rc, "roman_lc_tail_dev")

    def align_lc_batch_dev(self, params, feats_ptr, F, off1, n1, off2, n2, kmax, assoc_out_ptr, n_assoc_out_ptr, T_out_ptr, status_out_ptr,
                           lc_params, records_ptr, accepted_idx_ptr, n_accepted_ptr, stats_out_ptr=None, assoc_ptr=None, assoc_off=None, u0_ptr=None,
                           T_ref_ptr=None, enable_ptr=None, FL_ptr=None, iL_ptr=None, FR_ptr=None, iR_ptr=None):
        off1 = np.ascontiguousarray(off1, dtype=np.int64); off2 = np.ascontiguousarray(off2, dtype=np.int64)
        n1 = np.ascontiguousarray(n1, dtype=np.int32); n2 = np.ascontiguousarray(n2, dtype=np.int32)
        if assoc_off is not None:
            assoc_off = np.ascontiguousarray(assoc_off, dtype=np.int64)
        self._generation += 1
        rc = self._lib.roman_align_lc_batch_dev(self._h, C.byref(params), int(n1.shape[0]), _vp(feats_ptr), _ptr(off1), _ptr(n1), _ptr(off2), _ptr(n2),
                                                int(F), _vp(assoc_ptr), _ptr(assoc_off), _vp(u0_ptr), int(kmax), _vp(assoc_out_ptr), _vp(n_assoc_out_ptr),
                                                _vp(T_out_ptr), _vp(status_out_ptr), _vp(stats_out_ptr), C.byref(lc_params), _vp(T_ref_ptr), _vp(enable_ptr),
                                                _vp(FL_ptr), _vp(iL_ptr), _vp(FR_ptr), _vp(iR_ptr), _vp(records_ptr), _vp(accepted_idx_ptr), _vp(n_accepted_ptr))
        self._check(rc, "roman_align_lc_batch_dev")

    def score(self, params, D1, D2, assoc=None):
        D1, D2 = _f64(D1), _f64(D2)
        n1, n2 = D1.shape[0], D2.shape[0]
        F = D1.shape[1] if D1.ndim == 2 else 0
        if D2.ndim == 2 and D2.shape[1] != F and n1 > 0 and n2 > 0:
            raise ValueError("D1 and D2 must have the same number of features")
        if n1 == 0 and D2.ndim == 2:
            F = D2.shape[1]
        na = 0
        if assoc is not None:
            assoc = np.ascontiguousarray(assoc, dtype=np.int32).reshape(-1, 2)
            na = assoc.shape[0]
        self._generation += 1
        rc = self._lib.roman_score(self._h, C.byref(params), _ptr(D1), n1, _ptr(D2), n2, F, _ptr(assoc), na)
        self._check(rc, "roman_score")

    def set_matrix_data(self, params, M, Cm):
        M, Cm = _f64(M), _f64(Cm)
        if M.shape != Cm.shape or M.ndim != 2 or M.shape[0] != M.shape[1]:
            raise ValueError("M and C must be square matrices of the same shape")
        self._generation += 1
        self._check(self._lib.roman_set_matrix_data(self._h, C.byref(params), _ptr(M), _ptr(Cm), M.shape[0]),
                    "roman_set_matrix_data")

    def solve(self, u0=None):
        u0a = None if u0 is None else _f64(u0)
        self._check(self._lib.roman_solve(self._h, _ptr(u0a)), "roman_solve")

    def num_associations(self):
        n = C.c_int32(0)
        self._check(self._lib.roman_num_associations(self._h, C.byref(n)), "roman_num_associations")
        return n.value

    def selected_associations(self):
        n = C.c_int32(0)
        self._check(self._lib.roman_num_selected(self._h, C.byref(n)), "roman_num_selected")
        out = np.zeros((max(n.value, 1), 2), dtype=np.int32)
        self._check(self._lib.roman_get_selected_associations(self._h, _ptr(out)), "roman_get_selected_associations")
        return out[:n.value].copy()

    def solution(self):
        n = C.c_int32(0); na = C.c_int32(0)
        self._check(self._lib.roman_num_selected(self._h, C.byref(n)), "roman_num_selected")
        self._check(self._lib.roman_num_associations(self._h, C.byref(na)), "roman_num_associations")
        nodes = np.zeros(max(n.value, 1), dtype=np.int32)
        u = np.zeros(max(na.value, 1), dtype=np.float64)
        score = C.c_double(0.0); st = RomanStats()
        self._check(self._lib.roman_get_solution(self._h, _ptr(nodes), _ptr(u), C.byref(score), C.byref(st)),
                    "roman_get_solution")
        return nodes[:n.value].copy(), u[:na.value].copy(), score.value, st

    def dense_matrices(self):
        na = self.num_associations()
        M = np.zeros((na, na), dtype=np.float64); Cm = np.zeros((na, na), dtype=np.float64)
        if na > 0:
            self._check(self._lib.roman_get_dense_matrices(self._h, _ptr(M), _ptr(Cm)), "roman_get_dense_matrices")
        return M, Cm

    def upper_csr(self):
        na = self.num_associations()
        nnz = C.c_int64(0)
        self._check(self._lib.roman_get_upper_csr(self._h, C.byref(nnz), None, None, None, None), "roman_get_upper_csr")
        rowptr = np.zeros(na + 1, dtype=np.int64)
        cols = np.zeros(max(nnz.value, 1), dtype=np.int32); vals = np.zeros(max(nnz.value, 1), dtype=np.float64)
        diag = np.zeros(max(na, 1), dtype=np.float64)
        self._check(self._lib.roman_get_upper_csr(self._h, C.byref(nnz), _ptr(rowptr), _ptr(cols), _ptr(vals), _ptr(diag)),
                    "roman_get_upper_csr")
        return rowptr, cols[:nnz.value].copy(), vals[:nnz.value].copy(), diag[:na].copy()

    def live(self):
        n = C.c_int32(0)
        self._check(self._lib.roman_debug_live(self._h, C.byref(n), None, None), "roman_debug_live")
        idx = np.zeros(max(n.value, 1), dtype=np.int32); sc = np.zeros(max(n.value, 1), dtype=np.float64)
        self._check(self._lib.roman_debug_live(self._h, C.byref(n), _ptr(idx), _ptr(sc)), "roman_debug_live")
        return idx[:n.value].copy(), sc[:n.value].copy()

    def pose_batch(self, dim, pts1, pts2, corr_off):
        pts1 = _f64(pts1).reshape(-1, dim); pts2 = _f64(pts2).reshape(-1, dim)
        corr_off = np.ascontiguousarray(corr_off, dtype=np.int64)
        B = corr_off.shape[0] - 1
        T = np.zeros((max(B, 1), 16), dtype=np.float64); status = np.zeros(max(B, 1), dtype=np.int32)
        self._check(self._lib.roman_pose_batch(self._h, int(dim), B, _ptr(pts1), _ptr(pts2), _ptr(corr_off), _ptr(T),
                                               _ptr(status)), "roman_pose_batch")
        s = dim + 1
        return T[:B, :s * s].reshape(B, s, s).copy(), status[:B].copy()

    def profile_enable(self, on=True):
        self._check(self._lib.roman_profile_enable(self._h, int(bool(on))), "roman_profile_enable")

    def profile_reset(self):
        self._check(self._lib.roman_profile_reset(self._h), "roman_profile_reset")

    def profile_get(self):
        ms = (C.c_double * _abi.ROMAN_STAGE_COUNT)(); n = (C.c_int64 * _abi.ROMAN_STAGE_COUNT)()
        self._check(self._lib.roman_profile_get(self._h, ms, n), "roman_profile_get")
        return {name: (ms[i], n[i]) for i, name in enumerate(_abi.STAGE_NAMES)}

    def debug_math(self, kind, x, y=None):
        x = _f64(x).ravel(); ya = None if y is None else _f64(y).ravel()
        out = np.zeros_like(x)
        self._check(self._lib.roman_debug_math(self._h, int(kind), _ptr(x), _ptr(ya), x.size, _ptr(out)), "roman_debug_math")
        return out

    def debug_cosine(self, params, D1, D2):
        D1, D2 = _f64(D1), _f64(D2)
        out = np.zeros((D1.shape[0], D2.shape[0]), dtype=np.float64)
        self._generation += 1
        self._check(self._lib.roman_debug_cosine(self._h, C.byref(params), _ptr(D1), D1.shape[0], _ptr(D2), D2.shape[0],
                                                 D1.shape[1], _ptr(out)), "roman_debug_cosine")
        return out


    def cosine_matrix(self, A, B):
        A, B = _f64(A), _f64(B)
        if A.ndim != 2 or B.ndim != 2 or A.shape[1] != B.shape[1]:
            raise ValueError("cosine_matrix needs two (n, d) matrices of the same d")
        P = _abi.RomanParams.default()
        P.cos_feature_dim = A.shape[1]
        pad = lambda M: np.ascontiguousarray(np.hstack([np.zeros((M.shape[0], P.point_dim)), M]))
        if A.shape[0] == 0 or B.shape[0] == 0:
            return np.zeros((A.shape[0], B.shape[0]))
        return self.debug_cosine(P, pad(A), pad(B))


_DEFAULT_CTX = None


def default_context():
    global _DEFAULT_CTX
    if _DEFAULT_CTX is None:
        _DEFAULT_CTX = Context(0)
    return _DEFAULT_CTX


def version():
    return _abi.load_library().roman_version().decode()
```

Measured before the change: 178,800 alignments/s.

## Sort rows by degree within slices and mask padded SpMV lanes in solve

k_slicegeom now reorders rows within each 64-row slice by descending nonzero count, permuting perm, rowPos, listOff, rowCnt and the live arrays, so slice widths are tighter. The multi-wave solve kernel keeps a per-row quad count in LDS and tracks the current slice while streaming. Lanes past their row's real length load a fixed address and skip the atomic pushes, which cuts redundant memory traffic and LDS atomics on padding. In exchange it adds LDS use per workgroup, extra per-quad slice-tracking logic, and a larger slicegeom launch. A debug API for reading row positions is also added.

```diff
diff --git a/include/roman_hip.h b/include/roman_hip.h
--- a/include/roman_hip.h
+++ b/include/roman_hip.h
@@ -459,6 +459,7 @@
                        const double* D1, int32_t n1, const double* D2, int32_t n2, int32_t F,
                        double* out);
 ROMAN_API int roman_debug_live(const roman_ctx_t* ctx, int32_t* n_live, int32_t* idx, double* score);
+ROMAN_API int roman_debug_positions(const roman_ctx_t* ctx, int32_t* n_live, int32_t* pos, int32_t* upper);
 
 ROMAN_API const char* roman_version(void);
 
diff --git a/roman_amd/_abi.py b/roman_amd/_abi.py
--- a/roman_amd/_abi.py
+++ b/roman_amd/_abi.py
@@ -351,6 +351,7 @@
         "roman_debug_math": (C.c_int, [ctxp, C.c_int, vp, vp, i64, vp]),
         "roman_debug_cosine": (C.c_int, [ctxp, P(RomanParams), vp, i32, vp, i32, i32, vp]),
         "roman_debug_live": (C.c_int, [ctxp, P(i32), vp, vp]),
+        "roman_debug_positions": (C.c_int, [ctxp, P(i32), vp, vp]),
         "roman_version": (C.c_char_p, []),
     }
     for name, (res, args) in protos.items():
@@ -369,6 +370,6 @@
     "roman_set_matrix_data", "roman_solve", "roman_num_associations", "roman_num_selected",
     "roman_get_selected_associations", "roman_get_solution", "roman_get_dense_matrices",
     "roman_get_upper_csr", "roman_pose_batch", "roman_profile_enable", "roman_profile_reset",
-    "roman_profile_get", "roman_debug_math", "roman_debug_cosine", "roman_debug_live",
+    "roman_profile_get", "roman_debug_math", "roman_debug_cosine", "roman_debug_live", "roman_debug_positions",
     "roman_version",
 )
diff --git a/roman_amd/csrc/kernels.hip.h b/roman_amd/csrc/kernels.hip.h
--- a/roman_amd/csrc/kernels.hip.h
+++ b/roman_amd/csrc/kernels.hip.h
@@ -2463,26 +2463,46 @@
     }
 }
 
-__global__ void __launch_bounds__(64) k_slicegeom(const ProbDesc* __restrict__ probs, ProbState* __restrict__ st,
-                                                  const uint32_t* __restrict__ rowCnt,
-                                                  uint32_t* __restrict__ sliceWidth, uint32_t* __restrict__ sliceBase)
-{
-    const int b = blockIdx.x, lane = threadIdx.x;
+__global__ void __launch_bounds__(1024) k_slicegeom(const ProbDesc* __restrict__ probs, ProbState* __restrict__ st,
+                                                    uint32_t* __restrict__ rowCnt, uint32_t* __restrict__ perm, uint32_t* __restrict__ rowPos,
+                                                    uint32_t* __restrict__ listOff, int32_t* __restrict__ plp, double* __restrict__ pld,
+                                                    uint32_t* __restrict__ sliceWidth, uint32_t* __restrict__ sliceBase)
+{
+    __shared__ uint32_t widthS[64];
+    const int b = blockIdx.x, tid = threadIdx.x, lane = tid & 63, w = tid >> 6, nw = blockDim.x >> 6;
     if (st[b].kind != 0) return;
     const int L = st[b].L;
     const int64_t lo = probs[b].liveOff;
     const int nsl = (L + 63) >> 6;
-    uint32_t width = 0;
-    if (lane < nsl) {
-        const int hi = min(L, (lane << 6) + 64);
-        for (int p = lane << 6; p < hi; ++p) width = max(width, rowCnt[lo + p]);
-        width = (width + 3u) & ~3u;
-        sliceWidth[lo + lane] = width;
-    }
-    const uint32_t v = width * 64u;
-    const uint32_t ex = wave_excl_scan(v, lane);
-    if (lane < nsl) sliceBase[lo + lane] = ex;
-    if (lane == WAVE - 1) st[b].nnzCap = ex + v;
+    for (int s = w; s < nsl; s += nw) {
+        const int r = (s << 6) + lane;
+        const bool row = r < L;
+        const int cnt = row ? (int)rowCnt[lo + r] : -1;
+        uint32_t k = 0u, off = 0u; int32_t ap = 0; double dg = 0.0;
+        if (row) { k = perm[lo + r]; off = listOff[lo + r]; ap = plp[lo + r]; dg = pld[lo + r]; }
+        int at = 0;
+        for (int j = 0; j < WAVE; ++j) {
+            const int cj = __builtin_amdgcn_readlane(cnt, j);
+            at += (cj > cnt || (cj == cnt && j < lane)) ? 1 : 0;
+        }
+        int mx = cnt;
+        for (int o = 32; o > 0; o >>= 1) mx = max(mx, __shfl_xor(mx, o));
+        if (row) {
+            const int p = (s << 6) + at;
+            perm[lo + p] = k; rowPos[lo + k] = (uint32_t)p; listOff[lo + p] = off; rowCnt[lo + p] = (uint32_t)cnt;
+            plp[lo + p] = ap; pld[lo + p] = dg;
+        }
+        if (lane == 0) widthS[s] = ((uint32_t)max(mx, 0) + 3u) & ~3u;
+    }
+    __syncthreads();
+    if (w == 0) {
+        const uint32_t width = lane < nsl ? widthS[lane] : 0u;
+        if (lane < nsl) sliceWidth[lo + lane] = width;
+        const uint32_t v = width * 64u;
+        const uint32_t ex = wave_excl_scan(v, lane);
+        if (lane < nsl) sliceBase[lo + lane] = ex;
+        if (lane == WAVE - 1) st[b].nnzCap = ex + v;
+    }
 }
 
 __global__ void __launch_bounds__(1024) k_probscan(int B, int NG , long long capNnz, ProbState* __restrict__ st, BatchTotals* __restrict__ tot)
@@ -3803,6 +3823,7 @@
                          const double* __restrict__ u0, const SolveOut& O,
                          double* xg , unsigned long long* accM , unsigned long long* accC , int Lc,
                          uint32_t* cumQ , double* red, int* sint, unsigned char* cooLds ,
+                         const uint32_t* __restrict__ rowCntPool = nullptr , uint16_t* nqS = nullptr ,
                          int cooPre = -1 ,
                          int rbPre = -1 )
 {
@@ -3815,6 +3836,7 @@
 #endif
     constexpr int KMAX = (MAXL + NT - 1) / NT;
     constexpr int LCAP = MAXL + 64;
+    constexpr bool MASKED = NW != 1 && !COOONLY;
     const roman_params_t& P = D.p;
     const double p_eps = uni(P.eps), p_beta = uni(P.beta), p_tol_u = uni(P.tol_u), p_tol_F = uni(P.tol_F);
     const int p_maxin = uni(P.maxiniters), p_maxout = uni(P.maxoliters), p_maxls = uni(P.maxlsiters), p_rescale = uni(P.rescale_u0);
@@ -3851,6 +3873,9 @@
     const uint32_t cqv = cooPre >= 0 ? 0u : ((lane < nsl) ? (sliceBasePool[lo + lane] >> 8) : (st[b].nnzCap >> 8));
 #define CUMQ(s_) ((uint32_t)__builtin_amdgcn_readlane((int)cqv, (s_)))
     for (int p = tid; p < Lc; p += NT) { xg[p] = 0.0; accM[p] = 0ull; accC[p] = 0ull; }
+    if constexpr (MASKED) {
+        for (int p = tid; p < Lc; p += NT) nqS[p] = p < L ? (uint16_t)((rowCntPool[lo + p] + 3u) >> 2) : (uint16_t)0;
+    }
     double u[KMAX], Wu[KMAX], sd[KMAX], tk[KMAX], Mn[KMAX], Cn[KMAX];
     FOR_K_ALL(k, p) {
         const bool in = p < L;
@@ -3941,8 +3966,37 @@
         const uint32_t T = COOONLY ? 0u : CUMQ(Sx);
         const uint32_t qs = (uint32_t)(((unsigned long long)T * (unsigned)w) / NW), qe = (uint32_t)(((unsigned long long)T * (unsigned)(w + 1)) / NW);
         [[maybe_unused]] unsigned long long rc[ST_D]; [[maybe_unused]] dbl2_t rv0[ST_D], rv1[ST_D];
+        [[maybe_unused]] int sL = 0; [[maybe_unused]] uint32_t baseL = 0u, nextBL = 0u, nqL = 0u, nqLn = 0u; [[maybe_unused]] bool ra[ST_D];
+        [[maybe_unused]] g_quad_cp cbU = nullptr; [[maybe_unused]] g_pair_cp vbU = nullptr;
+#define UP_RING_LOAD(T_, QQ_)                                                                               \
+        {                                                                                                   \
+            const uint32_t qq__ = (QQ_);                                                                    \
+            if (qq__ >= nextBL && sL + 1 < Sx) {                                                            \
+                const int sOld__ = sL;                                                                      \
+                do { ++sL; baseL = nextBL; nextBL = CUMQ(sL + 1); } while (qq__ >= nextBL && sL + 1 < Sx);  \
+                nqL = (sL == sOld__ + 1) ? nqLn : (uint32_t)nqS[sL * 64 + lane];                            \
+                nqLn = (uint32_t)nqS[(sL + 1) * 64 + lane];                                                 \
+            }                                                                                               \
+            ra[T_] = qq__ - baseL < nqL;                                                                    \
+            const uint32_t ln__ = ra[T_] ? (uint32_t)lane : 0u;                                             \
+            rc[T_] = cbU[(size_t)qq__ * 64 + ln__];                                                         \
+            rv0[T_] = vbU[(size_t)(2 * qq__) * 64 + ln__]; rv1[T_] = vbU[(size_t)(2 * qq__ + 1) * 64 + ln__]; \
+        }
         if constexpr (!COOONLY) {
             const uint32_t qlast = (qe > qs ? qe : qs + 1u) - 1u;
+            if constexpr (MASKED) {
+                cbU = T ? (g_quad_cp)(colsPool + st[b].nnzOff) : (g_quad_cp)colsPool;
+                vbU = T ? (g_pair_cp)(valsPool + st[b].nnzOff) : (g_pair_cp)valsPool;
+                {
+                    int lo_ = 0, hi_ = Sx;
+                    while (hi_ - lo_ > 1) { const int mid_ = (lo_ + hi_) >> 1; if (CUMQ(mid_) <= qs) lo_ = mid_; else hi_ = mid_; }
+                    sL = lo_;
+                }
+                baseL = CUMQ(sL); nextBL = CUMQ(sL + 1);
+                nqL = (uint32_t)nqS[sL * 64 + lane]; nqLn = (uint32_t)nqS[(sL + 1) * 64 + lane];
+#pragma unroll
+                for (int t = 0; t < ST_D; ++t) UP_RING_LOAD(t, min(qs + (uint32_t)t, qlast))
+            } else {
             g_quad_cp cb0 = T ? cbase : (g_quad_cp)colsPool + lane;
             g_pair_cp vb0 = T ? vbase : (g_pair_cp)valsPool + lane;
 #pragma unroll
@@ -3950,6 +4004,7 @@
                 const uint32_t qq = min(qs + (uint32_t)t, qlast);
                 rc[t] = cb0[(size_t)qq * 64];
                 rv0[t] = vb0[(size_t)(2 * qq) * 64]; rv1[t] = vb0[(size_t)(2 * qq + 1) * 64];
+            }
             }
         }
         FOR_K(k, p) if (p < L) xg[p] = tk[k] * sc;
@@ -4001,7 +4056,7 @@
                 (X_)[0] = *(G_)[0]; (X_)[1] = *(G_)[1]; (X_)[2] = *(G_)[2]; (X_)[3] = *(G_)[3];             \
             }
 #define UP_PUSH(G_, OFF_, V_) __hip_atomic_fetch_add((l_acc_p)(G_) + (OFF_), (V_), __ATOMIC_RELAXED, __HIP_MEMORY_SCOPE_WORKGROUP)
-#define UP_CONSUME(Q_, C_, V0_, V1_)                                                                        \
+#define UP_CONSUME(Q_, C_, V0_, V1_, A_)                                                                    \
             {                                                                                               \
                 [[maybe_unused]] const uint32_t clo = (uint32_t)(C_), chi = (uint32_t)((C_) >> 32);         \
                                                          \
@@ -4026,7 +4081,7 @@
                         scI += (unsigned long long)__double_as_longlong(xa[3] + FX_MAGIC);                  \
                     }                                                                                       \
                 }                                                                                           \
-                if (xp != 0.0) {                                \
+                if (xp != 0.0 && (!MASKED || (A_))) {  \
                     UP_PUSH(ga[0], LCAP, (unsigned long long)__double_as_longlong(fma(w0, xp, FX_MAGIC)) - FX_MAGIC_BITS); \
                     UP_PUSH(ga[1], LCAP, (unsigned long long)__double_as_longlong(fma(w1, xp, FX_MAGIC)) - FX_MAGIC_BITS); \
                     UP_PUSH(ga[2], LCAP, (unsigned long long)__double_as_longlong(fma(w2, xp, FX_MAGIC)) - FX_MAGIC_BITS); \
@@ -4052,19 +4107,27 @@
                     }                                                                                       \
                 }                                                                                           \
             }
-            UP_GATHER(rc[0], ga, xa)
+            [[maybe_unused]] const uint32_t inert2 = (((uint32_t)L + (uint32_t)lane) | ST_CZ) * 0x10001u;
+            [[maybe_unused]] const unsigned long long inertW = ((unsigned long long)inert2 << 32) | inert2;
+#define UP_WORD(T_) (MASKED ? (ra[T_] ? rc[T_] : inertW) : rc[T_])
+            unsigned long long cw = UP_WORD(0), cwn; [[maybe_unused]] bool ca = MASKED ? ra[0] : true, can = true;
+            UP_GATHER(cw, ga, xa)
             uint32_t q0 = qs;
             for (; q0 + ST_D <= qe; q0 += ST_D) {
 #pragma unroll
                 for (int t = 0; t < ST_D; ++t) {
                     const uint32_t q = q0 + t;
-                    const unsigned long long c = rc[t];
                     const dbl2_t v0 = rv0[t], v1 = rv1[t];
                     const uint32_t qn = min(q + (uint32_t)ST_D, qe - 1u);
+                    if constexpr (MASKED) UP_RING_LOAD(t, qn)
+                    else {
                     rc[t] = cbase[(size_t)qn * 64];
                     rv0[t] = vbase[(size_t)(2 * qn) * 64]; rv1[t] = vbase[(size_t)(2 * qn + 1) * 64];
-                    UP_GATHER(rc[(t + 1) % ST_D], gn, xn)
-                    UP_CONSUME(q, c, v0, v1)
+                    }
+                    cwn = UP_WORD((t + 1) % ST_D); if constexpr (MASKED) can = ra[(t + 1) % ST_D];
+                    UP_GATHER(cwn, gn, xn)
+                    UP_CONSUME(q, cw, v0, v1, ca)
+                    cw = cwn; ca = can;
 #pragma unroll
                     for (int e = 0; e < 4; ++e) { ga[e] = gn[e]; xa[e] = xn[e]; }
                 }
@@ -4073,12 +4136,15 @@
             for (int t = 0; t < ST_D; ++t) {
                 const uint32_t q = q0 + t;
                 if (q < qe) {
-                    UP_GATHER(rc[(t + 1) % ST_D], gn, xn)
-                    UP_CONSUME(q, rc[t], rv0[t], rv1[t])
+                    cwn = UP_WORD((t + 1) % ST_D); if constexpr (MASKED) can = ra[(t + 1) % ST_D];
+                    UP_GATHER(cwn, gn, xn)
+                    UP_CONSUME(q, cw, rv0[t], rv1[t], ca)
+                    cw = cwn; ca = can;
 #pragma unroll
                     for (int e = 0; e < 4; ++e) { ga[e] = gn[e]; xa[e] = xn[e]; }
                 }
             }
+#undef UP_WORD
 #undef UP_CONSUME
 #undef UP_PUSH
 #undef UP_GATHER
@@ -4086,6 +4152,7 @@
         if (!COOONLY && qs < qe) {
             if (split) stream(std::true_type{}); else stream(std::false_type{});
         }
+#undef UP_RING_LOAD
         TMARK(Sx <= 2 ? 4 : 0);
         __syncthreads();
         TMARK(1);
@@ -4260,7 +4327,7 @@
                                                       const double* __restrict__ feats, const int32_t* __restrict__ assoc,
                                                       const int32_t* __restrict__ plp, const int32_t* __restrict__ lpAsc,
                                                       const uint32_t* __restrict__ rowPos, const double* __restrict__ pld,
-                                                      const uint32_t* __restrict__ sliceBase,
+                                                      const uint32_t* __restrict__ sliceBase, const uint32_t* __restrict__ rowCnt,
                                                       const uint16_t* __restrict__ cols, const double* __restrict__ vals,
                                                       const double* __restrict__ u0, SolveOut O,
                                                       int* __restrict__ queue, int Lc, int Llo, int Lhi, int R )
@@ -4273,6 +4340,7 @@
     uint32_t* cumQ = reinterpret_cast<uint32_t*>(red + red_doubles(NW));
     int* sint = reinterpret_cast<int*>(cumQ + ST_MAXSL + 2);
     unsigned char* cooLds = reinterpret_cast<unsigned char*>(sint + 8);
+    uint16_t* nqS = reinterpret_cast<uint16_t*>(sint + 8);
     for (;;) {
         if (threadIdx.x < WAVE) {
             const int ln = threadIdx.x;
@@ -4300,7 +4368,7 @@
         mask &= mask - 1ull;
         const ProbDesc pd = probs[b];
         solve_up<NW, HASCZ, MAXL>(D, b, pd, st, feats, assoc, plp, lpAsc, rowPos, pld, sliceBase, cols, vals, u0, O,
-                                  xg, accM, accC, Lc, cumQ, red, sint, cooLds);
+                                  xg, accM, accC, Lc, cumQ, red, sint, cooLds, rowCnt, nqS);
         __syncthreads();
         }
     }
@@ -4493,7 +4561,7 @@
             __syncthreads();
             SMARK(5);
             solve_up<1, false, SMALL_MAXL, true>(D, b, pd, st, feats, assoc, plp, lp, rowPos, pld, nullptr, nullptr, nullptr, u0, O,
-                                           xg, accM, accC, Lc1, cumQ, red, sint, cooLds, (int)nk, (int)lo);
+                                           xg, accM, accC, Lc1, cumQ, red, sint, cooLds, nullptr, nullptr, (int)nk, (int)lo);
             if (lane == 0) st[b].kind = 3;
 #ifdef ROMAN_SMALL_TIMING
             SMARK(6);
diff --git a/roman_amd/csrc/roman_hip.hip b/roman_amd/csrc/roman_hip.hip
--- a/roman_amd/csrc/roman_hip.hip
+++ b/roman_amd/csrc/roman_hip.hip
@@ -739,7 +739,9 @@
     DBG(c, "k_upper");
         }
         }
-        hipLaunchKernelGGL(k_slicegeom, dim3(B), dim3(64), 0, WS.stream, dP, dS, WS.rowCnt.as<uint32_t>(), WS.sliceWidth.as<uint32_t>(), WS.sliceBase.as<uint32_t>());
+        const int geomThr = 64 * std::max(1, std::min(16, (expL + 63) / 64));
+        hipLaunchKernelGGL(k_slicegeom, dim3(B), dim3(geomThr), 0, WS.stream, dP, dS, WS.rowCnt.as<uint32_t>(), WS.perm.as<uint32_t>(), WS.rowPos.as<uint32_t>(),
+                           WS.listOff.as<uint32_t>(), PP.lp, PP.ld, WS.sliceWidth.as<uint32_t>(), WS.sliceBase.as<uint32_t>());
     DBG(c, "k_slicegeom");
     }
     int NG = (int)std::max<int64_t>(1, std::min<int64_t>(FILLS_MAXSPI, (3 * (int64_t)c->num_cu + B / 2) / std::max(B, 1)));
@@ -824,7 +826,7 @@
 #endif
     constexpr int NW = SOLVE_WAVES;
     const int Lc = STREAM_MAXL + 64;
-    const size_t ldsUp = (size_t)3 * 8 * Lc + sizeof(double) * red_doubles(NW) + sizeof(uint32_t) * (ST_MAXSL + 2) + sizeof(int) * 8 + 16;
+    const size_t ldsUp = (size_t)3 * 8 * Lc + sizeof(double) * red_doubles(NW) + sizeof(uint32_t) * (ST_MAXSL + 2) + sizeof(int) * 8 + 16 + sizeof(uint16_t) * Lc;
     const int wgPerCu = std::max(1, std::min((int)(c->lds_max / ldsUp), 2048 / (NW * 64)));
     const int gridUp = std::max(1, std::min(B, c->num_cu * wgPerCu));
 
@@ -850,12 +852,12 @@
         auto kup = k_solve_up<NW, CZ_, STREAM_MAXL>;                                                                          \
         HIPCHK(c, dyn_lds(c, reinterpret_cast<const void*>(kup), ldsUp)); \
         hipLaunchKernelGGL(kup, dim3(gridUp), dim3(NW * 64), ldsUp, WS.stream, D, B, WS.probs.as<ProbDesc>(), WS.state.as<ProbState>(), feats, assoc, \
-                           WS.plp.as<int32_t>(), WS.lp.as<int32_t>(), WS.rowPos.as<uint32_t>(), WS.pld.as<double>(), WS.sliceBase.as<uint32_t>(), \
+                           WS.plp.as<int32_t>(), WS.lp.as<int32_t>(), WS.rowPos.as<uint32_t>(), WS.pld.as<double>(), WS.sliceBase.as<uint32_t>(), WS.rowCnt.as<uint32_t>(), \
                            WS.cols16.as<uint16_t>(), WS.vals.as<double>(), u0, O, WS.queue.as<int>(), Lc, small ? SMALL_MAXL + 1 : 0, STREAM_MAXL, (small && c->hist.valid && !c->hist.largeSeen) ? 64 : 1); \
         if (small) {                                                                                                          \
             HIPCHK(c, dyn_lds(c, reinterpret_cast<const void*>(k_solve_up<1, CZ_, SMALL_MAXL>), ldsUp1));                       \
             hipLaunchKernelGGL((k_solve_up<1, CZ_, SMALL_MAXL>), dim3(gridUp1), dim3(64), ldsUp1, WS.stream, D, B, WS.probs.as<ProbDesc>(), WS.state.as<ProbState>(), feats, assoc, \
-                               WS.plp.as<int32_t>(), WS.lp.as<int32_t>(), WS.rowPos.as<uint32_t>(), WS.pld.as<double>(), WS.sliceBase.as<uint32_t>(), \
+                               WS.plp.as<int32_t>(), WS.lp.as<int32_t>(), WS.rowPos.as<uint32_t>(), WS.pld.as<double>(), WS.sliceBase.as<uint32_t>(), WS.rowCnt.as<uint32_t>(), \
                                WS.cols16.as<uint16_t>(), WS.vals.as<double>(), u0, O, WS.queue.as<int>() + 1, Lc1, 0, SMALL_MAXL, 1); \
         }                                                                                                                     \
     } while (0)
@@ -2950,7 +2952,8 @@
             hipLaunchKernelGGL(k_upper, dim3(c->num_cu * 2), dim3(1024), 0, WS.stream, dP, dS, dT, WS.items.as<ItemDesc>(),
                                WS.maskPool.as<unsigned long long>(), WS.listPool.as<uint16_t>(), WS.listOff.as<uint32_t>(),
                                WS.rowCnt.as<uint32_t>(), WS.perm.as<uint32_t>(), WS.rowPos.as<uint32_t>(), LP, PP, RPB);
-            hipLaunchKernelGGL(k_slicegeom, dim3(1), dim3(64), 0, WS.stream, dP, dS, WS.rowCnt.as<uint32_t>(), WS.sliceWidth.as<uint32_t>(), WS.sliceBase.as<uint32_t>());
+            hipLaunchKernelGGL(k_slicegeom, dim3(1), dim3(64 * std::max(1, std::min(16, (n + 63) / 64))), 0, WS.stream, dP, dS, WS.rowCnt.as<uint32_t>(), WS.perm.as<uint32_t>(),
+                               WS.rowPos.as<uint32_t>(), WS.listOff.as<uint32_t>(), PP.lp, PP.ld, WS.sliceWidth.as<uint32_t>(), WS.sliceBase.as<uint32_t>());
         }
     }
     HIPCHK(c, hipGetLastError());
@@ -3180,4 +3183,18 @@
     return ROMAN_OK;
 }
 
-}
+int roman_debug_positions(const roman_ctx_t* cc, int32_t* n_live, int32_t* pos, int32_t* upper)
+{
+    if (!cc) return fail(nullptr, ROMAN_E_INVALID, "ctx is NULL");
+    roman_ctx* c = const_cast<roman_ctx*>(cc);
+    if (!c->last.scored) return fail(c, ROMAN_E_INVALID, "nothing scored yet");
+    const int L = c->last.L;
+    if (n_live) *n_live = L;
+    if (c->last.kind != 0) return fail(c, ROMAN_E_INVALID, "the last problem is not in the stream layout");
+    HIPCHK(c, hipSetDevice(c->device));
+    if (pos && L > 0) HIPCHK(c, hipMemcpy(pos, c->ws[0].rowPos.p, sizeof(uint32_t) * (size_t)L, hipMemcpyDeviceToHost));
+    if (upper && L > 0) HIPCHK(c, hipMemcpy(upper, c->ws[0].rowCnt.p, sizeof(uint32_t) * (size_t)L, hipMemcpyDeviceToHost));
+    return ROMAN_OK;
+}
+
+}
diff --git a/roman_amd/runtime.py b/roman_amd/runtime.py
--- a/roman_amd/runtime.py
+++ b/roman_amd/runtime.py
@@ -796,6 +796,13 @@
         self._check(self._lib.roman_debug_live(self._h, C.byref(n), _ptr(idx), _ptr(sc)), "roman_debug_live")
         return idx[:n.value].copy(), sc[:n.value].copy()
 
+    def positions(self):
+        n = C.c_int32(0)
+        self._check(self._lib.roman_debug_positions(self._h, C.byref(n), None, None), "roman_debug_positions")
+        pos = np.zeros(max(n.value, 1), dtype=np.int32); up = np.zeros(max(n.value, 1), dtype=np.int32)
+        self._check(self._lib.roman_debug_positions(self._h, C.byref(n), _ptr(pos), _ptr(up)), "roman_debug_positions")
+        return pos[:n.value].copy(), up[:n.value].copy()
+
     def pose_batch(self, dim, pts1, pts2, corr_off):
         pts1 = _f64(pts1).reshape(-1, dim); pts2 = _f64(pts2).reshape(-1, dim)
         corr_off = np.ascontiguousarray(corr_off, dtype=np.int64)
```

Result: no change. 180,200 alignments/s (median of 6 runs) (+0.8%).
